# LeiXu84/fireFoam-dev

Measured on AMD Instinct MI355X. Metric: PIMPLE outer-iterations/sec on 64M-cell hex mesh; pEqn SpMV GB/s vs HBM peak, higher is better.
Workload: dtype f64; 1 GPU; synthetic 400^3 hex box (64000000 cells), buoyant plume + 5-species EDC-shaped source, PIMPLE 1/2/0: rhoEqn + UEqn + YEEqn(4 Yi + h) + 2 pEqn per step; cells=64000000, faces=191520000, parallelism=1 GPU, transport_solvers=PBiCGStab+DILU

## Files before the change

### firefoam-dev_amd/csrc/ffm_fused.hip

```cpp
#include "ffm_mesh.hpp"

constexpr int FUSE_MAX = 4;
#define CHECK_M(m) if (!(m)) { ffm_set_error("null mesh"); return FFM_ERR_ARG; }

struct GradMulti {
    const double *vf[FUSE_MAX], *vb[FUSE_MAX];
    double *gx[FUSE_MAX], *gy[FUSE_MAX], *gz[FUSE_MAX];
};

template <int W, int NF>
__global__ __launch_bounds__(256) void k_grad_multi(MeshView q, GradMulti a)
{
    CELL_SCHED(ci, q) {
        const int c = (int)ci;
        RowEnt<W> L, U; load_lower<W>(q.v, c, L); load_upper<W>(q.v, c, U);
        double wl[W], wu[W], sx[2 * W], sy[2 * W], sz[2 * W];
#pragma unroll
        for (int s = 0; s < W; s++) {
            wl[s] = q.w[L.f[s]]; wu[s] = q.w[U.f[s]];
            sx[s] = q.Sfx[L.f[s]]; sy[s] = q.Sfy[L.f[s]]; sz[s] = q.Sfz[L.f[s]];
            sx[W + s] = q.Sfx[U.f[s]]; sy[W + s] = q.Sfy[U.f[s]]; sz[W + s] = q.Sfz[U.f[s]];
        }
        const double V = q.V[c];
        const int j = q.cellB[c];
#pragma unroll 1
        for (int i = 0; i < NF; i++) {
            const double *__restrict__ vf = a.vf[i];
            const double P = vf[c];
            double vl[W], vu[W];
#pragma unroll
            for (int s = 0; s < W; s++) { vl[s] = vf[L.nb[s]]; vu[s] = vf[U.nb[s]]; }
            double ax = 0, ay = 0, az = 0;
#pragma unroll
            for (int s = 0; s < W; s++) if (L.on[s]) {
                const double ff = wl[s] * vl[s] + (1.0 - wl[s]) * P;
                ax -= sx[s] * ff; ay -= sy[s] * ff; az -= sz[s] * ff;
            }
#pragma unroll
            for (int s = 0; s < W; s++) if (U.on[s]) {
                const double ff = wu[s] * P + (1.0 - wu[s]) * vu[s];
                ax += sx[W + s] * ff; ay += sy[W + s] * ff; az += sz[W + s] * ff;
            }
            if (j >= 0) for (int t = q.bcStart[j]; t < q.bcStart[j + 1]; t++) {
                const int k = q.bcItem[t]; const double b = a.vb[i][k];
                ax += q.bSfx[k] * b; ay += q.bSfy[k] * b; az += q.bSfz[k] * b;
            }
            a.gx[i][c] = ax / V; a.gy[i][c] = ay / V; a.gz[i][c] = az / V;
        }
    }
}

__device__ __forceinline__ double limited_weight(int scheme, double twoByk, double lo, double hi, double flux, double wlin,
                                                 double P, double Nn, double dx, double dy, double dz, double gxu, double gyu, double gzu)
{
    const double p0 = flux >= 0 ? 1.0 : 0.0;
    const double gradf = Nn - P;
    const double gradcf = dx * gxu + dy * gyu + dz * gzu;
    double r;
    if (fabs(gradcf) >= 1000.0 * fabs(gradf)) {
        const double sa = gradcf >= 0 ? 1.0 : -1.0, sb = gradf >= 0 ? 1.0 : -1.0;
        r = 2.0 * 1000.0 * sa * sb - 1.0;
    } else r = 2.0 * (gradcf / gradf) - 1.0;
    double lim = fmax(fmin(twoByk * r, 1.0), 0.0);
    if (scheme == 3) {
        if ((flux > 0 && (P < lo || Nn > hi)) || (flux < 0 && (Nn < lo || P > hi))) lim = 0.0;
    }
    return lim * wlin + (1.0 - lim) * p0;
}

struct ScalarEqns {
    const double *vf[FUSE_MAX], *gx[FUSE_MAX], *gy[FUSE_MAX], *gz[FUSE_MAX], *vf0[FUSE_MAX];
    const double *f[FUSE_MAX], *ref[FUSE_MAX], *refGrad[FUSE_MAX];
    const double *su[FUSE_MAX];
    const double *su2[FUSE_MAX], *sp[FUSE_MAX];
    const double *expl[FUSE_MAX][3];
    double *diag[FUSE_MAX], *upper[FUSE_MAX], *lower[FUSE_MAX], *src[FUSE_MAX];
    const double *rho, *rho0, *phi, *phib, *gamma, *gammab;
    const double *Cx, *Cy, *Cz, *bMagSf, *bDelta;
    double rdt, twoByk, lo, hi;
    int scheme;
    const double *wGiven;
    int nOffDiag;
};

template <int W, int NF, bool GIVENW = false>
__global__ __launch_bounds__(256, ((NF > 1 && !GIVENW) ? 4 : 1)) void k_scalar_eqns(MeshView q, ScalarEqns a)
{
    CELL_SCHED(ci, q) {
        const int c = (int)ci;
        RowEnt<W> L, U; load_lower<W>(q.v, c, L); load_upper<W>(q.v, c, U);
        double fl[W], fu[W], wl[W], wu[W], gl[W], gu[W], dlx[W], dly[W], dlz[W], dux[W], duy[W], duz[W];
        const double cx = GIVENW ? 0.0 : a.Cx[c], cy = GIVENW ? 0.0 : a.Cy[c], cz = GIVENW ? 0.0 : a.Cz[c];
#pragma unroll
        for (int s = 0; s < W; s++) {
            const int el = L.f[s], eu = U.f[s];
            fl[s] = a.phi[el]; fu[s] = a.phi[eu];
            wl[s] = GIVENW ? a.wGiven[el] : q.w[el]; wu[s] = GIVENW ? a.wGiven[eu] : q.w[eu];
            gl[s] = a.gamma[el] * q.magSf[el] * q.delta[el]; gu[s] = a.gamma[eu] * q.magSf[eu] * q.delta[eu];
            if (!GIVENW) {
                dlx[s] = cx - a.Cx[L.nb[s]]; dly[s] = cy - a.Cy[L.nb[s]]; dlz[s] = cz - a.Cz[L.nb[s]];
                dux[s] = a.Cx[U.nb[s]] - cx; duy[s] = a.Cy[U.nb[s]] - cy; duz[s] = a.Cz[U.nb[s]] - cz;
            } else { dlx[s] = dly[s] = dlz[s] = dux[s] = duy[s] = duz[s] = 0.0; }
        }
        const double V = q.V[c], rhoc = a.rho[c], rho0c = a.rho0[c];
        const int j = q.cellB[c];
#ifndef FFM_SE2_UNROLL
#define FFM_SE2_UNROLL 1
#endif
#pragma unroll FFM_SE2_UNROLL
        for (int i = 0; i < NF; i++) {
            const double *__restrict__ vf = a.vf[i], *__restrict__ gx = a.gx[i], *__restrict__ gy = a.gy[i], *__restrict__ gz = a.gz[i];
            const double P = GIVENW ? 0.0 : vf[c], gxc = GIVENW ? 0.0 : gx[c], gyc = GIVENW ? 0.0 : gy[c], gzc = GIVENW ? 0.0 : gz[c];
            double dDiv = 0.0, dLap = 0.0;
#pragma unroll
            for (int s = 0; s < W; s++) if (L.on[s]) {
                const int o = L.nb[s];
                const double flux = fl[s];
                const bool upO = flux > 0;
                const double w = GIVENW ? wl[s] : limited_weight(a.scheme, a.twoByk, a.lo, a.hi, flux, wl[s], vf[o], P, dlx[s], dly[s], dlz[s],
                                                                  upO ? gx[o] : gxc, upO ? gy[o] : gyc, upO ? gz[o] : gzc);
                (void)o; (void)upO;
                const double lo = -w * flux;
                dDiv -= (lo + flux);
                dLap -= gl[s];
            }
#pragma unroll
            for (int s = 0; s < W; s++) if (U.on[s]) {
                const int n = U.nb[s];
                const double flux = fu[s];
                const bool upO = flux > 0;
                const double w = GIVENW ? wu[s] : limited_weight(a.scheme, a.twoByk, a.lo, a.hi, flux, wu[s], P, vf[n], dux[s], duy[s], duz[s],
                                                                  upO ? gxc : gx[n], upO ? gyc : gy[n], upO ? gzc : gz[n]);
                (void)n; (void)upO;
                double lo = -w * flux, up = lo + flux;
                dDiv -= lo;
                dLap -= gu[s];
                lo = lo - gu[s]; up = up - gu[s];
                if (!GIVENW || i < a.nOffDiag) { a.upper[i][U.f[s]] = up; a.lower[i][U.f[s]] = lo; }
            }
            double d = a.rdt * rhoc * V;
            d = d + dDiv;
            d = d - dLap;
            double sc = a.rdt * rho0c * a.vf0[i][c] * V;
            if (a.expl[i][0]) sc = ((sc - V * a.expl[i][0][c]) - V * a.expl[i][1][c]) - V * a.expl[i][2][c];
            if (a.su[i]) sc = sc + V * a.su[i][c];
            if (a.sp[i]) d = d + V * a.sp[i][c];
            if (a.su2[i]) sc = sc + V * a.su2[i][c];
            if (j >= 0) for (int t = q.bcStart[j]; t < q.bcStart[j + 1]; t++) {
                const int k = q.bcItem[t];
                const double fk = a.f[i][k], rk = a.ref[i][k], gk = a.refGrad[i][k], dk = a.bDelta[k], pb = a.phib[k];
                double ic = pb * (1.0 - fk), bc = -pb * (fk * rk + (1.0 - fk) * gk / dk);
                const double pG = a.gammab[k] * a.bMagSf[k];
                const double li = pG * (-fk * dk), lb = -pG * (fk * dk * rk + (1.0 - fk) * gk);
                ic = ic - li; bc = bc - lb;
                d += ic; sc += bc;
            }
            a.diag[i][c] = d; a.src[i][c] = sc;
        }
    }
}

constexpr int MV_MAX = 8;
struct MvWeights {
    const double *vf[MV_MAX], *gx[MV_MAX], *gy[MV_MAX], *gz[MV_MAX];
    int scheme[MV_MAX], nf;
    const double *phi, *Cx, *Cy, *Cz;
    double twoByk, lo, hi;
    double *out;
};
__device__ __forceinline__ double mv_limiter(int scheme, double twoByk, double lo, double hi, double flux, double P, double Nn, double gradcf)
{
    const double gradf = Nn - P;
    double r;
    if (fabs(gradcf) >= 1000.0 * fabs(gradf)) {
        const double sa = gradcf >= 0 ? 1.0 : -1.0, sb = gradf >= 0 ? 1.0 : -1.0;
        r = 2.0 * 1000.0 * sa * sb - 1.0;
    } else r = 2.0 * (gradcf / gradf) - 1.0;
    double l = fmax(fmin(twoByk * r, 1.0), 0.0);
    if (scheme == 3) {
        if ((flux > 0 && (P < lo || Nn > hi)) || (flux < 0 && (Nn < lo || P > hi))) l = 0.0;
    }
    return l;
}
template <int W>
__global__ __launch_bounds__(256) void k_mv_weights(MeshView q, MvWeights a)
{
    CELL_SCHED(ci, q) {
        const int c = (int)ci;
        RowEnt<W> L, U; load_lower<W>(q.v, c, L); load_upper<W>(q.v, c, U);
        const double cx = a.Cx[c], cy = a.Cy[c], cz = a.Cz[c];
        double fl[2 * W], lim[2 * W], dx[2 * W], dy[2 * W], dz[2 * W];
        bool mine[2 * W], ghostUp[W];
#pragma unroll
        for (int s = 0; s < W; s++) {
            fl[s] = L.on[s] ? a.phi[L.f[s]] : 0.0; mine[s] = L.on[s] && !(fl[s] > 0);
            dx[s] = cx - a.Cx[L.nb[s]]; dy[s] = cy - a.Cy[L.nb[s]]; dz[s] = cz - a.Cz[L.nb[s]];
            fl[W + s] = U.on[s] ? a.phi[U.f[s]] : 0.0; mine[W + s] = U.on[s] && fl[W + s] > 0;
            ghostUp[s] = U.on[s] && !(fl[W + s] > 0) && U.nb[s] >= q.v.N;
            dx[W + s] = a.Cx[U.nb[s]] - cx; dy[W + s] = a.Cy[U.nb[s]] - cy; dz[W + s] = a.Cz[U.nb[s]] - cz;
            lim[s] = lim[W + s] = 1.0;
        }
#pragma unroll 1
        for (int i = 0; i < a.nf; i++) {
            const double *__restrict__ vf = a.vf[i];
            const double vc = vf[c], gxc = a.gx[i][c], gyc = a.gy[i][c], gzc = a.gz[i][c];
            const int sch = a.scheme[i];
#pragma unroll
            for (int s = 0; s < W; s++) {
                if (mine[s]) {
                    const double l = mv_limiter(sch, a.twoByk, a.lo, a.hi, fl[s], vf[L.nb[s]], vc, dx[s] * gxc + dy[s] * gyc + dz[s] * gzc);
                    lim[s] = i == 0 ? l : fmin(lim[s], l);
                }
                if (mine[W + s]) {
                    const double l = mv_limiter(sch, a.twoByk, a.lo, a.hi, fl[W + s], vc, vf[U.nb[s]], dx[W + s] * gxc + dy[W + s] * gyc + dz[W + s] * gzc);
                    lim[W + s] = i == 0 ? l : fmin(lim[W + s], l);
                } else if (ghostUp[s]) {
                    const int n = U.nb[s];
                    const double l = mv_limiter(sch, a.twoByk, a.lo, a.hi, fl[W + s], vc, vf[n], dx[W + s] * a.gx[i][n] + dy[W + s] * a.gy[i][n] + dz[W + s] * a.gz[i][n]);
                    lim[W + s] = i == 0 ? l : fmin(lim[W + s], l);
                }
            }
        }
#pragma unroll
        for (int s = 0; s < W; s++) {
            if (mine[s]) { const int e = L.f[s]; const double p0 = fl[s] >= 0 ? 1.0 : 0.0; a.out[e] = lim[s] * q.w[e] + (1.0 - lim[s]) * p0; }
            if (mine[W + s] || ghostUp[s]) { const int e = U.f[s]; const double p0 = fl[W + s] >= 0 ? 1.0 : 0.0; a.out[e] = lim[W + s] * q.w[e] + (1.0 - lim[W + s]) * p0; }
        }
    }
// ... 111 lines not shown
                }
#pragma unroll
                for (int s = 0; s < 2 * W; s++) gcur[s] = gnext[s];
            }
#pragma unroll
            for (int s = 0; s < W; s++) {
                if (mine[s]) { const int e = L.f[s]; const double p0 = fl[s] >= 0 ? 1.0 : 0.0; a.out[e] = lim[s] * q.w[e] + (1.0 - lim[s]) * p0; }
                if (mine[W + s]) { const int e = U.f[s]; const double p0 = fl[W + s] >= 0 ? 1.0 : 0.0; a.out[e] = lim[W + s] * q.w[e] + (1.0 - lim[W + s]) * p0; }
            }
        }
        __syncthreads();
    }
}

extern "C" int ffm_fv_multivariate_weights_tiled(ffm_mesh *m, int nf, const int *schemes, double k, double lo, double hi, const double *phi_f,
                                                 const double *const *vf, const double *const *vb, double *out_w)
{
    CHECK_M(m);
    if (nf < 1 || !schemes || !phi_f || !vf || !vb || !out_w) return FFM_ERR_ARG;
    FfmFvSegs sg;
    if (nf > MVT_FLD || m->A->maxW > 3 || !ffm_tile_fv_segments(m->A, MVT_RUN, &sg)) return FFM_ERR_UNSUPPORTED;
    MvTile a;
    for (int i = 0; i < MVT_FLD; i++) {
        const int qq = i < nf ? i : 0;
        if (i < nf && ((schemes[qq] != 2 && schemes[qq] != 3) || !vf[qq] || (m->B && !vb[qq]))) return FFM_ERR_ARG;
        a.vf[i] = vf[qq]; a.vb[i] = vb[qq]; a.scheme[i] = schemes[qq];
    }
    a.nf = nf; a.phi = phi_f; a.Cx = m->C[0]; a.Cy = m->C[1]; a.Cz = m->C[2]; a.twoByk = 2.0 / std::max(k, 1e-15); a.lo = lo; a.hi = hi; a.out = out_w;
    a.seg = sg.seg; a.rec = sg.rec;
    hipLaunchKernelGGL(k_mv_tile<3>, dim3(sg.nSeg), dim3(256), 0, m->ctx->stream, mview(m), a);
    FFM_HIP(hipGetLastError());
    return FFM_OK;
}

struct LustSource {
    const double *gx[3], *gy[3], *gz[3], *U0[3];
    double *src[3];
    const double *phi, *rho0, *Cx, *Cy, *Cz, *Cfx, *Cfy, *Cfz;
    double rdt;
};

template <int W>
__global__ __launch_bounds__(256) void k_lust_source(MeshView q, LustSource a)
{
    CELL_SCHED(ci, q) {
        const int c = (int)ci;
        RowEnt<W> L, U; load_lower<W>(q.v, c, L); load_upper<W>(q.v, c, U);
        const double cx = a.Cx[c], cy = a.Cy[c], cz = a.Cz[c];
        double fl[W], fu[W], dlx[W], dly[W], dlz[W], dux[W], duy[W], duz[W];
        int upl[W], upu[W];
#pragma unroll
        for (int s = 0; s < W; s++) {
            const int el = L.f[s], eu = U.f[s];
            fl[s] = a.phi[el]; fu[s] = a.phi[eu];
            upl[s] = fl[s] > 0 ? L.nb[s] : c;
            upu[s] = fu[s] > 0 ? c : U.nb[s];
            dlx[s] = a.Cfx[el] - a.Cx[upl[s]]; dly[s] = a.Cfy[el] - a.Cy[upl[s]]; dlz[s] = a.Cfz[el] - a.Cz[upl[s]];
            dux[s] = a.Cfx[eu] - a.Cx[upu[s]]; duy[s] = a.Cfy[eu] - a.Cy[upu[s]]; duz[s] = a.Cfz[eu] - a.Cz[upu[s]];
        }
        (void)cx; (void)cy; (void)cz;
        const double V = q.V[c], r0 = a.rho0[c];
#pragma unroll
        for (int i = 0; i < 3; i++) {
            const double *__restrict__ gx = a.gx[i], *__restrict__ gy = a.gy[i], *__restrict__ gz = a.gz[i];
            double acc = 0.0;
#pragma unroll
            for (int s = 0; s < W; s++) if (L.on[s]) {
                const int u = upl[s];
                const double corr = 0.25 * ((dlx[s] * gx[u] + dly[s] * gy[u]) + dlz[s] * gz[u]);
                acc -= fl[s] * corr;
            }
#pragma unroll
            for (int s = 0; s < W; s++) if (U.on[s]) {
                const int u = upu[s];
                const double corr = 0.25 * ((dux[s] * gx[u] + duy[s] * gy[u]) + duz[s] * gz[u]);
                acc += fu[s] * corr;
            }
            const double divc = acc / V;
            a.src[i][c] = a.rdt * r0 * a.U0[i][c] * V - V * divc;
        }
    }
}


extern "C" int ffm_fvc_grad_multi(ffm_mesh *m, int nf, const double *const *vf, const double *const *vb, double *const *gx,
                                  double *const *gy, double *const *gz)
{
    CHECK_M(m);
    if (nf < 1 || nf > FUSE_MAX || !vf || !vb || !gx || !gy || !gz) return FFM_ERR_ARG;
    GradMulti a;
    for (int i = 0; i < FUSE_MAX; i++) { const int k = i < nf ? i : 0; a.vf[i] = vf[k]; a.vb[i] = vb[k]; a.gx[i] = gx[k]; a.gy[i] = gy[k]; a.gz[i] = gz[k]; }
    for (int i = 0; i < nf; i++) if (!vf[i] || (m->B && !vb[i]) || !gx[i] || !gy[i] || !gz[i]) return FFM_ERR_ARG;
#define GM(NF) FFM_DISPATCH_W(m->A->maxW, LAUNCH_CELLS((k_grad_multi<W, NF>), mview(m), a))
    switch (nf) { case 1: GM(1); break; case 2: GM(2); break; case 3: GM(3); break; default: GM(4); break; }
#undef GM
    FFM_HIP(hipGetLastError());
    return FFM_OK;
}

extern "C" int ffm_fvm_scalar_transport_multi(ffm_mesh *m, int nf, int scheme, double k, double lo, double hi, double rDeltaT,
                                              const double *rho, const double *rho0, const double *phi_f, const double *phi_b,
                                              const double *gamma_f, const double *gamma_b,
                                              const double *const *vf, const double *const *gx, const double *const *gy,
                                              const double *const *gz, const double *const *vf0, const double *const *f,
                                              const double *const *ref, const double *const *refGrad, const double *const *su,
                                              const double *const *su2, const double *const *sp,
                                              const double *const *expl3, double *const *diag, double *const *upper,
                                              double *const *lower, double *const *source)
{
    CHECK_M(m);
    if (nf < 1 || nf > FUSE_MAX || (scheme != 2 && scheme != 3) || !rho || !rho0 || !phi_f || !gamma_f || (m->B && (!phi_b || !gamma_b)))
        return FFM_ERR_ARG;
    if (!vf || !gx || !gy || !gz || !vf0 || !f || !ref || !refGrad || !diag || !upper || !lower || !source) return FFM_ERR_ARG;
    ScalarEqns a;
    for (int i = 0; i < FUSE_MAX; i++) {
        const int q = i < nf ? i : 0;
        if (i < nf && (!vf[q] || !gx[q] || !gy[q] || !gz[q] || !vf0[q] || !diag[q] || !upper[q] || !lower[q] || !source[q] ||
                       (m->B && (!f[q] || !ref[q] || !refGrad[q])))) return FFM_ERR_ARG;
        a.vf[i] = vf[q]; a.gx[i] = gx[q]; a.gy[i] = gy[q]; a.gz[i] = gz[q]; a.vf0[i] = vf0[q];
        a.f[i] = f[q]; a.ref[i] = ref[q]; a.refGrad[i] = refGrad[q];
        a.su[i] = su ? su[q] : nullptr;
        a.su2[i] = su2 ? su2[q] : nullptr; a.sp[i] = sp ? sp[q] : nullptr;
        for (int e = 0; e < 3; e++) a.expl[i][e] = expl3 ? expl3[3 * q + e] : nullptr;
        if (a.expl[i][0] && (!a.expl[i][1] || !a.expl[i][2])) return FFM_ERR_ARG;
        a.diag[i] = diag[q]; a.upper[i] = upper[q]; a.lower[i] = lower[q]; a.src[i] = source[q];
    }
    a.rho = rho; a.rho0 = rho0; a.phi = phi_f; a.phib = phi_b; a.gamma = gamma_f; a.gammab = gamma_b;
    a.Cx = m->C[0]; a.Cy = m->C[1]; a.Cz = m->C[2]; a.bMagSf = m->bMagSf; a.bDelta = m->bDelta;
    a.rdt = rDeltaT; a.twoByk = 2.0 / std::max(k, 1e-15); a.lo = lo; a.hi = hi; a.scheme = scheme; a.wGiven = nullptr; a.nOffDiag = nf;
#define SE(NF) FFM_DISPATCH_W(m->A->maxW, LAUNCH_CELLS((k_scalar_eqns<W, NF>), mview(m), a))
    switch (nf) { case 1: SE(1); break; case 2: SE(2); break; case 3: SE(3); break; default: SE(4); break; }
#undef SE
    FFM_HIP(hipGetLastError());
    return FFM_OK;
}

extern "C" int ffm_fv_multivariate_weights(ffm_mesh *m, int nf, const int *schemes, double k, double lo, double hi, const double *phi_f,
                                           const double *const *vf, const double *const *gx, const double *const *gy, const double *const *gz,
                                           double *out_w)
{
    CHECK_M(m);
    if (nf < 1 || nf > MV_MAX || !schemes || !phi_f || !vf || !gx || !gy || !gz || !out_w) return FFM_ERR_ARG;
    MvWeights a;
    for (int i = 0; i < MV_MAX; i++) {
        const int q = i < nf ? i : 0;
        if (i < nf && ((schemes[q] != 2 && schemes[q] != 3) || !vf[q] || !gx[q] || !gy[q] || !gz[q])) return FFM_ERR_ARG;
        a.vf[i] = vf[q]; a.gx[i] = gx[q]; a.gy[i] = gy[q]; a.gz[i] = gz[q]; a.scheme[i] = schemes[q];
    }
    a.nf = nf; a.phi = phi_f; a.Cx = m->C[0]; a.Cy = m->C[1]; a.Cz = m->C[2]; a.twoByk = 2.0 / std::max(k, 1e-15); a.lo = lo; a.hi = hi; a.out = out_w;
    FFM_DISPATCH_W(m->A->maxW, LAUNCH_CELLS(k_mv_weights<W>, mview(m), a));
    FFM_HIP(hipGetLastError());
    return FFM_OK;
}

extern "C" int ffm_fvm_scalar_transport_multi_w(ffm_mesh *m, int nf, const double *w_f, double rDeltaT, const double *rho, const double *rho0,
                                                const double *phi_f, const double *phi_b, const double *gamma_f, const double *gamma_b,
                                                const double *const *vf0, const double *const *f, const double *const *ref,
                                                const double *const *refGrad, const double *const *su, const double *const *su2,
                                                const double *const *sp, const double *const *expl3, double *const *diag,
                                                double *const *upper, double *const *lower, double *const *source)
{
    CHECK_M(m);
    if (nf < 1 || nf > FUSE_MAX || !w_f || !rho || !rho0 || !phi_f || !gamma_f || (m->B && (!phi_b || !gamma_b))) return FFM_ERR_ARG;
    if (!vf0 || !f || !ref || !refGrad || !diag || !upper || !lower || !source) return FFM_ERR_ARG;
    ScalarEqns a;
    for (int i = 0; i < FUSE_MAX; i++) {
        const int q = i < nf ? i : 0;
        if (i < nf && (!vf0[q] || !diag[q] || !source[q] || (m->B && (!f[q] || !ref[q] || !refGrad[q])))) return FFM_ERR_ARG;
        a.vf[i] = a.gx[i] = a.gy[i] = a.gz[i] = nullptr; a.vf0[i] = vf0[q];
        a.f[i] = f[q]; a.ref[i] = ref[q]; a.refGrad[i] = refGrad[q];
        a.su[i] = su ? su[q] : nullptr;
        a.su2[i] = su2 ? su2[q] : nullptr; a.sp[i] = sp ? sp[q] : nullptr;
        for (int e = 0; e < 3; e++) a.expl[i][e] = expl3 ? expl3[3 * q + e] : nullptr;
        if (a.expl[i][0] && (!a.expl[i][1] || !a.expl[i][2])) return FFM_ERR_ARG;
        a.diag[i] = diag[q]; a.upper[i] = upper[q]; a.lower[i] = lower[q]; a.src[i] = source[q];
    }
    a.rho = rho; a.rho0 = rho0; a.phi = phi_f; a.phib = phi_b; a.gamma = gamma_f; a.gammab = gamma_b;
    a.Cx = m->C[0]; a.Cy = m->C[1]; a.Cz = m->C[2]; a.bMagSf = m->bMagSf; a.bDelta = m->bDelta;
    a.rdt = rDeltaT; a.twoByk = 2.0; a.lo = 0.0; a.hi = 1.0; a.scheme = 0; a.wGiven = w_f;
    a.nOffDiag = 0;
    for (int i = 0; i < nf; i++) { if (upper[i] && lower[i]) { if (a.nOffDiag != i) return FFM_ERR_ARG; a.nOffDiag = i + 1; } else if ((upper[i] == nullptr) != (lower[i] == nullptr)) return FFM_ERR_ARG; }
#define SEW(NF) FFM_DISPATCH_W(m->A->maxW, LAUNCH_CELLS((k_scalar_eqns<W, NF, true>), mview(m), a))
    switch (nf) { case 1: SEW(1); break; case 2: SEW(2); break; case 3: SEW(3); break; default: SEW(4); break; }
#undef SEW
    FFM_HIP(hipGetLastError());
    return FFM_OK;
}

extern "C" int ffm_fvm_lust_source3(ffm_mesh *m, double rDeltaT, const double *phi_f, const double *rho0, const double *const *U0,
                                    const double *const *gx, const double *const *gy, const double *const *gz, double *const *source)
{
    CHECK_M(m);
    if (!phi_f || !rho0 || !U0 || !gx || !gy || !gz || !source) return FFM_ERR_ARG;
    if (!m->Cf[0]) { ffm_set_error("ffm_fvm_lust_source3: face centres not set (ffm_mesh_set_face_centres)"); return FFM_ERR_ARG; }
    LustSource a;
    for (int i = 0; i < 3; i++) {
        if (!U0[i] || !gx[i] || !gy[i] || !gz[i] || !source[i]) return FFM_ERR_ARG;
        a.gx[i] = gx[i]; a.gy[i] = gy[i]; a.gz[i] = gz[i]; a.U0[i] = U0[i]; a.src[i] = source[i];
    }
    a.phi = phi_f; a.rho0 = rho0; a.Cx = m->C[0]; a.Cy = m->C[1]; a.Cz = m->C[2]; a.Cfx = m->Cf[0]; a.Cfy = m->Cf[1]; a.Cfz = m->Cf[2];
    a.rdt = rDeltaT;
    FFM_DISPATCH_W(m->A->maxW, LAUNCH_CELLS(k_lust_source<W>, mview(m), a));
    FFM_HIP(hipGetLastError());
    return FFM_OK;
}

struct HbyA3 {
    const double *upper, *lower, *src[3], *ic[3], *bc[3], *psi[3], *rAU;
    double *out[3];
};
template <int W>
__global__ __launch_bounds__(256) void k_matrix_HbyA3(MeshView q, HbyA3 a)
{
    CELL_SCHED(ci, q) {
        const int c = (int)ci;
        RowEnt<W> L, U; load_lower<W>(q.v, c, L); load_upper<W>(q.v, c, U);
        double al[W], au[W];
#pragma unroll
        for (int s = 0; s < W; s++) { al[s] = a.lower[L.f[s]]; au[s] = a.upper[U.f[s]]; }
        double bd[3] = {0.0, 0.0, 0.0}, bda = 0.0, bs[3] = {0.0, 0.0, 0.0};
        const int j = q.cellB[c];
        if (j >= 0) for (int t = q.bcStart[j]; t < q.bcStart[j + 1]; t++) {
            const int k = q.bcItem[t];
            const double i0 = a.ic[0][k], i1 = a.ic[1][k], i2 = a.ic[2][k];
            bd[0] += i0; bd[1] += i1; bd[2] += i2; bda += (i0 + i1 + i2) / 3.0;
            bs[0] += a.bc[0][k]; bs[1] += a.bc[1][k]; bs[2] += a.bc[2][k];
        }
        const double V = q.V[c], r = a.rAU ? a.rAU[c] : 1.0;
#pragma unroll
        for (int d = 0; d < 3; d++) {
            const double *psi = a.psi[d];
            double hl = 0.0;
#pragma unroll
            for (int s = 0; s < W; s++) if (L.on[s]) hl -= al[s] * psi[L.nb[s]];
#pragma unroll
            for (int s = 0; s < W; s++) if (U.on[s]) hl -= au[s] * psi[U.nb[s]];
            double h = (bda - bd[d]) * psi[c];
            h += hl + a.src[d][c];
            h += bs[d];
            h = h / V;
            a.out[d][c] = a.rAU ? r * h : h;
        }
    }
}

extern "C" int ffm_fvm_HbyA3(ffm_mesh *m, const double *upper, const double *lower, const double *const *source, const double *const *ic,
                             const double *const *bc, const double *const *psi, const double *rAU, double *const *out)
{
    CHECK_M(m);
    if (!upper || !lower || !source || !ic || !bc || !psi || !out) return FFM_ERR_ARG;
    HbyA3 a; a.upper = upper; a.lower = lower; a.rAU = rAU;
    for (int d = 0; d < 3; d++) {
        if (!source[d] || !psi[d] || !out[d] || (m->B && (!ic[d] || !bc[d]))) return FFM_ERR_ARG;
        a.src[d] = source[d]; a.ic[d] = ic[d]; a.bc[d] = bc[d]; a.psi[d] = psi[d]; a.out[d] = out[d];
    }
    FFM_DISPATCH_W(m->A->maxW, LAUNCH_CELLS(k_matrix_HbyA3<W>, mview(m), a));
    FFM_HIP(hipGetLastError());
    return FFM_OK;
}

__global__ __launch_bounds__(256) void k_flux_rho(MeshView q, const double *__restrict__ rho, const double *__restrict__ vx,
                                                  const double *__restrict__ vy, const double *__restrict__ vz, double *__restrict__ out)
{
    CELL_SCHED(ci, q) {
        const int c = (int)ci; const double rP = rho[c]; const double Px = rP * vx[c], Py = rP * vy[c], Pz = rP * vz[c];
        FOR_OWN_FACES(q, c, e, nb) {
            const double w = q.w[e], rN = rho[nb];
            out[e] = (w * Px + (1.0 - w) * (rN * vx[nb])) * q.Sfx[e] + (w * Py + (1.0 - w) * (rN * vy[nb])) * q.Sfy[e] + (w * Pz + (1.0 - w) * (rN * vz[nb])) * q.Sfz[e];
        }
    }
}
extern "C" int ffm_fvc_flux_rho(ffm_mesh *m, const double *rho, const double *vx, const double *vy, const double *vz, double *out_f)
{
    CHECK_M(m);
    if (!rho || !vx || !vy || !vz || !out_f) return FFM_ERR_ARG;
    LAUNCH_CELLS(k_flux_rho, mview(m), rho, vx, vy, vz, out_f);
    FFM_HIP(hipGetLastError());
    return FFM_OK;
}

#define PC_ALL_SLOTS(q, c, e, nb)                                                      \
    const int sl_ = (c) >> 6, lane_ = (c)&63;                                          \
    const int ub_ = up_base((q).v, sl_), uw_ = up_width((q).v, sl_);                   \
    for (int s_ = 0, e = ub_ + lane_, nb = 0; s_ < uw_ && ((nb = (q).v.upNbr[e]), true); s_++, e += 64)
__global__ __launch_bounds__(256) void k_pc_phig(MeshView q, const double *__restrict__ rhorAUf, const double *__restrict__ ghf,
                                                 const double *__restrict__ rho, double *__restrict__ out)
{
    CELL_SCHED(ci, q) {
        const int c = (int)ci; const double P = rho[c];
        PC_ALL_SLOTS(q, c, e, nb) {
            if (nb < 0) { out[e] = 0.0; continue; }
            const double sg = q.delta[e] * (rho[nb] - P); out[e] = -rhorAUf[e] * ghf[e] * sg * q.magSf[e];
        }
    }
}
__global__ __launch_bounds__(256) void k_pc_phiHbyA(MeshView q, const double *__restrict__ rho, const double *__restrict__ vx,
                                                    const double *__restrict__ vy, const double *__restrict__ vz, const double *__restrict__ rhorAUf,
                                                    const double *__restrict__ dc, const double *__restrict__ phig, double *__restrict__ out)
{
    CELL_SCHED(ci, q) {
        const int c = (int)ci; const double rP = rho[c]; const double Px = rP * vx[c], Py = rP * vy[c], Pz = rP * vz[c];
        PC_ALL_SLOTS(q, c, e, nb) {
            if (nb < 0) { out[e] = 0.0; continue; }
            const double w = q.w[e], rN = rho[nb];
            const double fl = (w * Px + (1.0 - w) * (rN * vx[nb])) * q.Sfx[e] + (w * Py + (1.0 - w) * (rN * vy[nb])) * q.Sfy[e] + (w * Pz + (1.0 - w) * (rN * vz[nb])) * q.Sfz[e];
            out[e] = (fl + rhorAUf[e] * dc[e]) + phig[e];
        }
    }
}
__global__ __launch_bounds__(256) void k_pc_flux(MeshView q, const double *__restrict__ upper, const double *__restrict__ lower,
                                                 const double *__restrict__ psi, const double *__restrict__ phiHbyA, const double *__restrict__ phig,
                                                 const double *__restrict__ rhorAUf, double *__restrict__ fl, double *__restrict__ phi,
                                                 double *__restrict__ t)
{
    CELL_SCHED(ci, q) {
        const int c = (int)ci; const double P = psi[c];
        PC_ALL_SLOTS(q, c, e, nb) {
            if (nb < 0) { fl[e] = 0.0; phi[e] = 0.0; t[e] = 0.0; continue; }
            const double f = upper[e] * psi[nb] - lower[e] * P;
            fl[e] = f; phi[e] = phiHbyA[e] + f;
            t[e] = rhorAUf[e] != 0.0 ? (f + phig[e]) / rhorAUf[e] : 0.0;
        }
    }
}
__global__ __launch_bounds__(256) void k_ue_buoyancy_flux(MeshView q, const double *__restrict__ ghf, const double *__restrict__ rho,
                                                         const double *__restrict__ prgh, double *__restrict__ out)
{
    CELL_SCHED(ci, q) {
        const int c = (int)ci; const double rP = rho[c], pP = prgh[c];
        PC_ALL_SLOTS(q, c, e, nb) {
            if (nb < 0) { out[e] = 0.0; continue; }
            const double sgr = q.delta[e] * (rho[nb] - rP), sgp = q.delta[e] * (prgh[nb] - pP);
            out[e] = (-ghf[e] * sgr - sgp) * q.magSf[e];
        }
    }
}
extern "C" int ffm_ue_buoyancy_flux(ffm_mesh *m, const double *ghf, const double *rho, const double *p_rgh, double *t_f)
{
    CHECK_M(m);
    if (!ghf || !rho || !p_rgh || !t_f) return FFM_ERR_ARG;
    LAUNCH_CELLS(k_ue_buoyancy_flux, mview(m), ghf, rho, p_rgh, t_f);
    FFM_HIP(hipGetLastError());
    return FFM_OK;
}
extern "C" int ffm_pc_phig(ffm_mesh *m, const double *rhorAUf, const double *ghf, const double *rho, double *phig)
{
    CHECK_M(m);
    if (!rhorAUf || !ghf || !rho || !phig) return FFM_ERR_ARG;
    LAUNCH_CELLS(k_pc_phig, mview(m), rhorAUf, ghf, rho, phig);
    FFM_HIP(hipGetLastError());
    return FFM_OK;
}
extern "C" int ffm_pc_phiHbyA(ffm_mesh *m, const double *rho, const double *vx, const double *vy, const double *vz, const double *rhorAUf,
// ... 193 lines not shown
```

### firefoam-dev_amd/csrc/ffm_fv.hip

```cpp
#include "ffm_internal.hpp"
#include "ffm_device.hpp"
#include <algorithm>
#include <cmath>

#include "ffm_mesh.hpp"

template <class T, class Al> static int up(ffm_ctx *c, T **d, const std::vector<T, Al> &v)
{
    return ffm_upload_vec(c, d, v);
}

extern "C" int ffm_mesh_create(ffm_ldu *A, const double *V, const double *C, const double *Sf, const double *magSf,
                               const double *weights, const double *deltaCoeffs, int nPatches, const int *patchSizes,
                               const int *const *faceCells, const double *const *pSf, const double *const *pDelta,
                               ffm_mesh **out)
{
    if (!A || !V || !C || !out || nPatches < 0) return FFM_ERR_ARG;
    if (!A->identity) { ffm_set_error("ffm_mesh_create needs a mesh numbered with ffm_renumber_levels (native order)"); return FFM_ERR_UNSUPPORTED; }
    ffm_mesh *m = new ffm_mesh();
    m->A = A; m->ctx = A->ctx; m->N = A->nCells; m->F = A->nFaces; m->nNat = A->upTotal; m->nPatches = nPatches;
    const int N = m->N, F = m->F, nNat = m->nNat;
    m->patchOff.assign(nPatches + 1, 0);
    for (int p = 0; p < nPatches; p++) m->patchOff[p + 1] = m->patchOff[p] + patchSizes[p];
    m->B = m->patchOff[nPatches];
// ... 227 lines not shown
                const double d2 = (dx * a.gx[2][cc] + dy * a.gy[2][cc]) + dz * a.gz[2][cc];
                tc[s] = 2.0 * ((g0 * d0 + g1 * d1) + g2 * d2);
            }
            const double den = fmax(fabs(tc[0]), fabs(tc[1])) + 1.0e-15;
            double lim = (df > 0) ? l1 - kk * fmin(fmax(df - tc[0], 0.0), fmax(df - tc[1], 0.0)) / den
                                  : l1 - kk * fmin(fmax(tc[0] - df, 0.0), fmax(tc[1] - df, 0.0)) / den;
            lim = fmax(fmin(lim, 1.0), 0.0);
            const double p0 = phi[e] >= 0 ? 1.0 : 0.0;
            out[e] = lim * q.w[e] + (1.0 - lim) * p0;
        }
    }
}

__global__ void k_lust_correction(MeshView q, const double *__restrict__ phi, const double *__restrict__ gx, const double *__restrict__ gy,
                                  const double *__restrict__ gz, const double *__restrict__ Cx, const double *__restrict__ Cy,
                                  const double *__restrict__ Cz, const double *__restrict__ Cfx, const double *__restrict__ Cfy,
                                  const double *__restrict__ Cfz, double factor, double *__restrict__ out)
{
    CELL_SCHED(ci, q) {
        const int c = (int)ci;
        FOR_OWN_FACES(q, c, e, nb) {
            const int up = phi[e] > 0 ? c : nb;
            const double dx = Cfx[e] - Cx[up], dy = Cfy[e] - Cy[up], dz = Cfz[e] - Cz[up];
            out[e] = factor * ((dx * gx[up] + dy * gy[up]) + dz * gz[up]);
        }
    }
}

template <int W>
__global__ void k_relax(MeshView q, double alpha, int nc, const double *__restrict__ upper, const double *__restrict__ lower,
                        const double *__restrict__ ic0, const double *__restrict__ ic1, const double *__restrict__ ic2,
                        double *__restrict__ diag, const double *__restrict__ p0, const double *__restrict__ p1,
                        const double *__restrict__ p2, double *__restrict__ s0, double *__restrict__ s1, double *__restrict__ s2)
{
    CELL_SCHED(ci, q) {
        const int c = (int)ci;
        RowEnt<W> L, U; load_lower<W>(q.v, c, L); load_upper<W>(q.v, c, U);
        double sumOff = 0.0;
#pragma unroll
        for (int s = 0; s < W; s++) if (L.on[s]) sumOff += fabs(lower[L.f[s]]);
#pragma unroll
        for (int s = 0; s < W; s++) if (U.on[s]) sumOff += fabs(upper[U.f[s]]);
        const double D0 = diag[c];
        double D = D0;
        const int j = q.cellB[c];
        if (j >= 0) for (int t = q.bcStart[j]; t < q.bcStart[j + 1]; t++) {
            const int k = q.bcItem[t];
            D += (nc == 3) ? fmax(fmax(fabs(ic0[k]), fabs(ic1[k])), fabs(ic2[k])) : fabs(ic0[k]);
        }
        D = fmax(fabs(D), sumOff);
        D = D / alpha;
        if (j >= 0) for (int t = q.bcStart[j]; t < q.bcStart[j + 1]; t++) {
            const int k = q.bcItem[t];
            D -= (nc == 3) ? fmin(fmin(ic0[k], ic1[k]), ic2[k]) : ic0[k];
        }
        diag[c] = D;
        const double dd = D - D0;
        s0[c] += dd * p0[c];
        if (nc == 3) { s1[c] += dd * p1[c]; s2[c] += dd * p2[c]; }
    }
}

template <int MODE, int W>
__global__ void k_face_sum(MeshView q, const double *__restrict__ ssf, const double *__restrict__ ssb, double *__restrict__ out)
{
    CELL_SCHED(ci, q) {
        const int c = (int)ci;
        RowEnt<W> L, U; load_lower<W>(q.v, c, L); load_upper<W>(q.v, c, U);
        double a[W], b[W];
#pragma unroll
        for (int s = 0; s < W; s++) { a[s] = ssf[L.f[s]]; b[s] = ssf[U.f[s]]; }
        double acc = 0.0;
#pragma unroll
        for (int s = 0; s < W; s++) if (L.on[s]) acc = (MODE == 0) ? acc - a[s] : acc + a[s];
#pragma unroll
        for (int s = 0; s < W; s++) if (U.on[s]) acc += b[s];
        const int j = q.cellB[c];
        if (j >= 0 && ssb) for (int t = q.bcStart[j]; t < q.bcStart[j + 1]; t++) acc += ssb[q.bcItem[t]];
        out[c] = (MODE == 0) ? acc / q.V[c] : acc;
    }
}

template <int W>
__global__ void k_grad(MeshView q, const double *__restrict__ vf, const double *__restrict__ vb, double *__restrict__ gx,
                       double *__restrict__ gy, double *__restrict__ gz)
{
    CELL_SCHED(ci, q) {
        const int c = (int)ci;
        RowEnt<W> L, U; load_lower<W>(q.v, c, L); load_upper<W>(q.v, c, U);
        const double P = vf[c];
        double vl[W], vu[W], wl[W], wu[W], sx[2 * W], sy[2 * W], sz[2 * W];
#pragma unroll
        for (int s = 0; s < W; s++) {
            vl[s] = vf[L.nb[s]]; vu[s] = vf[U.nb[s]]; wl[s] = q.w[L.f[s]]; wu[s] = q.w[U.f[s]];
            sx[s] = q.Sfx[L.f[s]]; sy[s] = q.Sfy[L.f[s]]; sz[s] = q.Sfz[L.f[s]];
            sx[W + s] = q.Sfx[U.f[s]]; sy[W + s] = q.Sfy[U.f[s]]; sz[W + s] = q.Sfz[U.f[s]];
        }
        double ax = 0, ay = 0, az = 0;
#pragma unroll
        for (int s = 0; s < W; s++) if (L.on[s]) {
            const double ff = wl[s] * vl[s] + (1.0 - wl[s]) * P;
            ax -= sx[s] * ff; ay -= sy[s] * ff; az -= sz[s] * ff;
        }
#pragma unroll
        for (int s = 0; s < W; s++) if (U.on[s]) {
            const double ff = wu[s] * P + (1.0 - wu[s]) * vu[s];
            ax += sx[W + s] * ff; ay += sy[W + s] * ff; az += sz[W + s] * ff;
        }
        const int j = q.cellB[c];
        if (j >= 0) for (int t = q.bcStart[j]; t < q.bcStart[j + 1]; t++) {
            const int k = q.bcItem[t]; const double b = vb[k];
            ax += q.bSfx[k] * b; ay += q.bSfy[k] * b; az += q.bSfz[k] * b;
        }
        const double V = q.V[c];
        gx[c] = ax / V; gy[c] = ay / V; gz[c] = az / V;
    }
}

template <int W>
__global__ void k_reconstruct(MeshView q, long invStride, const double *__restrict__ invT, const double *__restrict__ bMagSf,
                              const double *__restrict__ ssf, const double *__restrict__ ssb, double *__restrict__ ox,
                              double *__restrict__ oy, double *__restrict__ oz)
{
    CELL_SCHED(ci, q) {
        const int c = (int)ci; const long N = invStride;
        RowEnt<W> L, U; load_lower<W>(q.v, c, L); load_upper<W>(q.v, c, U);
        double vx = 0, vy = 0, vz = 0;
#pragma unroll
        for (int s = 0; s < W; s++) if (L.on[s]) {
            const int e = L.f[s]; const double t = ssf[e], mg = q.magSf[e];
            vx += q.Sfx[e] / mg * t; vy += q.Sfy[e] / mg * t; vz += q.Sfz[e] / mg * t;
        }
#pragma unroll
        for (int s = 0; s < W; s++) if (U.on[s]) {
            const int e = U.f[s]; const double t = ssf[e], mg = q.magSf[e];
            vx += q.Sfx[e] / mg * t; vy += q.Sfy[e] / mg * t; vz += q.Sfz[e] / mg * t;
        }
        const int j = q.cellB[c];
        if (j >= 0 && ssb) for (int t = q.bcStart[j]; t < q.bcStart[j + 1]; t++) {
            const int k = q.bcItem[t]; const double b = ssb[k], mg = bMagSf[k];
            vx += q.bSfx[k] / mg * b; vy += q.bSfy[k] / mg * b; vz += q.bSfz[k] / mg * b;
        }
        const double xx = invT[c], xy = invT[N + c], xz = invT[2 * N + c], yy = invT[3 * N + c], yz = invT[4 * N + c], zz = invT[5 * N + c];
        ox[c] = xx * vx + xy * vy + xz * vz; oy[c] = xy * vx + yy * vy + yz * vz; oz[c] = xz * vx + yz * vy + zz * vz;
    }
}

template <int W>
__global__ void k_fvm_transport(MeshView q, double rDeltaT, const double *__restrict__ rho, const double *__restrict__ phi,
                                const double *__restrict__ wf, const double *__restrict__ gamma, double lapSign,
                                double *__restrict__ diag, double *__restrict__ upper, double *__restrict__ lower)
{
    CELL_SCHED(ci, q) {
        const int c = (int)ci;
        RowEnt<W> L, U; load_lower<W>(q.v, c, L); load_upper<W>(q.v, c, U);
        double dDiv = 0.0, dLap = 0.0;
#pragma unroll
        for (int s = 0; s < W; s++) if (L.on[s]) {
            const int e = L.f[s];
            if (phi) { const double f = phi[e]; const double lo = -wf[e] * f; dDiv -= (lo + f); }
            if (gamma) dLap -= gamma[e] * q.magSf[e] * q.delta[e];
        }
#pragma unroll
        for (int s = 0; s < W; s++) if (U.on[s]) {
            const int e = U.f[s];
            double lo = 0.0, up = 0.0;
            if (phi) { const double f = phi[e]; lo = -wf[e] * f; up = lo + f; dDiv -= lo; }
            if (gamma) {
                const double g = gamma[e] * q.magSf[e] * q.delta[e];
                dLap -= g;
                if (phi) { lo = lapSign < 0 ? lo - g : lo + g; up = lapSign < 0 ? up - g : up + g; }
                else { lo = lapSign < 0 ? -g : g; up = lo; }
            }
            if (upper) upper[e] = up;
            if (lower) lower[e] = lo;
        }
        double d = rho ? rDeltaT * rho[c] * q.V[c] : 0.0;
        if (phi) d = rho ? d + dDiv : dDiv;
        if (gamma) d = (rho || phi) ? (lapSign < 0 ? d - dLap : d + dLap) : (lapSign < 0 ? -dLap : dLap);
        diag[c] = d;
    }
}

__global__ void k_boundary_coeffs(int B, const double *__restrict__ phib, const double *__restrict__ gammab, double lapSign,
                                  const double *__restrict__ magSf, const double *__restrict__ delta, const double *__restrict__ f,
                                  const double *__restrict__ ref, const double *__restrict__ refGrad, double *__restrict__ ic,
                                  double *__restrict__ bc)
{
    GRID_STRIDE(k, B) {
        const double fk = f[k], rk = ref[k], gk = refGrad[k], dk = delta[k];
        double i = 0.0, b = 0.0;
        if (phib) { i = phib[k] * (1.0 - fk); b = -phib[k] * (fk * rk + (1.0 - fk) * gk / dk); }
        if (gammab) {
            const double pG = gammab[k] * magSf[k];
            const double li = pG * (-fk * dk), lb = -pG * (fk * dk * rk + (1.0 - fk) * gk);
            if (phib) { i = lapSign < 0 ? i - li : i + li; b = lapSign < 0 ? b - lb : b + lb; }
            else { i = lapSign < 0 ? -li : li; b = lapSign < 0 ? -lb : lb; }
        }
        ic[k] = i; bc[k] = b;
    }
}

__global__ void k_bc_values(int B, const int *__restrict__ fc, const double *__restrict__ delta, const double *__restrict__ f,
                            const double *__restrict__ ref, const double *__restrict__ refGrad, const double *__restrict__ vf,
                            double *__restrict__ out)
{ GRID_STRIDE(k, B) out[k] = f[k] * ref[k] + (1.0 - f[k]) * (vf[fc[k]] + refGrad[k] / delta[k]); }

__global__ void k_add_boundary(MeshView q, const double *__restrict__ ic, const double *__restrict__ bc,
                               const double *__restrict__ diag, const double *__restrict__ src, const double *__restrict__ su,
                               double *__restrict__ diagOut, double *__restrict__ srcOut)
{
    CELL_SCHED(ci, q) {
        const int c = (int)ci;
        double d = diag ? diag[c] : 0.0, s = src ? src[c] : 0.0;
        const int j = q.cellB[c];
        if (j >= 0) for (int t = q.bcStart[j]; t < q.bcStart[j + 1]; t++) { const int k = q.bcItem[t]; if (ic) d += ic[k]; if (bc) s += bc[k]; }
        if (su) s += q.V[c] * su[c];
        if (diagOut) diagOut[c] = d;
        if (srcOut) srcOut[c] = s;
    }
}

__global__ void k_matrix_A(MeshView q, int nc, const double *__restrict__ diag, const double *__restrict__ ic0,
                           const double *__restrict__ ic1, const double *__restrict__ ic2, double *__restrict__ out)
{
    CELL_SCHED(ci, q) {
        const int c = (int)ci;
        double d = diag[c];
        const int j = q.cellB[c];
        if (j >= 0) for (int t = q.bcStart[j]; t < q.bcStart[j + 1]; t++) {
            const int k = q.bcItem[t];
            d += (nc == 3) ? (ic0[k] + ic1[k] + ic2[k]) / 3.0 : ic0[k];
        }
        out[c] = d / q.V[c];
    }
}

template <int W>
__global__ void k_matrix_H(MeshView q, int nc, const double *__restrict__ upper, const double *__restrict__ lower,
                           const double *__restrict__ src, const double *__restrict__ icC, const double *__restrict__ ic0,
                           const double *__restrict__ ic1, const double *__restrict__ ic2, const double *__restrict__ bcC,
                           const double *__restrict__ psi, double *__restrict__ out)
{
    CELL_SCHED(ci, q) {
        const int c = (int)ci;
        RowEnt<W> L, U; load_lower<W>(q.v, c, L); load_upper<W>(q.v, c, U);
        double al[W], au[W], xl[W], xu[W];
#pragma unroll
        for (int s = 0; s < W; s++) { al[s] = lower[L.f[s]]; au[s] = upper[U.f[s]]; xl[s] = psi[L.nb[s]]; xu[s] = psi[U.nb[s]]; }
        double bd = 0.0, bda = 0.0, bs = 0.0;
        const int j = q.cellB[c];
        if (j >= 0) for (int t = q.bcStart[j]; t < q.bcStart[j + 1]; t++) {
            const int k = q.bcItem[t];
            bd += icC[k]; bda += (nc == 3) ? (ic0[k] + ic1[k] + ic2[k]) / 3.0 : ic0[k]; bs += bcC[k];
        }
        double hl = 0.0;
#pragma unroll
        for (int s = 0; s < W; s++) if (L.on[s]) hl -= al[s] * xl[s];
#pragma unroll
        for (int s = 0; s < W; s++) if (U.on[s]) hl -= au[s] * xu[s];
        double h = (bda - bd) * psi[c];
        h += hl + src[c];
        h += bs;
        out[c] = h / q.V[c];
    }
}

__global__ void k_matrix_flux(MeshView q, const double *__restrict__ upper, const double *__restrict__ lower,
                              const double *__restrict__ psi, double *__restrict__ out)
{
    CELL_SCHED(ci, q) {
        const int c = (int)ci; const double P = psi[c];
        FOR_OWN_FACES(q, c, e, nb) out[e] = upper[e] * psi[nb] - lower[e] * P;
    }
}
__global__ void k_matrix_flux_b(int B, const int *__restrict__ fc, const double *__restrict__ ic, const double *__restrict__ bc,
                                const double *__restrict__ psi, double *__restrict__ out)
{ GRID_STRIDE(k, B) out[k] = ic[k] * psi[fc[k]] - bc[k]; }

#define CHECK_M(m) if (!(m)) { ffm_set_error("null mesh"); return FFM_ERR_ARG; }
#define DONE() FFM_HIP(hipGetLastError()); return FFM_OK

extern "C" int ffm_fvc_interpolate(ffm_mesh *m, const double *w_f, const double *vf, double *out_f)
{ CHECK_M(m); LAUNCH_CELLS(k_interpolate, mview(m), w_f, vf, out_f); DONE(); }
extern "C" int ffm_fvc_snGrad(ffm_mesh *m, const double *vf, double *out_f)
{ CHECK_M(m); LAUNCH_CELLS(k_snGrad, mview(m), vf, out_f); DONE(); }
extern "C" int ffm_fvc_snGrad_b(ffm_mesh *m, const double *vf, const double *vb, double *out_b)
{ CHECK_M(m); if (m->B) LAUNCH(k_snGrad_b, m->B, m->B, m->bCells, m->bDelta, vf, vb, out_b); DONE(); }
extern "C" int ffm_fvc_flux(ffm_mesh *m, const double *vx, const double *vy, const double *vz, double *out_f)
{ CHECK_M(m); LAUNCH_CELLS(k_flux, mview(m), vx, vy, vz, out_f); DONE(); }
extern "C" int ffm_fvc_surface_integrate(ffm_mesh *m, const double *ssf, const double *ssb, double *out)
{ CHECK_M(m); FFM_DISPATCH_W(m->A->maxW, LAUNCH_CELLS((k_face_sum<0, W>), mview(m), ssf, ssb, out)); DONE(); }
extern "C" int ffm_fvc_surface_sum(ffm_mesh *m, const double *ssf, const double *ssb, double *out)
{ CHECK_M(m); FFM_DISPATCH_W(m->A->maxW, LAUNCH_CELLS((k_face_sum<1, W>), mview(m), ssf, ssb, out)); DONE(); }
extern "C" int ffm_fvc_grad(ffm_mesh *m, const double *vf, const double *vb, double *gx, double *gy, double *gz)
{ CHECK_M(m); FFM_DISPATCH_W(m->A->maxW, LAUNCH_CELLS(k_grad<W>, mview(m), vf, vb, gx, gy, gz)); DONE(); }
extern "C" int ffm_fvc_reconstruct(ffm_mesh *m, const double *ssf, const double *ssb, double *ox, double *oy, double *oz)
{ CHECK_M(m); FFM_DISPATCH_W(m->A->maxW, LAUNCH_CELLS(k_reconstruct<W>, mview(m), (long)m->N, m->invT, m->bMagSf, ssf, ssb, ox, oy, oz)); DONE(); }
extern "C" int ffm_fv_limited_weights(ffm_mesh *m, int scheme, double k, double lo, double hi, const double *phi_f,
                                      const double *vf, const double *gx, const double *gy, const double *gz, double *out_w)
{
    CHECK_M(m);
    if (scheme < 0 || scheme > 5 || !phi_f || !out_w || ((scheme == 2 || scheme == 3) && (!vf || !gx || !gy || !gz))) return FFM_ERR_ARG;
    LAUNCH_CELLS(k_limited_weights<0>, mview(m), scheme, 2.0 / std::max(k, 1e-15), lo, hi, phi_f, vf, gx, gy, gz, m->C[0], m->C[1], m->C[2], out_w);
    DONE();
}
extern "C" int ffm_fv_limited_limiter(ffm_mesh *m, int scheme, double k, double lo, double hi, const double *phi_f, const double *vf,
                                      const double *gx, const double *gy, const double *gz, double *lim_f, int accumulateMin)
{
    CHECK_M(m);
    if ((scheme != 2 && scheme != 3) || !phi_f || !lim_f || !vf || !gx || !gy || !gz) return FFM_ERR_ARG;
    if (accumulateMin) LAUNCH_CELLS(k_limited_weights<2>, mview(m), scheme, 2.0 / std::max(k, 1e-15), lo, hi, phi_f, vf, gx, gy, gz, m->C[0], m->C[1], m->C[2], lim_f);
    else LAUNCH_CELLS(k_limited_weights<1>, mview(m), scheme, 2.0 / std::max(k, 1e-15), lo, hi, phi_f, vf, gx, gy, gz, m->C[0], m->C[1], m->C[2], lim_f);
    DONE();
}
__global__ void k_weights_from_limiter(MeshView q, const double *__restrict__ phi, const double *__restrict__ lim, double *__restrict__ out)
{
    CELL_SCHED(ci, q) {
        const int c = (int)ci;
        FOR_OWN_FACES(q, c, e, nb) { (void)nb; const double l = lim[e], p0 = phi[e] >= 0 ? 1.0 : 0.0; out[e] = l * q.w[e] + (1.0 - l) * p0; }
    }
}
extern "C" int ffm_fv_weights_from_limiter(ffm_mesh *m, const double *phi_f, const double *lim_f, double *out_w)
{
    CHECK_M(m);
    if (!phi_f || !lim_f || !out_w) return FFM_ERR_ARG;
    LAUNCH_CELLS(k_weights_from_limiter, mview(m), phi_f, lim_f, out_w);
    DONE();
}
extern "C" int ffm_fv_filtered_linear2V_weights(ffm_mesh *m, double k, double l, const double *phi_f, const double *const *U,
                                                const double *const *gx, const double *const *gy, const double *const *gz, double *out_w)
{
    CHECK_M(m);
    if (!phi_f || !U || !gx || !gy || !gz || !out_w || k < 0 || k > 1 || l < 0 || l > 1) return FFM_ERR_ARG;
    FL2V a;
    for (int d = 0; d < 3; d++) {
        if (!U[d] || !gx[d] || !gy[d] || !gz[d]) return FFM_ERR_ARG;
        a.U[d] = U[d]; a.gx[d] = gx[d]; a.gy[d] = gy[d]; a.gz[d] = gz[d];
    }
    LAUNCH_CELLS(k_filtered_linear2V_weights, mview(m), k, l + 1.0, phi_f, a, m->C[0], m->C[1], m->C[2], out_w);
    DONE();
}
extern "C" int ffm_mesh_set_face_centres(ffm_mesh *m, const double *Cf)
{
    CHECK_M(m);
    if (!Cf) return FFM_ERR_ARG;
    std::vector<double> v(std::max(m->nNat, 1));
    for (int d = 0; d < 3; d++) {
        const int *c2n = m->A->h_callerToNative.data(); double *vp = v.data(); const double *src = Cf + (size_t)d * m->F;
        ffm_parallel_for(m->nNat, [=](long lo, long hi) { for (long q = lo; q < hi; q++) vp[q] = 0.0; });
        ffm_parallel_for(m->F, [=](long lo, long hi) { for (long f = lo; f < hi; f++) vp[c2n[f]] = src[f]; });
        hipFree(m->Cf[d]); m->Cf[d] = nullptr;
        FFM_TRY(up(m->ctx, &m->Cf[d], v));
    }
    return FFM_OK;
}
extern "C" int ffm_mesh_set_nonorth_correction(ffm_mesh *m, const double *corrVec)
{
    CHECK_M(m);
    if (!corrVec) return FFM_ERR_ARG;
    std::vector<double> v(std::max(m->nNat, 1));
    for (int d = 0; d < 3; d++) {
        const int *c2n = m->A->h_callerToNative.data(); double *vp = v.data(); const double *src = corrVec + (size_t)d * m->F;
        ffm_parallel_for(m->nNat, [=](long lo, long hi) { for (long q = lo; q < hi; q++) vp[q] = 0.0; });
        ffm_parallel_for(m->F, [=](long lo, long hi) { for (long f = lo; f < hi; f++) vp[c2n[f]] = src[f]; });
        hipFree(m->corr[d]); m->corr[d] = nullptr;
        FFM_TRY(up(m->ctx, &m->corr[d], v));
    }
    return FFM_OK;
}
extern "C" int ffm_fvc_snGrad_correction(ffm_mesh *m, const double *gx, const double *gy, const double *gz, double *out_f)
{
    CHECK_M(m);
    if (!gx || !gy || !gz || !out_f) return FFM_ERR_ARG;
    if (!m->corr[0]) { ffm_set_error("ffm_fvc_snGrad_correction: correction vectors not set (ffm_mesh_set_nonorth_correction)"); return FFM_ERR_ARG; }
    LAUNCH_CELLS(k_snGrad_correction, mview(m), m->corr[0], m->corr[1], m->corr[2], gx, gy, gz, out_f);
    DONE();
}
extern "C" int ffm_fv_lust_correction(ffm_mesh *m, const double *phi_f, const double *gx, const double *gy, const double *gz, double *out_f)
{
    CHECK_M(m);
    if (!phi_f || !gx || !gy || !gz || !out_f) return FFM_ERR_ARG;
    if (!m->Cf[0]) { ffm_set_error("ffm_fv_lust_correction: face centres not set (ffm_mesh_set_face_centres)"); return FFM_ERR_ARG; }
    LAUNCH_CELLS(k_lust_correction, mview(m), phi_f, gx, gy, gz, m->C[0], m->C[1], m->C[2], m->Cf[0], m->Cf[1], m->Cf[2], 0.25, out_f);
    DONE();
}
extern "C" int ffm_fv_linear_upwind_correction(ffm_mesh *m, const double *phi_f, const double *gx, const double *gy, const double *gz, double *out_f)
{
    CHECK_M(m);
    if (!phi_f || !gx || !gy || !gz || !out_f) return FFM_ERR_ARG;
    if (!m->Cf[0]) { ffm_set_error("ffm_fv_linear_upwind_correction: face centres not set (ffm_mesh_set_face_centres)"); return FFM_ERR_ARG; }
    LAUNCH_CELLS(k_lust_correction, mview(m), phi_f, gx, gy, gz, m->C[0], m->C[1], m->C[2], m->Cf[0], m->Cf[1], m->Cf[2], 1.0, out_f);
    DONE();
}
extern "C" int ffm_fvm_relax(ffm_mesh *m, double alpha, int nc, const double *upper, const double *lower, const double *ic0,
                             const double *ic1, const double *ic2, double *diag, const double *psi0, const double *psi1,
                             const double *psi2, double *src0, double *src1, double *src2)
{
    CHECK_M(m);
    if ((nc != 1 && nc != 3) || !upper || !lower || !diag || !psi0 || !src0 || (m->B && !ic0)) return FFM_ERR_ARG;
    if (nc == 3 && (!psi1 || !psi2 || !src1 || !src2 || (m->B && (!ic1 || !ic2)))) return FFM_ERR_ARG;
    if (alpha <= 0) return FFM_OK;
    FFM_DISPATCH_W(m->A->maxW, LAUNCH_CELLS(k_relax<W>, mview(m), alpha, nc, upper, lower, ic0, ic1, ic2, diag, psi0, psi1, psi2, src0, src1, src2));
    DONE();
}
extern "C" int ffm_fvm_transport(ffm_mesh *m, double rDeltaT, const double *rho, const double *phi_f, const double *w_f,
                                 const double *gamma_f, int laplacianSign, double *diag, double *upper, double *lower)
{
    CHECK_M(m);
    if (!diag || ((phi_f || gamma_f) && !upper) || (phi_f && (!w_f || !lower))) return FFM_ERR_ARG;
    FFM_DISPATCH_W(m->A->maxW, LAUNCH_CELLS(k_fvm_transport<W>, mview(m), rDeltaT, rho, phi_f, w_f, gamma_f, (double)laplacianSign, diag, upper, lower));
    DONE();
}
extern "C" int ffm_fvm_boundary_coeffs(ffm_mesh *m, const double *phib, const double *gammab, int laplacianSign, const double *f,
                                       const double *ref, const double *refGrad, double *ic, double *bc)
{ CHECK_M(m); if (m->B) LAUNCH(k_boundary_coeffs, m->B, m->B, phib, gammab, (double)laplacianSign, m->bMagSf, m->bDelta, f, ref, refGrad, ic, bc); DONE(); }
extern "C" int ffm_bc_values(ffm_mesh *m, const double *f, const double *ref, const double *refGrad, const double *vf, double *out_b)
{ CHECK_M(m); if (m->B) LAUNCH(k_bc_values, m->B, m->B, m->bCells, m->bDelta, f, ref, refGrad, vf, out_b); DONE(); }
extern "C" int ffm_fvm_add_boundary(ffm_mesh *m, const double *ic, const double *bc, const double *diag, const double *src,
                                    const double *su, double *diagOut, double *srcOut)
{ CHECK_M(m); LAUNCH_CELLS(k_add_boundary, mview(m), ic, bc, diag, src, su, diagOut, srcOut); DONE(); }
extern "C" int ffm_fvm_A(ffm_mesh *m, int nc, const double *diag, const double *ic0, const double *ic1, const double *ic2, double *out)
{ CHECK_M(m); if (nc != 1 && nc != 3) return FFM_ERR_ARG; LAUNCH_CELLS(k_matrix_A, mview(m), nc, diag, ic0, ic1, ic2, out); DONE(); }
extern "C" int ffm_fvm_H(ffm_mesh *m, int nc, int cmpt, const double *upper, const double *lower, const double *src,
                         const double *ic0, const double *ic1, const double *ic2, const double *bcC, const double *psi, double *out)
{
    CHECK_M(m); if ((nc != 1 && nc != 3) || cmpt < 0 || cmpt >= nc) return FFM_ERR_ARG;
    const double *icC = cmpt == 0 ? ic0 : cmpt == 1 ? ic1 : ic2;
    FFM_DISPATCH_W(m->A->maxW, LAUNCH_CELLS(k_matrix_H<W>, mview(m), nc, upper, lower, src, icC, ic0, ic1, ic2, bcC, psi, out));
    DONE();
}
extern "C" int ffm_fvm_flux(ffm_mesh *m, const double *upper, const double *lower, const double *ic, const double *bc,
                            const double *psi, double *out_f, double *out_b)
{
    CHECK_M(m);
    if (out_f) LAUNCH_CELLS(k_matrix_flux, mview(m), upper, lower, psi, out_f);
    if (m->B && out_b) LAUNCH(k_matrix_flux_b, m->B, m->B, m->bCells, ic, bc, psi, out_b);
    DONE();
}

extern "C" const double *ffm_mesh_geometry_d(const ffm_mesh *m, int which)
{
    if (!m) return nullptr;
    switch (which) {
    case 0: return m->V; case 1: return m->magSf; case 2: return m->delta; case 3: return m->w; case 4: return m->bMagSf; case 5: return m->bDelta;
    case 6: return m->bSf[0]; case 7: return m->bSf[1]; case 8: return m->bSf[2];
    case 9: return m->Sf[0]; case 10: return m->Sf[1]; case 11: return m->Sf[2]; case 12: return m->C[0]; case 13: return m->C[1]; case 14: return m->C[2];
    }
    return nullptr;
}

const int *ffm_mesh_bcells(const ffm_mesh *m) { return m->bCells; }
const double *ffm_mesh_geom(const ffm_mesh *m, int which)
{
    switch (which) {
    case 0: return m->V; case 1: return m->magSf; case 2: return m->delta; case 3: return m->w;
    case 4: return m->bMagSf; case 5: return m->bDelta; case 6: return m->bSf[0]; case 7: return m->bSf[1]; case 8: return m->bSf[2];
    case 9: return m->Sf[0]; case 10: return m->Sf[1]; case 11: return m->Sf[2]; case 12: return m->C[0]; case 13: return m->C[1]; case 14: return m->C[2];
    }
    return nullptr;
}
```

### firefoam-dev_amd/csrc/ffm_plume.hip

```cpp
#include "ffm_internal.hpp"
#include "ffm_device.hpp"
#include <algorithm>
#include <cmath>
#include <string>

struct ffm_mesh;
extern "C" {
int ffm_ldu_bind_coeffs_native_d(ffm_ldu *, const double *, const double *, const double *, int);
int ffm_mesh_create(ffm_ldu *, const double *, const double *, const double *, const double *, const double *, const double *, int,
                    const int *, const int *const *, const double *const *, const double *const *, ffm_mesh **);
int ffm_mesh_destroy(ffm_mesh *);
int ffm_mesh_set_face_centres(ffm_mesh *, const double *);
int ffm_fv_lust_correction(ffm_mesh *, const double *, const double *, const double *, const double *, double *);
int ffm_fvc_interpolate(ffm_mesh *, const double *, const double *, double *);
int ffm_fvc_snGrad(ffm_mesh *, const double *, double *);
int ffm_fvc_snGrad_b(ffm_mesh *, const double *, const double *, double *);
int ffm_fvc_flux(ffm_mesh *, const double *, const double *, const double *, double *);
int ffm_fvc_surface_integrate(ffm_mesh *, const double *, const double *, double *);
int ffm_fvc_grad(ffm_mesh *, const double *, const double *, double *, double *, double *);
int ffm_fvc_reconstruct(ffm_mesh *, const double *, const double *, double *, double *, double *);
int ffm_fv_limited_weights(ffm_mesh *, int, double, double, double, const double *, const double *, const double *, const double *,
                           const double *, double *);
int ffm_fvm_transport(ffm_mesh *, double, const double *, const double *, const double *, const double *, int, double *, double *, double *);
int ffm_fvm_boundary_coeffs(ffm_mesh *, const double *, const double *, int, const double *, const double *, const double *, double *, double *);
int ffm_bc_values(ffm_mesh *, const double *, const double *, const double *, const double *, double *);
int ffm_fvm_add_boundary(ffm_mesh *, const double *, const double *, const double *, const double *, const double *, double *, double *);
int ffm_fvm_A(ffm_mesh *, int, const double *, const double *, const double *, const double *, double *);
int ffm_fvm_H(ffm_mesh *, int, int, const double *, const double *, const double *, const double *, const double *, const double *,
              const double *, const double *, double *);
int ffm_fvm_flux(ffm_mesh *, const double *, const double *, const double *, const double *, const double *, double *, double *);
int ffm_fvc_grad_multi(ffm_mesh *, int, const double *const *, const double *const *, double *const *, double *const *, double *const *);
int ffm_fvm_scalar_transport_multi(ffm_mesh *, int, int, double, double, double, double, const double *, const double *, const double *,
                                   const double *, const double *, const double *, const double *const *, const double *const *,
                                   const double *const *, const double *const *, const double *const *, const double *const *,
                                   const double *const *, const double *const *, const double *const *, const double *const *,
                                   const double *const *, const double *const *,
                                   double *const *, double *const *, double *const *, double *const *);
int ffm_pc_phig(ffm_mesh *, const double *, const double *, const double *, double *);
int ffm_ue_buoyancy_flux(ffm_mesh *, const double *, const double *, const double *, double *);
int ffm_pc_phiHbyA(ffm_mesh *, const double *, const double *, const double *, const double *, const double *, const double *, const double *, double *);
int ffm_pc_flux(ffm_mesh *, const double *, const double *, const double *, const double *, const double *, const double *, double *, double *, double *);
int ffm_fv_limited_limiter(ffm_mesh *, int, double, double, double, const double *, const double *, const double *, const double *,
                           const double *, double *, int);
int ffm_fv_weights_from_limiter(ffm_mesh *, const double *, const double *, double *);
int ffm_fv_multivariate_weights(ffm_mesh *, int, const int *, double, double, double, const double *, const double *const *,
                                const double *const *, const double *const *, const double *const *, double *);
int ffm_fvm_scalar_transport_multi_w(ffm_mesh *, int, const double *, double, const double *, const double *, const double *, const double *,
                                     const double *, const double *, const double *const *, const double *const *, const double *const *,
                                     const double *const *, const double *const *, const double *const *, const double *const *,
                                     const double *const *, double *const *, double *const *, double *const *, double *const *);
int ffm_fvm_lust_source3(ffm_mesh *, double, const double *, const double *, const double *const *, const double *const *,
                         const double *const *, const double *const *, double *const *);
int ffm_fv_multivariate_weights_tiled(ffm_mesh *, int, const int *, double, double, double, const double *, const double *const *,
                                      const double *const *, double *);
}
const int *ffm_mesh_bcells(const ffm_mesh *m);
const double *ffm_mesh_geom(const ffm_mesh *m, int which);

namespace {
constexpr double RR = 8314.47, CP = 1005.0, TREF = 298.15, PREF = 101325.0, MU = 1.8e-5, PR = 0.7;
constexpr double S_O2 = 3.6282945, HC = 46357151.0, TAU = 0.05, T_IN = 600.0, U_IN = 0.5;
constexpr int NSP = 5, INERT = 4;
const double WMOL[NSP] = {31.9988, 18.0153, 44.0962, 44.01, 28.0134};
const double Y_AMB[NSP] = {0.23301, 0.0, 0.0, 0.0, 0.76699};
const double Y_IN[NSP] = {0.0, 0.0, 1.0, 0.0, 0.0};
const double NU[NSP] = {-S_O2, 4 * 18.0153 / 44.0962, -1.0, 3 * 44.01 / 44.0962, 0.0};
const char *SPN[NSP] = {"O2", "H2O", "C3H8", "CO2", "N2"};
enum { P_INLET = 0, P_FLOOR = 1, P_TOP = 2, P_SIDES = 3 };

template <class F> __global__ void k_for(long n, F f)
{
    for (long i = (long)blockIdx.x * blockDim.x + threadIdx.x; i < n; i += (long)gridDim.x * blockDim.x) f(i);
}
inline int sgrid(long n) { long g = (n + 255) / 256; return (int)std::max(1L, std::min(g, (long)RED_BLOCKS)); }
}

struct SolveLog { char name[16]; ffm_perf perf; };

struct ffm_plume {
    ffm_ctx *ctx = nullptr; ffm_ldu *A = nullptr; ffm_mesh *mesh = nullptr;
    int nx = 0, ny = 0, nz = 0, N = 0, nOwn = 0, F = 0, nNat = 0, B = 0;
    double h = 0.05, dt = 1e-3, rdt = 1e3, time = 0.0;
    std::vector<int> newToOld;
    std::vector<int> faceNewToOld;
    bool mvOverride = false;
    double hAmb = 0.0;
    std::vector<double *> pool;
    double *Y[NSP], *Y0[NSP], *T, *hs, *hs0, *U[3], *U0[3], *p, *p0, *p_rgh, *p_rgh0, *psi, *psi0, *rho, *rho0, *K, *K0, *dpdt;
    double *phi, *phi0, *phib, *phib0, *gh, *ghf, *ph_rgh, *ph_rgh_b;
    double *kind_d;
    double *fU[3], *refU[3], *fS, *refS, *fP, *refP, *gradP, *zeroB, *oneB;
    double *fStaticU[3], *fStaticS, *fStaticH, *fH, *refY[NSP], *refH;
    double *diag, *upper, *lower, *src[3], *ic[3], *bc[3], *dWork, *sWork;
    double *UdW[3] = {nullptr, nullptr, nullptr}, *UsW[3] = {nullptr, nullptr, nullptr};
    double *wN[12], *wF[6], *wB[8];
    double *ddtCorrF = nullptr; bool ddtCorrValid = false;
    double *gM[4][3], *spD[4], *spU[4], *spL[4], *spS[4], *spB[4], *suM[4];
    bool mvSelection = true;
    double *wMv = nullptr, *mvG[2][3] = {{nullptr, nullptr, nullptr}, {nullptr, nullptr, nullptr}};
    bool fused = true;
    double *Udiag, *Uupper, *Ulower, *Usrc[3], *Uic[3], *Ubc[3];
    std::vector<SolveLog> log;
    bool tight = false;
    int stepNo = 0, radFreq = 0;
    std::vector<double> rayD, rayOmega;
    std::vector<int> hL2, hU2, hOldToNew; std::vector<signed char> hFd2;
    int *radCm[3] = {nullptr, nullptr, nullptr}, *radFm[3] = {nullptr, nullptr, nullptr};
    double *radDB = nullptr, *radSB = nullptr, *radPsiB = nullptr, *radUB = nullptr, *radLB = nullptr;
    bool radOrdered = false;
    std::vector<double *> I; double *G = nullptr, *radJ = nullptr, *radW = nullptr, *radJb = nullptr, *radF = nullptr, *radRef = nullptr, *radSrc = nullptr;
    bool radCoupled = false; double radA = 0.1, Ehrr1 = 0.0, Ehrr2 = 0.0;
    double *radE = nullptr, *radShSu = nullptr, *radShSp = nullptr; bool radHaveG = false;
    bool stecklerSolvers = false;
};

#define PL_HIP(call) do { hipError_t e_ = (call); if (e_ != hipSuccess) { ffm_set_error("%s:%d %s", __FILE__, __LINE__, hipGetErrorString(e_)); return FFM_ERR_HIP; } } while (0)

static double *dalloc(ffm_plume *P, size_t n)
{
    double *p = nullptr;
    if (hipMalloc((void **)&p, sizeof(double) * std::max<size_t>(n, 1)) != hipSuccess) return nullptr;
    if (ffm_dzero(P->ctx, p, sizeof(double) * std::max<size_t>(n, 1)) != FFM_OK) { hipFree(p); return nullptr; }
    P->pool.push_back(p);
    return p;
}
static double *dupload(ffm_plume *P, const std::vector<double> &v)
{
    double *p = dalloc(P, v.size());
    if (p && !v.empty() && ffm_h2d(P->ctx, p, v.data(), sizeof(double) * v.size()) != FFM_OK) return nullptr;
    return p;
}
template <class Fn> static void forN(ffm_plume *P, long n, Fn f)
{
    if (n > 0) hipLaunchKernelGGL(k_for<Fn>, dim3(sgrid(n)), dim3(256), 0, P->ctx->stream, n, f);
}
static double *dfill(ffm_plume *P, size_t n, double value)
{
    double *p = dalloc(P, n);
    if (p && n) forN(P, (long)n, [=] __device__(long i) { p[i] = value; });
    return p;
}
static void dcopy(ffm_plume *P, double *d, const double *s, long n)
{ hipMemcpyAsync(d, s, sizeof(double) * n, hipMemcpyDeviceToDevice, P->ctx->stream); }

static int HX(ffm_plume *P, double *f) { return (P->N > P->nOwn) ? ffm_halo_refresh_d(P->A, f) : FFM_OK; }

static void standin_thermo(ffm_plume *P)
{
    double *T = P->T, *psi = P->psi; const double *h = P->hs;
    const double *y0 = P->Y[0], *y1 = P->Y[1], *y2 = P->Y[2], *y3 = P->Y[3], *y4 = P->Y[4];
    const double w0 = WMOL[0], w1 = WMOL[1], w2 = WMOL[2], w3 = WMOL[3], w4 = WMOL[4];
    forN(P, P->N, [=] __device__(long i) {
        const double t = TREF + h[i] / CP;
        T[i] = t;
        psi[i] = 1.0 / (RR * t * ((((y0[i] / w0 + y1[i] / w1) + y2[i] / w2) + y3[i] / w3) + y4[i] / w4));
    });
}
static void mul(ffm_plume *P, double *o, const double *a, const double *b, long n) { forN(P, n, [=] __device__(long i) { o[i] = a[i] * b[i]; }); }

static void zg(ffm_plume *P, double *ob, const double *vf)
{ const int *fc = ffm_mesh_bcells(P->mesh); forN(P, P->B, [=] __device__(long k) { ob[k] = vf[fc[k]]; }); }

static void bc_update_f(ffm_plume *P, double *f, const double *fStatic)
{ const double *pb = P->phib; forN(P, P->B, [=] __device__(long k) { f[k] = fStatic[k] < 0 ? 1.0 - (pb[k] >= 0 ? 1.0 : 0.0) : fStatic[k]; }); }

static int solve_named(ffm_plume *P, const char *name, int solver, int pre, double tol, double relTol, const double *d,
                       const double *up, const double *lo, double *psi, const double *src, bool sameOffDiag = false, bool keepSolver = false)
{
    FFM_TRY(ffm_ldu_bind_coeffs_native_d(P->A, d, up, lo, sameOffDiag ? 1 : 0));
    SolveLog L; memset(&L, 0, sizeof(L)); strncpy(L.name, name, sizeof(L.name) - 1);
    if (P->tight) { tol = 1e-13; relTol = 0.0; }
    int maxIter = 1000;
    if (P->stecklerSolvers && solver == FFM_PBICGSTAB && !keepSolver) { solver = FFM_SMOOTH; pre = FFM_SYMGS; maxIter = P->tight ? 1000 : 10; }
    FFM_TRY(ffm_solve_d(P->A, solver, pre, tol, relTol, 0, maxIter, 1, psi, src, &L.perf));
    P->log.push_back(L);
    return FFM_OK;
}

static int solve_named_multi(ffm_plume *P, int n, const char *const *names, double tol, const double *const *d, const double *up, const double *lo,
                             double *const *psi, const double *const *src)
{
    if (P->stecklerSolvers || n < 2) {
        for (int i = 0; i < n; i++) FFM_TRY(solve_named(P, names[i], FFM_PBICGSTAB, FFM_DILU, tol, 0.0, d[i], up, lo, psi[i], src[i], i > 0));
        return FFM_OK;
    }
    double relTol = 0.0;
    if (P->tight) { tol = 1e-13; relTol = 0.0; }
    std::vector<ffm_perf> pf(n);
    FFM_TRY(ffm_solve_multi_d(P->A, n, FFM_PBICGSTAB, FFM_DILU, tol, relTol, 0, 1000, d, up, lo, psi, src, pf.data()));
    for (int i = 0; i < n; i++) { SolveLog L; memset(&L, 0, sizeof(L)); strncpy(L.name, names[i], sizeof(L.name) - 1); L.perf = pf[i]; P->log.push_back(L); }
    return FFM_OK;
}

static int U_boundary(ffm_plume *P, double *Ub[3])
{
    for (int c = 0; c < 3; c++) FFM_TRY(ffm_bc_values(P->mesh, P->fU[c], P->refU[c], P->zeroB, P->U[c], Ub[c]));
    return FFM_OK;
}

static int update_bcs(ffm_plume *P)
{
    for (int c = 0; c < 3; c++) bc_update_f(P, P->fU[c], P->fStaticU[c]);
    bc_update_f(P, P->fS, P->fStaticS);
    bc_update_f(P, P->fH, P->fStaticH);
    return FFM_OK;
}

static int bc_p_rgh(ffm_plume *P, const double *grad , double *Ub[3], const double *rhob)
{
    const double *kind = P->kind_d, *pb = P->phib, *phb = P->ph_rgh_b;
    const double *u0 = Ub[0], *u1 = Ub[1], *u2 = Ub[2];
    double *f = P->fP, *ref = P->refP, *g = P->gradP;
    forN(P, P->B, [=] __device__(long k) {
        if (kind[k] < 1.5) { f[k] = 0.0; ref[k] = 0.0; g[k] = grad ? grad[k] : 0.0; }
        else {
            f[k] = 1.0; g[k] = 0.0;
            ref[k] = phb[k] - 0.5 * rhob[k] * (1.0 - (pb[k] >= 0 ? 1.0 : 0.0)) * ((u0[k] * u0[k] + u1[k] * u1[k]) + u2[k] * u2[k]);
        }
    });
    return FFM_OK;
}

static int rho_eqn(ffm_plume *P)
{
    double *div = P->wN[0];
    FFM_TRY(ffm_fvc_surface_integrate(P->mesh, P->phi, P->phib, div));
    const double *V = ffm_mesh_geom(P->mesh, 0), *rho0 = P->rho0; double *rho = P->rho; const double rdt = P->rdt;
    forN(P, P->nOwn, [=] __device__(long i) { rho[i] = (rdt * rho0[i] * V[i] - V[i] * div[i]) / (rdt * V[i]); });
    return HX(P, rho);
}

static int hydrostatic_init(ffm_plume *P)
{
    ffm_mesh *m = P->mesh; const int N = P->N, B = P->B;
    double *ph = P->ph_rgh, *rhof = P->wF[0], *sg = P->wF[1], *phig = P->wF[2], *rhob = P->wB[0];
    const double *gh = P->gh, *ghf = P->ghf, *magSf = ffm_mesh_geom(m, 1);
    double *p = P->p, *rho = P->rho; const double *psi = P->psi;
    double *fTop = P->wB[1]; const double *kind = P->kind_d;
    forN(P, B, [=] __device__(long k) { fTop[k] = (kind[k] > 1.5 && kind[k] < 2.5) ? 1.0 : 0.0; });
    forN(P, N, [=] __device__(long i) { p[i] = ph[i] + rho[i] * gh[i] + PREF; });
    standin_thermo(P); mul(P, rho, psi, p, N);
    const long nNat = P->nNat;
    for (int corr = 0; corr < 5; corr++) {
        FFM_TRY(ffm_fvc_interpolate(m, nullptr, rho, rhof));
        zg(P, rhob, rho);
        FFM_TRY(ffm_fvc_snGrad(m, rho, sg));
        forN(P, nNat, [=] __device__(long e) { phig[e] = -rhof[e] * ghf[e] * sg[e] * magSf[e]; });
        FFM_TRY(ffm_fvm_transport(m, 0.0, nullptr, nullptr, nullptr, rhof, +1, P->diag, P->upper, P->lower));
        FFM_TRY(ffm_fvm_boundary_coeffs(m, nullptr, rhob, +1, fTop, P->zeroB, P->zeroB, P->ic[0], P->bc[0]));
        FFM_TRY(ffm_fvc_surface_integrate(m, phig, P->zeroB, P->wN[0]));
        {
            double *s0 = P->src[0]; const double *dv = P->wN[0], *V = ffm_mesh_geom(m, 0);
            forN(P, N, [=] __device__(long i) { s0[i] = V[i] * dv[i]; });
        }
        FFM_TRY(ffm_fvm_add_boundary(m, P->ic[0], P->bc[0], P->diag, P->src[0], nullptr, P->dWork, P->sWork));
        FFM_TRY(solve_named(P, "ph_rgh", FFM_PCG, FFM_DIC, 1e-6, 0.01, P->dWork, P->upper, nullptr, ph, P->sWork));
        FFM_TRY(HX(P, ph));
        forN(P, N, [=] __device__(long i) { p[i] = ph[i] + rho[i] * gh[i] + PREF; });
        standin_thermo(P); mul(P, rho, psi, p, N);
    }
    FFM_TRY(ffm_bc_values(m, fTop, P->zeroB, P->zeroB, ph, P->ph_rgh_b));
    dcopy(P, P->p_rgh, ph, N);
    return FFM_OK;
}

static int scalar_transport(ffm_plume *P, const char *name, int scheme, double *vf, const double *vf0, const double *fBC, const double *ref,
                            const double *gamma_f, const double *gamma_b, const double *su, const double *const *expl, double tol,
                            const double *su2 = nullptr, const double *sp = nullptr, const double *wGiven = nullptr)
{
    ffm_mesh *m = P->mesh; const int N = P->N;
    double *vb = P->wB[2], *gx = P->wN[1], *gy = P->wN[2], *gz = P->wN[3];
    const double *w = wGiven;
    if (!wGiven) {
        FFM_TRY(ffm_bc_values(m, fBC, ref, P->zeroB, vf, vb));
        FFM_TRY(ffm_fvc_grad(m, vf, vb, gx, gy, gz));
        FFM_TRY(HX(P, gx)); FFM_TRY(HX(P, gy)); FFM_TRY(HX(P, gz));
        FFM_TRY(ffm_fv_limited_weights(m, scheme, 1.0, 0.0, 1.0, P->phi, vf, gx, gy, gz, P->wF[3]));
        w = P->wF[3];
    }
    FFM_TRY(ffm_fvm_transport(m, P->rdt, P->rho, P->phi, w, gamma_f, -1, P->diag, P->upper, P->lower));
    FFM_TRY(ffm_fvm_boundary_coeffs(m, P->phib, gamma_b, -1, fBC, ref, P->zeroB, P->ic[0], P->bc[0]));
    const double *V = ffm_mesh_geom(m, 0), *rho0 = P->rho0; double *s = P->src[0]; const double rdt = P->rdt;
    if (expl) { const double *e0 = expl[0], *e1 = expl[1], *e2 = expl[2];
                forN(P, N, [=] __device__(long i) { s[i] = ((rdt * rho0[i] * vf0[i] * V[i] - V[i] * e0[i]) - V[i] * e1[i]) - V[i] * e2[i]; }); }
    else forN(P, N, [=] __device__(long i) { s[i] = rdt * rho0[i] * vf0[i] * V[i]; });
    double *s2 = P->wN[4];
    if (su) { forN(P, N, [=] __device__(long i) { s2[i] = s[i] + V[i] * su[i]; }); }
    else s2 = s;
    if (sp) { double *dg = P->diag; forN(P, N, [=] __device__(long i) { dg[i] = dg[i] + V[i] * sp[i]; }); }
    if (su2) { double *s3 = P->src[1]; const double *sIn = s2; forN(P, N, [=] __device__(long i) { s3[i] = sIn[i] + V[i] * su2[i]; }); s2 = s3; }
    FFM_TRY(ffm_fvm_add_boundary(m, P->ic[0], P->bc[0], P->diag, s2, nullptr, P->dWork, P->sWork));
    FFM_TRY(solve_named(P, name, FFM_PBICGSTAB, FFM_DILU, tol, 0.0, P->dWork, P->upper, P->lower, vf, P->sWork));
    return HX(P, vf);
}

constexpr double SIGMA_SB = 5.670367e-8;
extern "C" int ffm_reduce_sum(ffm_ctx *, const double *, long, double *);
static int plume_rad_fraction(ffm_plume *P, double *out)
{
    const double *kind = P->kind_d, *pb = P->phib; double *t = P->wB[0];
    forN(P, P->B, [=] __device__(long k) { t[k] = kind[k] < 0.5 ? pb[k] : 0.0; });
    double sum = 0.0;
    FFM_TRY(ffm_reduce_sum(P->ctx, t, P->B, &sum));
    const double mlr = -sum, e1 = P->Ehrr1, e2 = P->Ehrr2;
    *out = std::max(std::min(e1, e2), (mlr * e1 + mlr * e2) / std::max(1e-15, mlr + mlr));
    return FFM_OK;
}
static int radiation_correct(ffm_plume *P)
{
    ffm_mesh *m = P->mesh; const int N = P->N, B = P->B; const long nNat = P->nNat;
    const double *V = ffm_mesh_geom(m, 0);
    const double *sx = ffm_mesh_geom(m, 9), *sy = ffm_mesh_geom(m, 10), *sz = ffm_mesh_geom(m, 11);
    const double *bx = ffm_mesh_geom(m, 6), *by = ffm_mesh_geom(m, 7), *bz = ffm_mesh_geom(m, 8);
    const double Ib = SIGMA_SB * ((TREF * TREF) * (TREF * TREF)) / M_PI;
    double *G = P->G, *J = P->radJ, *w = P->radW, *Jb = P->radJb, *f = P->radF, *ref = P->radRef, *su = P->radSrc;
    const double *T = P->T;
    forN(P, N, [=] __device__(long c) { G[c] = 0.0; });
    forN(P, B, [=] __device__(long k) { ref[k] = Ib; });
    const double KA = P->radA;
    const double *Ee = nullptr;
    if (P->radCoupled) {
        double frac = 0.0;
        FFM_TRY(plume_rad_fraction(P, &frac));
        double *E = P->radE; const double *Qd = P->wN[9];
        forN(P, N, [=] __device__(long c) { E[c] = frac * Qd[c]; });
        Ee = E;
    }
    const int nRay = (int)P->rayOmega.size();
    for (int i = 0; i < nRay; i++) {
        const double d0 = P->rayD[3 * i], d1 = P->rayD[3 * i + 1], d2 = P->rayD[3 * i + 2], omega = P->rayOmega[i];
        forN(P, nNat, [=] __device__(long e) { const double j = (d0 * sx[e] + d1 * sy[e]) + d2 * sz[e]; J[e] = j; w[e] = j >= 0 ? 1.0 : 0.0; });
        forN(P, B, [=] __device__(long k) { const double j = (d0 * bx[k] + d1 * by[k]) + d2 * bz[k]; Jb[k] = j; f[k] = 1.0 - (j >= 0 ? 1.0 : 0.0); });
        FFM_TRY(ffm_fvm_transport(m, 0.0, nullptr, J, w, nullptr, -1, P->diag, P->upper, P->lower));
        FFM_TRY(ffm_fvm_boundary_coeffs(m, Jb, nullptr, -1, f, ref, P->zeroB, P->ic[0], P->bc[0]));
        double *dg = P->diag; const double kO = KA * omega, cS = 1.0 / M_PI * omega, kS = KA * SIGMA_SB;
        forN(P, N, [=] __device__(long c) {
            dg[c] = dg[c] + V[c] * kO;
            const double t = T[c];
            su[c] = Ee ? V[c] * (cS * (kS * ((t * t) * (t * t)) + Ee[c] / 4.0)) : V[c] * (cS * (kS * ((t * t) * (t * t))));
        });
        FFM_TRY(ffm_fvm_add_boundary(m, P->ic[0], P->bc[0], P->diag, su, nullptr, P->dWork, P->sWork));
        char nm[16]; snprintf(nm, sizeof(nm), "I%d", i);
        int flip = -1;
        if (P->radOrdered) {
            const int neg = (d0 < 0) + (d1 < 0) + (d2 < 0);
            if (neg == 1) flip = d0 < 0 ? 0 : d1 < 0 ? 1 : 2;
            else if (neg == 2) flip = d0 >= 0 ? 0 : d1 >= 0 ? 1 : 2;
        }
        if (flip < 0) {
            FFM_TRY(solve_named(P, nm, FFM_PBICGSTAB, FFM_DILU, 1e-4, 0.0, P->dWork, P->upper, P->lower, P->I[i], P->sWork, false, true));
        } else {
            const int *cm = P->radCm[flip], *fm = P->radFm[flip];
            const double *dW = P->dWork, *sW = P->sWork, *up = P->upper, *lo = P->lower; double *Ii = P->I[i];
            double *dB = P->radDB, *sB = P->radSB, *pB = P->radPsiB, *uB = P->radUB, *lB = P->radLB;
            forN(P, N, [=] __device__(long c) { const int s = cm[c]; dB[c] = dW[s]; sB[c] = sW[s]; pB[c] = Ii[s]; });
            forN(P, nNat, [=] __device__(long e) {
                const int t = fm[e];
                if (t >= 0) { uB[e] = up[t]; lB[e] = lo[t]; } else { uB[e] = lo[~t]; lB[e] = up[~t]; }
            });
            FFM_TRY(solve_named(P, nm, FFM_PBICGSTAB, FFM_DILU, 1e-4, 0.0, dB, uB, lB, pB, sB, false, true));
            forN(P, N, [=] __device__(long c) { Ii[cm[c]] = pB[c]; });
        }
        FFM_TRY(HX(P, P->I[i]));
        const double *Ii = P->I[i];
        forN(P, N, [=] __device__(long c) { G[c] = G[c] + Ii[c] * omega; });
    }
    P->radHaveG = true;
    return FFM_OK;
}

static int p_corrector(ffm_plume *P, bool final)
{
    ffm_mesh *m = P->mesh; const int N = P->N, B = P->B; const long nNat = P->nNat; const double rdt = P->rdt;
    const double *V = ffm_mesh_geom(m, 0), *magSf = ffm_mesh_geom(m, 1), *bMag = ffm_mesh_geom(m, 4);
    const double *bSx = ffm_mesh_geom(m, 6), *bSy = ffm_mesh_geom(m, 7), *bSz = ffm_mesh_geom(m, 8);
    const double *Sx = ffm_mesh_geom(m, 9), *Sy = ffm_mesh_geom(m, 10), *Sz = ffm_mesh_geom(m, 11), *wlin = ffm_mesh_geom(m, 3);
    double *rho = P->rho; const double *psi = P->psi; double *p = P->p;
    double *rAU = P->wN[0], *rhorAU = P->wN[1], *HbyA[3] = {P->wN[2], P->wN[3], P->wN[4]};
    FFM_TRY(ffm_fvm_A(m, 3, P->Udiag, P->Uic[0], P->Uic[1], P->Uic[2], rAU));
    if (P->fused && P->N == P->nOwn) {
        forN(P, N, [=] __device__(long i) { const double r = psi[i] * p[i], a = 1.0 / rAU[i]; rho[i] = r; rAU[i] = a; rhorAU[i] = r * a; });
    } else {
    mul(P, rho, psi, p, N);
    forN(P, P->nOwn, [=] __device__(long i) { rAU[i] = 1.0 / rAU[i]; });
    FFM_TRY(HX(P, rAU));
    forN(P, N, [=] __device__(long i) { rhorAU[i] = rho[i] * rAU[i]; });
    }
    double *rhorAUf = P->wF[0], *rhorAUfb = P->wB[0];
    FFM_TRY(ffm_fvc_interpolate(m, nullptr, rhorAU, rhorAUf));
    zg(P, rhorAUfb, rhorAU);
    if (P->fused) {
        const double *srcs[3] = {P->Usrc[0], P->Usrc[1], P->Usrc[2]}, *ics[3] = {P->Uic[0], P->Uic[1], P->Uic[2]}, *bcs[3] = {P->Ubc[0], P->Ubc[1], P->Ubc[2]};
        const double *us[3] = {P->U[0], P->U[1], P->U[2]};
        FFM_TRY(ffm_fvm_HbyA3(m, P->Uupper, P->Ulower, srcs, ics, bcs, us, rAU, HbyA));
        for (int c = 0; c < 3; c++) FFM_TRY(HX(P, HbyA[c]));
    } else
    for (int c = 0; c < 3; c++) {
        FFM_TRY(ffm_fvm_H(m, 3, c, P->Uupper, P->Ulower, P->Usrc[c], P->Uic[0], P->Uic[1], P->Uic[2], P->Ubc[c], P->U[c], HbyA[c]));
        double *Hc = HbyA[c];
        forN(P, P->nOwn, [=] __device__(long i) { Hc[i] = rAU[i] * Hc[i]; });
        FFM_TRY(HX(P, Hc));
    }
    FFM_TRY(update_bcs(P));
    double *Ub[3] = {P->wB[1], P->wB[2], P->wB[3]};
    FFM_TRY(U_boundary(P, Ub));
    double *rhob = P->wB[4];
    zg(P, rhob, rho);
    double *sg = P->wF[1], *phig = P->wF[2];
    const double *ghf = P->ghf;
    if (P->fused) FFM_TRY(ffm_pc_phig(m, rhorAUf, ghf, rho, phig));
    else {
    FFM_TRY(ffm_fvc_snGrad(m, rho, sg));
    forN(P, nNat, [=] __device__(long e) { phig[e] = -rhorAUf[e] * ghf[e] * sg[e] * magSf[e]; });
    }
    double *phiHbyA = P->wF[3], *phiHbyAb = P->wB[5];
    if (P->fused) {  }
    else {
        double *rH[3] = {P->wN[5], P->wN[6], P->wN[7]};
        for (int c = 0; c < 3; c++) mul(P, rH[c], rho, HbyA[c], N);
        FFM_TRY(ffm_fvc_flux(m, rH[0], rH[1], rH[2], phiHbyA));
    }
    {
        const int *fc = ffm_mesh_bcells(m); const double *kind = P->kind_d;
        const double *h0 = HbyA[0], *h1 = HbyA[1], *h2 = HbyA[2], *u0 = Ub[0], *u1 = Ub[1], *u2 = Ub[2];
        forN(P, B, [=] __device__(long k) {
            const bool fixed = kind[k] < 1.5; const int c = fc[k];
            const double a0 = fixed ? u0[k] : h0[c], a1 = fixed ? u1[k] : h1[c], a2 = fixed ? u2[k] : h2[c];
            phiHbyAb[k] = (rhob[k] * a0 * bSx[k] + rhob[k] * a1 * bSy[k]) + rhob[k] * a2 * bSz[k];
        });
    }
    {
        double *dc = P->ddtCorrF;
        if (!P->ddtCorrValid) {
            double *fl0 = P->wF[4];
            if (P->fused) FFM_TRY(ffm_fvc_flux_rho(m, P->rho0, P->U0[0], P->U0[1], P->U0[2], fl0));
            else {
                double *rU0[3] = {P->wN[8], P->wN[9], P->wN[10]};
                for (int c = 0; c < 3; c++) mul(P, rU0[c], P->rho0, P->U0[c], N);
                FFM_TRY(ffm_fvc_flux(m, rU0[0], rU0[1], rU0[2], fl0));
            }
            const double *phi0 = P->phi0;
            forN(P, nNat, [=] __device__(long e) {
                const double phiCorr = phi0[e] - fl0[e];
                const double coeff = 1.0 - fmin(fabs(phiCorr) / (fabs(phi0[e]) + 1e-15), 1.0);
                dc[e] = coeff * rdt * phiCorr;
            });
            P->ddtCorrValid = true;
        }
        if (P->fused) FFM_TRY(ffm_pc_phiHbyA(m, rho, HbyA[0], HbyA[1], HbyA[2], rhorAUf, dc, phig, phiHbyA));
        else forN(P, nNat, [=] __device__(long e) { phiHbyA[e] = (phiHbyA[e] + rhorAUf[e] * dc[e]) + phig[e]; });
        (void)Sx; (void)Sy; (void)Sz; (void)wlin;
    }
    double *grads = P->wB[6];
    {
        const double *u0 = Ub[0], *u1 = Ub[1], *u2 = Ub[2];
        forN(P, B, [=] __device__(long k) {
            grads[k] = (phiHbyAb[k] - rhob[k] * ((bSx[k] * u0[k] + bSy[k] * u1[k]) + bSz[k] * u2[k])) / (bMag[k] * rhorAUfb[k]);
        });
    }
    FFM_TRY(bc_p_rgh(P, grads, Ub, rhob));
    if (P->fused) {
        FFM_TRY(ffm_fvm_boundary_coeffs(m, nullptr, rhorAUfb, -1, P->fP, P->refP, P->gradP, P->ic[0], P->bc[0]));
        FFM_TRY(ffm_fvm_pressure_eqn(m, rdt, psi, P->psi0, P->p_rgh0, rho, P->rho0, P->gh, PREF, rhorAUf, phiHbyA, phiHbyAb, P->ic[0], P->bc[0],
                                     P->upper, P->lower, P->dWork, P->sWork));
    } else {
    FFM_TRY(ffm_fvm_transport(m, rdt, psi, nullptr, nullptr, rhorAUf, -1, P->diag, P->upper, P->lower));
    FFM_TRY(ffm_fvm_boundary_coeffs(m, nullptr, rhorAUfb, -1, P->fP, P->refP, P->gradP, P->ic[0], P->bc[0]));
    double *div = P->wN[8];
    FFM_TRY(ffm_fvc_surface_integrate(m, phiHbyA, phiHbyAb, div));
    {
        double *s = P->src[0]; const double *psi0 = P->psi0, *prgh0 = P->p_rgh0, *rho0 = P->rho0, *gh = P->gh;
        forN(P, N, [=] __device__(long i) {
            s[i] = ((rdt * psi0[i] * prgh0[i] * V[i] - V[i] * (rdt * (psi[i] * rho[i] - psi0[i] * rho0[i]) * gh[i]))
                    - V[i] * (rdt * (psi[i] - psi0[i]) * PREF)) - V[i] * div[i];
        });
    }
    FFM_TRY(ffm_fvm_add_boundary(m, P->ic[0], P->bc[0], P->diag, P->src[0], nullptr, P->dWork, P->sWork));
    }
    FFM_TRY(solve_named(P, "p_rgh", FFM_PCG, FFM_DIC, 1e-6, final ? 0.0 : 0.01, P->dWork, P->upper, nullptr, P->p_rgh, P->sWork));
    FFM_TRY(HX(P, P->p_rgh));
    double *fl = P->wF[4], *flb = P->wB[7];
    if (P->fused) {
        FFM_TRY(ffm_fvm_flux(m, P->upper, P->lower, P->ic[0], P->bc[0], P->p_rgh, nullptr, flb));
        FFM_TRY(ffm_pc_flux(m, P->upper, P->lower, P->p_rgh, phiHbyA, phig, rhorAUf, fl, P->phi, P->wF[5]));
    } else
    FFM_TRY(ffm_fvm_flux(m, P->upper, P->lower, P->ic[0], P->bc[0], P->p_rgh, fl, flb));
    {
        double *phi = P->phi, *phib = P->phib, *t = P->wF[5], *tb = P->wB[6];
        if (!P->fused) forN(P, nNat, [=] __device__(long e) { phi[e] = phiHbyA[e] + fl[e]; t[e] = rhorAUf[e] != 0.0 ? (fl[e] + phig[e]) / rhorAUf[e] : 0.0; });
        forN(P, B, [=] __device__(long k) { phib[k] = phiHbyAb[k] + flb[k]; tb[k] = flb[k] / rhorAUfb[k]; });
        double *rx = P->wN[5], *ry = P->wN[6], *rz = P->wN[7];
        FFM_TRY(ffm_fvc_reconstruct(m, t, tb, rx, ry, rz));
        double *U0 = P->U[0], *U1 = P->U[1], *U2 = P->U[2]; const double *h0 = HbyA[0], *h1 = HbyA[1], *h2 = HbyA[2];
        double *K = P->K, *dpdt = P->dpdt; const double *p_rgh = P->p_rgh, *gh = P->gh, *p0 = P->p0;
        if (P->fused && P->N == P->nOwn) {
            forN(P, N, [=] __device__(long i) {
                const double a = h0[i] + rAU[i] * rx[i], b = h1[i] + rAU[i] * ry[i], c = h2[i] + rAU[i] * rz[i];
                U0[i] = a; U1[i] = b; U2[i] = c;
                K[i] = 0.5 * ((a * a + b * b) + c * c);
                const double pp = p_rgh[i] + rho[i] * gh[i] + PREF;
                p[i] = pp; dpdt[i] = rdt * (pp - p0[i]);
            });
            FFM_TRY(rho_eqn(P));
        } else {
        forN(P, P->nOwn, [=] __device__(long i) {
            const double a = h0[i] + rAU[i] * rx[i], b = h1[i] + rAU[i] * ry[i], c = h2[i] + rAU[i] * rz[i];
            U0[i] = a; U1[i] = b; U2[i] = c;
        });
        FFM_TRY(HX(P, U0)); FFM_TRY(HX(P, U1)); FFM_TRY(HX(P, U2));
        forN(P, N, [=] __device__(long i) { p[i] = p_rgh[i] + rho[i] * gh[i] + PREF; });
        FFM_TRY(rho_eqn(P));
        forN(P, N, [=] __device__(long i) {
            K[i] = 0.5 * ((U0[i] * U0[i] + U1[i] * U1[i]) + U2[i] * U2[i]);
            dpdt[i] = rdt * (p[i] - p0[i]);
        });
        }
    }
    return FFM_OK;
}

extern "C" int ffm_plume_step(ffm_plume *P)
{
    if (!P) return FFM_ERR_ARG;
    ffm_mesh *m = P->mesh; const int N = P->N, B = P->B; const long nNat = P->nNat; const double rdt = P->rdt;
    const double *V = ffm_mesh_geom(m, 0), *magSf = ffm_mesh_geom(m, 1);
    P->log.clear();
    P->ddtCorrValid = false;
    dcopy(P, P->rho0, P->rho, N); dcopy(P, P->hs0, P->hs, N); dcopy(P, P->K0, P->K, N); dcopy(P, P->p0, P->p, N);
    dcopy(P, P->psi0, P->psi, N); dcopy(P, P->p_rgh0, P->p_rgh, N); dcopy(P, P->phi0, P->phi, nNat); dcopy(P, P->phib0, P->phib, B);
    for (int c = 0; c < 3; c++) dcopy(P, P->U0[c], P->U[c], N);
    for (int i = 0; i < NSP; i++) dcopy(P, P->Y0[i], P->Y[i], N);
    FFM_TRY(rho_eqn(P));
    FFM_TRY(update_bcs(P));
    double *Ub[3] = {P->wB[1], P->wB[2], P->wB[3]};
    FFM_TRY(U_boundary(P, Ub));
    double *gx = P->wN[1], *gy = P->wN[2], *gz = P->wN[3], *wU = P->wF[3];
    FFM_TRY(ffm_fv_limited_weights(m, 4, 1.0, 0.0, 1.0, P->phi, nullptr, nullptr, nullptr, nullptr, wU));
    double *muf = P->wF[0], *mub = P->wB[4];
    forN(P, nNat, [=] __device__(long e) { muf[e] = MU; });
    forN(P, B, [=] __device__(long k) { mub[k] = MU; });
    FFM_TRY(ffm_fvm_transport(m, rdt, P->rho, P->phi, wU, muf, -1, P->Udiag, P->Uupper, P->Ulower));
    double *sgr = P->wF[1], *sgp = P->wF[2], *t = P->wF[4], *tb = P->wB[5], *rhob = P->wB[6], *pb = P->wB[7];
    if (!P->fused) FFM_TRY(ffm_fvc_snGrad(m, P->rho, sgr));
    zg(P, rhob, P->rho);
    FFM_TRY(bc_p_rgh(P, nullptr, Ub, rhob));
    FFM_TRY(ffm_bc_values(m, P->fP, P->refP, P->gradP, P->p_rgh, pb));
    if (!P->fused) FFM_TRY(ffm_fvc_snGrad(m, P->p_rgh, sgp));
    FFM_TRY(ffm_fvc_snGrad_b(m, P->p_rgh, pb, tb));
    {
        const double *ghf = P->ghf, *bMag = ffm_mesh_geom(m, 4);
        if (P->fused) FFM_TRY(ffm_ue_buoyancy_flux(m, ghf, P->rho, P->p_rgh, t));
        else forN(P, nNat, [=] __device__(long e) { t[e] = (-ghf[e] * sgr[e] - sgp[e]) * magSf[e]; });
        forN(P, B, [=] __device__(long k) { tb[k] = -tb[k] * bMag[k]; });
    }
    double *rx = P->wN[5], *ry = P->wN[6], *rz = P->wN[7];
    FFM_TRY(ffm_fvc_reconstruct(m, t, tb, rx, ry, rz));
    double *rec[3] = {rx, ry, rz};
    if (P->fused) {
        for (int c = 0; c < 3; c++) FFM_TRY(ffm_fvm_boundary_coeffs(m, P->phib, mub, -1, P->fU[c], P->refU[c], P->zeroB, P->Uic[c], P->Ubc[c]));
        const double *uf[3] = {P->U[0], P->U[1], P->U[2]}, *ub[3] = {Ub[0], Ub[1], Ub[2]}, *u0[3] = {P->U0[0], P->U0[1], P->U0[2]};
        double *ggx[3] = {P->gM[0][0], P->gM[1][0], P->gM[2][0]}, *ggy[3] = {P->gM[0][1], P->gM[1][1], P->gM[2][1]}, *ggz[3] = {P->gM[0][2], P->gM[1][2], P->gM[2][2]};
        FFM_TRY(ffm_fvc_grad_multi(m, 3, uf, ub, ggx, ggy, ggz));
        for (int c = 0; c < 3; c++) { FFM_TRY(HX(P, ggx[c])); FFM_TRY(HX(P, ggy[c])); FFM_TRY(HX(P, ggz[c])); }
        FFM_TRY(ffm_fvm_lust_source3(m, rdt, P->phi, P->rho0, u0, ggx, ggy, ggz, P->Usrc));
    } else
    for (int c = 0; c < 3; c++) {
        FFM_TRY(ffm_fvm_boundary_coeffs(m, P->phib, mub, -1, P->fU[c], P->refU[c], P->zeroB, P->Uic[c], P->Ubc[c]));
        double *corr = P->wF[4], *divc = P->wN[4];
        FFM_TRY(ffm_fvc_grad(m, P->U[c], Ub[c], gx, gy, gz));
        FFM_TRY(HX(P, gx)); FFM_TRY(HX(P, gy)); FFM_TRY(HX(P, gz));
        FFM_TRY(ffm_fv_lust_correction(m, P->phi, gx, gy, gz, corr));
        { const double *phi = P->phi; forN(P, nNat, [=] __device__(long e) { corr[e] = phi[e] * corr[e]; }); }
        FFM_TRY(ffm_fvc_surface_integrate(m, corr, P->zeroB, divc));
        double *s = P->Usrc[c]; const double *rho0 = P->rho0, *u0 = P->U0[c];
        forN(P, N, [=] __device__(long i) { s[i] = rdt * rho0[i] * u0[i] * V[i] - V[i] * divc[i]; });
    }
    {
        const char *nm[3] = {"Ux", "Uy", "Uz"};
        const double *dd[3], *ss[3]; double *pp[3];
        for (int c = 0; c < 3; c++) {
            if (!P->UdW[c]) { P->UdW[c] = dalloc(P, N); P->UsW[c] = dalloc(P, N); if (!P->UdW[c] || !P->UsW[c]) return FFM_ERR_HIP; }
            FFM_TRY(ffm_fvm_add_boundary(m, P->Uic[c], P->Ubc[c], P->Udiag, P->Usrc[c], rec[c], P->UdW[c], P->UsW[c]));
            dd[c] = P->UdW[c]; ss[c] = P->UsW[c]; pp[c] = P->U[c];
        }
        FFM_TRY(solve_named_multi(P, 3, nm, 1e-6, dd, P->Uupper, P->Ulower, pp, ss));
        for (int c = 0; c < 3; c++) FFM_TRY(HX(P, P->U[c]));
    }
    {
        double *K = P->K; const double *U0 = P->U[0], *U1 = P->U[1], *U2 = P->U[2];
        forN(P, N, [=] __device__(long i) { K[i] = 0.5 * ((U0[i] * U0[i] + U1[i] * U1[i]) + U2[i] * U2[i]); });
    }
    double *af = P->wF[0], *afb = P->wB[4];
    forN(P, nNat, [=] __device__(long e) { af[e] = 0.5 * (MU / PR) + (1.0 - 0.5) * (MU / PR); });
    forN(P, B, [=] __device__(long k) { afb[k] = MU / PR; });
    double *wFuel = P->wN[8], *Qdot = P->wN[9], *Yt = P->wN[10], *su = P->wN[11];
    {
        const double *rho = P->rho, *fuel = P->Y[2], *o2 = P->Y[0];
        forN(P, N, [=] __device__(long i) { const double w = rho[i] * fmin(fuel[i], o2[i] / S_O2) / TAU; wFuel[i] = w; Qdot[i] = w * HC; Yt[i] = 0.0; });
    }
    if (P->mvSelection && P->mvOverride) P->mvOverride = false;
    else if (P->mvSelection) {
        int sp4[NSP - 1], n4 = 0;
        for (int i = 0; i < NSP; i++) if (i != INERT) sp4[n4++] = i;
        double *Nb = P->wB[1], *hb = P->wB[3];
        for (int j = 0; j < n4; j++) FFM_TRY(ffm_bc_values(m, P->fS, P->refY[sp4[j]], P->zeroB, P->Y[sp4[j]], P->spB[j]));
        {
            const double *b0 = P->spB[0], *b1 = P->spB[1], *b2 = P->spB[2], *b3 = P->spB[3];
            forN(P, B, [=] __device__(long k) { const double t = ((fmax(b0[k], 0.0) + fmax(b1[k], 0.0)) + fmax(b2[k], 0.0)) + fmax(b3[k], 0.0); Nb[k] = fmax(1.0 - t, 0.0); });
        }
        FFM_TRY(ffm_bc_values(m, P->fH, P->refH, P->zeroB, P->hs, hb));
        int rcTiled = FFM_ERR_UNSUPPORTED;
        if (P->fused) {
            const double *af6[6] = {P->hs, P->Y[sp4[0]], P->Y[sp4[1]], P->Y[sp4[2]], P->Y[sp4[3]], P->Y[INERT]};
            const double *ab6[6] = {hb, P->spB[0], P->spB[1], P->spB[2], P->spB[3], Nb};
            const int sch6[6] = {2, 3, 3, 3, 3, 3};
            rcTiled = ffm_fv_multivariate_weights_tiled(m, 6, sch6, 1.0, 0.0, 1.0, P->phi, af6, ab6, P->wMv);
            if (rcTiled != FFM_OK && rcTiled != FFM_ERR_UNSUPPORTED) return rcTiled;
        }
        if (rcTiled == FFM_OK) {  }
        else if (P->fused) {
            const double *vf[6], *vb[4], *cgx[6], *cgy[6], *cgz[6]; double *ggx[4], *ggy[4], *ggz[4]; int sch[6];
            const double *vf2[2] = {P->hs, P->Y[INERT]}, *vb2[2] = {hb, Nb};
            double *g2x[2] = {P->mvG[0][0], P->mvG[1][0]}, *g2y[2] = {P->mvG[0][1], P->mvG[1][1]}, *g2z[2] = {P->mvG[0][2], P->mvG[1][2]};
            FFM_TRY(ffm_fvc_grad_multi(m, 2, vf2, vb2, g2x, g2y, g2z));
            for (int j = 0; j < n4; j++) { vf[j] = P->Y[sp4[j]]; vb[j] = P->spB[j]; ggx[j] = P->gM[j][0]; ggy[j] = P->gM[j][1]; ggz[j] = P->gM[j][2]; }
            FFM_TRY(ffm_fvc_grad_multi(m, n4, vf, vb, ggx, ggy, ggz));
            for (int j = 0; j < 2; j++) { FFM_TRY(HX(P, g2x[j])); FFM_TRY(HX(P, g2y[j])); FFM_TRY(HX(P, g2z[j])); }
            for (int j = 0; j < n4; j++) { FFM_TRY(HX(P, ggx[j])); FFM_TRY(HX(P, ggy[j])); FFM_TRY(HX(P, ggz[j])); }
            const double *af6[6] = {P->hs, P->Y[sp4[0]], P->Y[sp4[1]], P->Y[sp4[2]], P->Y[sp4[3]], P->Y[INERT]};
            for (int j = 0; j < 6; j++) { vf[j] = af6[j]; sch[j] = j == 0 ? 2 : 3; }
            cgx[0] = g2x[0]; cgy[0] = g2y[0]; cgz[0] = g2z[0]; cgx[5] = g2x[1]; cgy[5] = g2y[1]; cgz[5] = g2z[1];
            for (int j = 0; j < n4; j++) { cgx[1 + j] = ggx[j]; cgy[1 + j] = ggy[j]; cgz[1 + j] = ggz[j]; }
            FFM_TRY(ffm_fv_multivariate_weights(m, 6, sch, 1.0, 0.0, 1.0, P->phi, vf, cgx, cgy, cgz, P->wMv));
        } else {
            double *gx = P->wN[1], *gy = P->wN[2], *gz = P->wN[3], *lim = P->wF[1];
            const double *fld[6] = {P->hs, P->Y[sp4[0]], P->Y[sp4[1]], P->Y[sp4[2]], P->Y[sp4[3]], P->Y[INERT]};
            const double *fb[6] = {hb, P->spB[0], P->spB[1], P->spB[2], P->spB[3], Nb};
            for (int j = 0; j < 6; j++) {
                FFM_TRY(ffm_fvc_grad(m, fld[j], fb[j], gx, gy, gz));
                FFM_TRY(HX(P, gx)); FFM_TRY(HX(P, gy)); FFM_TRY(HX(P, gz));
                FFM_TRY(ffm_fv_limited_limiter(m, j == 0 ? 2 : 3, 1.0, 0.0, 1.0, P->phi, fld[j], gx, gy, gz, lim, j == 0 ? 0 : 1));
            }
            FFM_TRY(ffm_fv_weights_from_limiter(m, P->phi, lim, P->wMv));
        }
    }
    if (P->fused) {
        int sp[NSP - 1], ns = 0;
        for (int i = 0; i < NSP; i++) if (i != INERT) sp[ns++] = i;
        const double *vf[4], *vb[4], *vf0[4], *fq[4], *rq[4], *gq[4], *suq[4], *cgx[4], *cgy[4], *cgz[4];
        double *ggx[4], *ggy[4], *ggz[4];
        for (int j = 0; j < ns; j++) {
            const int i = sp[j]; const double nu = NU[i]; double *sj = P->suM[j];
            forN(P, N, [=] __device__(long c) { sj[c] = nu * wFuel[c]; });
            if (!P->mvSelection) FFM_TRY(ffm_bc_values(m, P->fS, P->refY[i], P->zeroB, P->Y[i], P->spB[j]));
            vf[j] = P->Y[i]; vb[j] = P->spB[j]; vf0[j] = P->Y0[i]; fq[j] = P->fS; rq[j] = P->refY[i]; gq[j] = P->zeroB; suq[j] = sj;
            ggx[j] = P->gM[j][0]; ggy[j] = P->gM[j][1]; ggz[j] = P->gM[j][2]; cgx[j] = ggx[j]; cgy[j] = ggy[j]; cgz[j] = ggz[j];
        }
        double *uShared[4] = {P->spU[0], nullptr, nullptr, nullptr}, *lShared[4] = {P->spL[0], nullptr, nullptr, nullptr};
        if (P->mvSelection)
            FFM_TRY(ffm_fvm_scalar_transport_multi_w(m, ns, P->wMv, rdt, P->rho, P->rho0, P->phi, P->phib, af, afb, vf0, fq, rq, gq, suq, nullptr, nullptr,
                                                     nullptr, P->spD, uShared, lShared, P->spS));
        else {
        FFM_TRY(ffm_fvc_grad_multi(m, ns, vf, vb, ggx, ggy, ggz));
        for (int j = 0; j < ns; j++) { FFM_TRY(HX(P, ggx[j])); FFM_TRY(HX(P, ggy[j])); FFM_TRY(HX(P, ggz[j])); }
        FFM_TRY(ffm_fvm_scalar_transport_multi(m, ns, 3, 1.0, 0.0, 1.0, rdt, P->rho, P->rho0, P->phi, P->phib, af, afb, vf, cgx, cgy, cgz, vf0,
                                               fq, rq, gq, suq, nullptr, nullptr, nullptr, P->spD, P->spU, P->spL, P->spS));
        }
        if (P->mvSelection) {
            const char *nmq[4]; const double *dq[4], *sq[4]; double *pq[4];
            for (int j = 0; j < ns; j++) { nmq[j] = SPN[sp[j]]; dq[j] = P->spD[j]; sq[j] = P->spS[j]; pq[j] = P->Y[sp[j]]; }
            FFM_TRY(solve_named_multi(P, ns, nmq, 1e-8, dq, P->spU[0], P->spL[0], pq, sq));
        }
        for (int j = 0; j < ns; j++) {
            const int i = sp[j];
            if (!P->mvSelection) FFM_TRY(solve_named(P, SPN[i], FFM_PBICGSTAB, FFM_DILU, 1e-8, 0.0, P->spD[j], P->spU[j], P->spL[j], P->Y[i], P->spS[j]));
            FFM_TRY(HX(P, P->Y[i]));
            double *Yi = P->Y[i];
            forN(P, N, [=] __device__(long c) { const double v = fmax(Yi[c], 0.0); Yi[c] = v; Yt[c] += v; });
        }
    } else
    for (int i = 0; i < NSP; i++) {
        if (i == INERT) continue;
        const double nu = NU[i];
        forN(P, N, [=] __device__(long c) { su[c] = nu * wFuel[c]; });
        FFM_TRY(scalar_transport(P, SPN[i], 3, P->Y[i], P->Y0[i], P->fS, P->refY[i], af, afb, su, nullptr, 1e-8, nullptr, nullptr, P->mvSelection ? P->wMv : nullptr));
        double *Yi = P->Y[i];
        forN(P, N, [=] __device__(long c) { const double v = fmax(Yi[c], 0.0); Yi[c] = v; Yt[c] += v; });
    }
    {
        double *Yn = P->Y[INERT];
        forN(P, N, [=] __device__(long c) { Yn[c] = fmax(1.0 - Yt[c], 0.0); });
    }
    bool speciesOffDiagBound = P->fused && P->mvSelection;
    if (P->radFreq > 0 && P->stepNo % P->radFreq == 0) { FFM_TRY(radiation_correct(P)); speciesOffDiagBound = false; }
    {
        FFM_TRY(U_boundary(P, Ub));
        double *Kb = P->wB[0], *kgx = P->wN[1], *kgy = P->wN[2], *kgz = P->wN[3], *wK = P->wF[3], *Kf = P->wF[4], *KfB = P->wB[5];
        const double *b0 = Ub[0], *b1 = Ub[1], *b2 = Ub[2];
        forN(P, B, [=] __device__(long k) { Kb[k] = 0.5 * ((b0[k] * b0[k] + b1[k] * b1[k]) + b2[k] * b2[k]); });
        FFM_TRY(ffm_fvc_grad(m, P->K, Kb, kgx, kgy, kgz));
        FFM_TRY(HX(P, kgx)); FFM_TRY(HX(P, kgy)); FFM_TRY(HX(P, kgz));
        FFM_TRY(ffm_fv_limited_weights(m, 2, 1.0, 0.0, 1.0, P->phi, P->K, kgx, kgy, kgz, wK));
        FFM_TRY(ffm_fvc_interpolate(m, wK, P->K, Kf));
        const double *phi = P->phi, *phib = P->phib;
        forN(P, nNat, [=] __device__(long e) { Kf[e] = phi[e] * Kf[e]; });
        forN(P, B, [=] __device__(long k) { KfB[k] = phib[k] * Kb[k]; });
        double *divK = P->wN[4];
        FFM_TRY(ffm_fvc_surface_integrate(m, Kf, KfB, divK));
        double *ddtK = P->wN[0], *ndpdt = P->wN[5]; const double *rho = P->rho, *rho0 = P->rho0, *K = P->K, *K0 = P->K0, *dpdt = P->dpdt;
        forN(P, N, [=] __device__(long c) { ddtK[c] = rdt * (rho[c] * K[c] - rho0[c] * K0[c]); ndpdt[c] = -dpdt[c]; });
        const double *expl[3] = {ddtK, divK, ndpdt};
        const double *shSu = nullptr, *shSp = nullptr;
        if (P->radCoupled && P->radHaveG) {
            double frac = 0.0;
            FFM_TRY(plume_rad_fraction(P, &frac));
            const double Rp = 4.0 * P->radA * SIGMA_SB, KA = P->radA;
            double *su2 = P->radShSu, *sp2 = P->radShSp; const double *G = P->G, *T = P->T, *hh = P->hs, *Qd = Qdot;
            forN(P, N, [=] __device__(long c) {
                const double t = T[c], T3 = t * t * t;
                const double Ru = KA * G[c] - frac * Qd[c];
                sp2[c] = 4.0 * Rp * T3 / CP;
                su2[c] = Ru - Rp * T3 * (t - 4.0 * hh[c] / CP);
            });
            shSu = su2; shSp = sp2;
        }
        if (P->fused) {
            const double *vf[1] = {P->hs}, *vb[1] = {P->spB[0]}, *vf0[1] = {P->hs0}, *fq[1] = {P->fH}, *rq[1] = {P->refH}, *gq[1] = {P->zeroB}, *suq[1] = {Qdot};
            double *ggx[1] = {P->gM[0][0]}, *ggy[1] = {P->gM[0][1]}, *ggz[1] = {P->gM[0][2]};
            const double *cgx[1] = {ggx[0]}, *cgy[1] = {ggy[0]}, *cgz[1] = {ggz[0]}, *su2q[1] = {shSu}, *spq[1] = {shSp};
            double *dd[1] = {P->dWork}, *uu[1] = {P->upper}, *ll[1] = {P->lower}, *ss[1] = {P->sWork};
            const bool shareH = speciesOffDiagBound;
            if (shareH) { uu[0] = nullptr; ll[0] = nullptr; }
            if (P->mvSelection)
                FFM_TRY(ffm_fvm_scalar_transport_multi_w(m, 1, P->wMv, rdt, P->rho, P->rho0, P->phi, P->phib, af, afb, vf0, fq, rq, gq, suq, su2q, spq, expl,
                                                         dd, uu, ll, ss));
            else {
            FFM_TRY(ffm_bc_values(m, P->fH, P->refH, P->zeroB, P->hs, P->spB[0]));
            FFM_TRY(ffm_fvc_grad_multi(m, 1, vf, vb, ggx, ggy, ggz));
            FFM_TRY(HX(P, ggx[0])); FFM_TRY(HX(P, ggy[0])); FFM_TRY(HX(P, ggz[0]));
            FFM_TRY(ffm_fvm_scalar_transport_multi(m, 1, 2, 1.0, 0.0, 1.0, rdt, P->rho, P->rho0, P->phi, P->phib, af, afb, vf, cgx, cgy, cgz, vf0,
                                                   fq, rq, gq, suq, su2q, spq, expl, dd, uu, ll, ss));
            }
            if (shareH) FFM_TRY(solve_named(P, "h", FFM_PBICGSTAB, FFM_DILU, 1e-8, 0.0, P->dWork, P->spU[0], P->spL[0], P->hs, P->sWork, true));
            else FFM_TRY(solve_named(P, "h", FFM_PBICGSTAB, FFM_DILU, 1e-8, 0.0, P->dWork, P->upper, P->lower, P->hs, P->sWork));
            FFM_TRY(HX(P, P->hs));
        } else
        FFM_TRY(scalar_transport(P, "h", 2, P->hs, P->hs0, P->fH, P->refH, af, afb, Qdot, expl, 1e-8, shSu, shSp, P->mvSelection ? P->wMv : nullptr));
    }
    standin_thermo(P);
    FFM_TRY(p_corrector(P, false));
    FFM_TRY(p_corrector(P, true));
    mul(P, P->rho, P->psi, P->p, N);
    P->time += P->dt; P->stepNo++;
    PL_HIP(hipStreamSynchronize(P->ctx->stream));
    return FFM_OK;
}

extern "C" int ffm_plume_create(ffm_ctx *ctx, int nx, int ny, int nz, double h, double dt, ffm_plume **out)
{
    const int lo[3] = {0, 0, 0}, hi[3] = {nx, ny, nz}, nbr[6] = {-1, -1, -1, -1, -1, -1};
    return ffm_plume_create_block(ctx, nx, ny, nz, lo, hi, nbr, h, dt, out);
}

extern "C" int ffm_plume_create_block(ffm_ctx *ctx, int gx, int gy, int gz, const int *lo, const int *hi, const int *nbrRank,
                                      double h, double dt, ffm_plume **out)
{
    if (!ctx || !out || !lo || !hi || !nbrRank) return FFM_ERR_ARG;
    const int nx = hi[0] - lo[0], ny = hi[1] - lo[1], nz = hi[2] - lo[2];
    if (nx < 2 || ny < 2 || nz < 2) { ffm_set_error("plume block must be at least 2 cells wide in every direction"); return FFM_ERR_ARG; }
    for (int d = 0; d < 3; d++) {
        const int G = d == 0 ? gx : d == 1 ? gy : gz;
        if ((lo[d] == 0) != (nbrRank[2 * d] < 0) || (hi[d] == G) != (nbrRank[2 * d + 1] < 0)) { ffm_set_error("plume block: neighbour ranks inconsistent with the block position"); return FFM_ERR_ARG; }
    }
    PL_HIP(hipSetDevice(ctx->device));
    FfmStageTimer tmAll_("plume_create: total");
    ffm_plume *P = new ffm_plume();
    P->ctx = ctx; P->nx = nx; P->ny = ny; P->nz = nz; P->h = h; P->dt = dt; P->rdt = 1.0 / dt;
    P->tight = getenv("FFM_PLUME_TIGHT") != nullptr;
    if (const char *e = getenv("FFM_PLUME_SOLVERS")) P->stecklerSolvers = e[0] == 's';
    const long nOwn = (long)nx * ny * nz;
    const int cnt[6] = {ny * nz, ny * nz, nx * nz, nx * nz, nx * ny, nx * ny};
    int gOff[7]; gOff[0] = 0;
    for (int s6 = 0; s6 < 6; s6++) gOff[s6 + 1] = gOff[s6] + (nbrRank[s6] >= 0 ? cnt[s6] : 0);
    const long nGhost = gOff[6], N = nOwn + nGhost;
    P->N = (int)N; P->nOwn = (int)nOwn;
    auto cellOf = [&](int i, int j, int k) { return i + nx * (j + ny * k); };
    auto ghostOf = [&](int side, int i, int j, int k) -> int {
        switch (side >> 1) {
        case 0: return (int)nOwn + gOff[side] + j + ny * k;
        case 1: return (int)nOwn + gOff[side] + i + nx * k;
        default: return (int)nOwn + gOff[side] + i + nx * j;
        }
    };
// ... 25 lines not shown
      int *l2p = l2.data(), *u2p = u2.data(); signed char *fd2p = fd2.data(), *sg2p = sg2.data();
      ffm_parallel_for(F, [=](long a, long b) { for (long f = a; f < b; f++) { l2p[f] = o2n[lp[f2p[f]]]; u2p[f] = o2n[up_[f2p[f]]]; fd2p[f] = fdp[f2p[f]]; sg2p[f] = sgp[f2p[f]]; } }); }
    delete tmS_; tmS_ = nullptr;
    {
        std::vector<int> hintNew(nOwn);
        for (long c = 0; c < nOwn; c++) hintNew[c] = hint[c2[c]];
        FfmStageTimer tm_("plume_create: ldu_create");
        FFM_TRY(ffm_ldu_create_hint(ctx, (int)nOwn, (int)nGhost, F, l2.data(), u2.data(), hintNew.data(), &P->A));
    }
    if (!P->A->identity) { ffm_set_error("plume: renumbered mesh is not native"); return FFM_ERR_ADDR; }
    if (nGhost == 0) { P->hL2 = l2; P->hU2 = u2; P->hOldToNew = oldToNew; P->hFd2 = fd2; }
    FFM_TRY(ffm_ldu_set_global_cells(P->A, (long)gx * gy * gz));
    P->nNat = P->A->upTotal;
    tmS_ = new FfmStageTimer("plume_create: geometry + patches");
    ffm_hvec<double> V = ffm_hvec_fill<double>(N, h * h * h), C(3 * N), Sf = ffm_hvec_fill<double>(3 * (size_t)F, 0.0), magSf = ffm_hvec_fill<double>(F, h * h),
                     wgt = ffm_hvec_fill<double>(F, 0.5), del = ffm_hvec_fill<double>(F, 1.0 / h), Cfy(F);
    {
        double *Cp = C.data(), *Sfp = Sf.data(), *Cfyp = Cfy.data(); const int *c2p = c2.data(), *l2p = l2.data(); const signed char *fd2p = fd2.data(), *sg2p = sg2.data();
        const int lo0 = lo[0], lo1 = lo[1], lo2 = lo[2]; int gO[7]; for (int q = 0; q < 7; q++) gO[q] = gOff[q];
        ffm_parallel_for(N, [=](long a, long b) { for (long cn = a; cn < b; cn++) {
            const int co = c2p[cn];
            int i, j, k;
            if (co < nOwn) { i = co % nx; j = (co / nx) % ny; k = co / (nx * ny); }
            else {
                int side = 0; while (co - nOwn >= gO[side + 1]) side++;
                const int r = co - (int)nOwn - gO[side];
                switch (side >> 1) {
                case 0: j = r % ny; k = r / ny; i = (side & 1) ? nx : -1; break;
                case 1: i = r % nx; k = r / nx; j = (side & 1) ? ny : -1; break;
                default: i = r % nx; j = r / nx; k = (side & 1) ? nz : -1; break;
                }
            }
            Cp[cn] = (lo0 + i + 0.5) * h; Cp[N + cn] = (lo1 + j + 0.5) * h; Cp[2 * N + cn] = (lo2 + k + 0.5) * h;
        } });
        ffm_parallel_for(F, [=](long a, long b) { for (long f = a; f < b; f++) { Sfp[(size_t)fd2p[f] * F + f] = sg2p[f] * h * h; Cfyp[f] = Cp[N + l2p[f]] + (fd2p[f] == 1 ? sg2p[f] * 0.5 * h : 0.0); } });
    }
    {
        std::vector<int> ranks, sc, rc, cells;
        for (int s6 = 0; s6 < 6; s6++) if (nbrRank[s6] >= 0) {
            ranks.push_back(nbrRank[s6]); sc.push_back(cnt[s6]); rc.push_back(cnt[s6]);
            const int d = s6 >> 1, pos = (s6 & 1) ? (d == 0 ? nx : d == 1 ? ny : nz) - 1 : 0;
            if (d == 0) for (int k = 0; k < nz; k++) for (int j = 0; j < ny; j++) cells.push_back(oldToNew[cellOf(pos, j, k)]);
            else if (d == 1) for (int k = 0; k < nz; k++) for (int i = 0; i < nx; i++) cells.push_back(oldToNew[cellOf(i, pos, k)]);
            else for (int j = 0; j < ny; j++) for (int i = 0; i < nx; i++) cells.push_back(oldToNew[cellOf(i, j, pos)]);
        }
        if (!ranks.empty()) FFM_TRY(ffm_ldu_set_ghost_exchange(P->A, (int)ranks.size(), ranks.data(), sc.data(), cells.data(), rc.data()));
    }
    const double Lx = gx * h, Lz = gz * h, hwx = std::min(0.5, Lx / 4), hwz = std::min(0.5, Lz / 4);
    std::vector<int> pc[4]; std::vector<double> pS[4][3];
    auto addFace = [&](int patch, int cOld, double sx, double sy, double sz) {
        pc[patch].push_back(oldToNew[cOld]); pS[patch][0].push_back(sx); pS[patch][1].push_back(sy); pS[patch][2].push_back(sz);
    };
    if (nbrRank[2] < 0) for (int k = 0; k < nz; k++) for (int i = 0; i < nx; i++) {
        const bool in = std::fabs((lo[0] + i + 0.5) * h - Lx / 2) < hwx && std::fabs((lo[2] + k + 0.5) * h - Lz / 2) < hwz;
        addFace(in ? P_INLET : P_FLOOR, cellOf(i, 0, k), 0, -h * h, 0);
    }
    if (nbrRank[3] < 0) for (int k = 0; k < nz; k++) for (int i = 0; i < nx; i++) addFace(P_TOP, cellOf(i, ny - 1, k), 0, h * h, 0);
    if (nbrRank[0] < 0) for (int k = 0; k < nz; k++) for (int j = 0; j < ny; j++) addFace(P_SIDES, cellOf(0, j, k), -h * h, 0, 0);
    if (nbrRank[1] < 0) for (int k = 0; k < nz; k++) for (int j = 0; j < ny; j++) addFace(P_SIDES, cellOf(nx - 1, j, k), h * h, 0, 0);
    if (nbrRank[4] < 0) for (int j = 0; j < ny; j++) for (int i = 0; i < nx; i++) addFace(P_SIDES, cellOf(i, j, 0), 0, 0, -h * h);
    if (nbrRank[5] < 0) for (int j = 0; j < ny; j++) for (int i = 0; i < nx; i++) addFace(P_SIDES, cellOf(i, j, nz - 1), 0, 0, h * h);
    int sizes[4]; const int *fcs[4]; const double *pSf[4]; const double *pDel[4];
    std::vector<double> pSflat[4], pD[4];
    int Btot = 0;
    for (int p = 0; p < 4; p++) {
        sizes[p] = (int)pc[p].size(); fcs[p] = pc[p].data(); Btot += sizes[p];
        for (int d = 0; d < 3; d++) pSflat[p].insert(pSflat[p].end(), pS[p][d].begin(), pS[p][d].end());
        pD[p].assign(sizes[p], 2.0 / h); pSf[p] = pSflat[p].data(); pDel[p] = pD[p].data();
    }
    P->B = Btot;
    delete tmS_; tmS_ = nullptr;
    { FfmStageTimer tm_("plume_create: mesh_create"); FFM_TRY(ffm_mesh_create(P->A, V.data(), C.data(), Sf.data(), magSf.data(), wgt.data(), del.data(), 4, sizes, fcs, pSf, pDel, &P->mesh)); }
    tmS_ = new FfmStageTimer("plume_create: face centres");
    {
        ffm_hvec<double> Cf(3 * (size_t)F);
        { double *Cfp = Cf.data(); const double *Cp = C.data(); const int *l2p = l2.data(); const signed char *fd2p = fd2.data(), *sg2p = sg2.data();
          ffm_parallel_for(F, [=](long a, long b) { for (long f = a; f < b; f++) for (int d = 0; d < 3; d++) Cfp[(size_t)d * F + f] = Cp[(size_t)d * N + l2p[f]] + (fd2p[f] == d ? sg2p[f] * 0.5 * h : 0.0); }); }
        FFM_TRY(ffm_mesh_set_face_centres(P->mesh, Cf.data()));
    }
    delete tmS_; tmS_ = new FfmStageTimer("plume_create: fields + tables");
    const int ny_glob = gy;
    const int B = Btot; const long nNat = P->nNat;
    auto NN = [&]() { return dalloc(P, N); };
    for (int i = 0; i < NSP; i++) { P->Y[i] = dfill(P, N, Y_AMB[i]); P->Y0[i] = NN(); }
    P->T = dfill(P, N, TREF); P->hs = NN(); P->hs0 = NN();
    for (int c = 0; c < 3; c++) { P->U[c] = NN(); P->U0[c] = NN(); }
    P->p = dfill(P, N, PREF); P->p0 = NN(); P->p_rgh = NN(); P->p_rgh0 = NN(); P->psi = NN(); P->psi0 = NN();
    P->rho = NN(); P->rho0 = NN(); P->K = NN(); P->K0 = NN(); P->dpdt = NN(); P->ph_rgh = NN();
    P->phi = dalloc(P, nNat); P->phi0 = dalloc(P, nNat); P->phib = dalloc(P, B); P->phib0 = dalloc(P, B); P->ph_rgh_b = dalloc(P, B);
    {
        const double ghRef = -9.81 * (ny_glob * h);
        std::vector<double> gh(N), ghf(std::max<long>(nNat, 1), 0.0);
        for (long c = 0; c < N; c++) gh[c] = -9.81 * C[N + c] - ghRef;
        for (int f = 0; f < F; f++) ghf[P->A->h_callerToNative[f]] = -9.81 * Cfy[f] - ghRef;
        P->gh = dupload(P, gh); P->ghf = dupload(P, ghf);
    }
    std::vector<double> kind(B), fsU[3], rU[3], fsS(B), fsH(B), rY[NSP], rH(B);
    for (int c = 0; c < 3; c++) { fsU[c].assign(B, 0.0); rU[c].assign(B, 0.0); }
    for (int i = 0; i < NSP; i++) rY[i].assign(B, 0.0);
    int k0 = 0;
    for (int p = 0; p < 4; p++) for (int q = 0; q < sizes[p]; q++, k0++) {
        kind[k0] = p;
        for (int c = 0; c < 3; c++) {
            if (p == P_INLET) { fsU[c][k0] = 1.0; rU[c][k0] = (c == 1) ? U_IN : 0.0; }
            else if (p == P_FLOOR) fsU[c][k0] = 1.0;
            else fsU[c][k0] = (pS[p][c][q] != 0.0) ? 0.0 : -1.0;
        }
        fsH[k0] = (p == P_INLET || p == P_FLOOR) ? 1.0 : -1.0;
        if (p == P_INLET) { fsS[k0] = 1.0; rH[k0] = CP * (T_IN - TREF); for (int i = 0; i < NSP; i++) rY[i][k0] = Y_IN[i]; }
        else if (p == P_FLOOR) { fsS[k0] = 0.0; }
        else { fsS[k0] = -1.0; rH[k0] = 0.0; for (int i = 0; i < NSP; i++) rY[i][k0] = Y_AMB[i]; }
    }
    P->kind_d = dupload(P, kind);
    for (int c = 0; c < 3; c++) { P->fStaticU[c] = dupload(P, fsU[c]); P->refU[c] = dupload(P, rU[c]); P->fU[c] = dalloc(P, B); }
    P->fStaticS = dupload(P, fsS); P->fS = dalloc(P, B); P->refH = dupload(P, rH);
    P->fStaticH = dupload(P, fsH); P->fH = dalloc(P, B);
    for (int i = 0; i < NSP; i++) P->refY[i] = dupload(P, rY[i]);
    P->fP = dalloc(P, B); P->refP = dalloc(P, B); P->gradP = dalloc(P, B); P->zeroB = dalloc(P, B);
    P->oneB = dupload(P, std::vector<double>(std::max(B, 1), 1.0));
    P->diag = NN(); P->upper = dalloc(P, nNat); P->lower = dalloc(P, nNat); P->dWork = NN(); P->sWork = NN();
    P->Udiag = NN(); P->Uupper = dalloc(P, nNat); P->Ulower = dalloc(P, nNat);
    for (int c = 0; c < 3; c++) { P->src[c] = NN(); P->ic[c] = dalloc(P, B); P->bc[c] = dalloc(P, B); P->Usrc[c] = NN(); P->Uic[c] = dalloc(P, B); P->Ubc[c] = dalloc(P, B); }
    for (auto &w : P->wN) w = NN();
    for (auto &w : P->wF) w = dalloc(P, nNat);
    P->ddtCorrF = dalloc(P, nNat);
    for (auto &w : P->wB) w = dalloc(P, B);
    P->fused = getenv("FFM_PLUME_UNFUSED") == nullptr;
    P->mvSelection = getenv("FFM_PLUME_INDEPENDENT_LIMITERS") == nullptr;
    if (P->mvSelection) { P->wMv = dalloc(P, nNat); if (P->fused) for (int j = 0; j < 2; j++) for (int d = 0; d < 3; d++) P->mvG[j][d] = NN(); }
    for (int j = 0; j < 4; j++) {
        for (int d = 0; d < 3; d++) P->gM[j][d] = P->fused ? NN() : nullptr;
        P->spD[j] = P->fused ? NN() : nullptr; P->spS[j] = P->fused ? NN() : nullptr; P->suM[j] = P->fused ? NN() : nullptr;
        const bool ownOffDiag = P->fused && (j == 0 || !P->mvSelection);
        P->spU[j] = ownOffDiag ? dalloc(P, nNat) : nullptr; P->spL[j] = ownOffDiag ? dalloc(P, nNat) : nullptr; P->spB[j] = (P->fused || P->mvSelection) ? dalloc(P, B) : nullptr;
    }
    for (double *p : P->pool) if (!p) { ffm_set_error("plume: out of device memory"); return FFM_ERR_HIP; }
    PL_HIP(hipDeviceSynchronize());
    delete tmS_; tmS_ = new FfmStageTimer("plume_create: hydrostatic init");
    standin_thermo(P);
    mul(P, P->rho, P->psi, P->p, N);
    FFM_TRY(hydrostatic_init(P));
    PL_HIP(hipStreamSynchronize(ctx->stream));
    delete tmS_; tmS_ = nullptr;
    if (const char *e = getenv("FFM_PLUME_RADIATION")) { if (atoi(e) > 0) FFM_TRY(ffm_plume_set_radiation(P, atoi(e), 2, 4, nullptr, nullptr)); }
    *out = P;
    return FFM_OK;
}

extern "C" int ffm_plume_destroy(ffm_plume *P)
{
    if (!P) return FFM_OK;
    hipStreamSynchronize(P->ctx->stream);
    for (double *p : P->pool) hipFree(p);
    for (int a = 0; a < 3; a++) { hipFree(P->radCm[a]); hipFree(P->radFm[a]); }
    ffm_mesh_destroy(P->mesh); ffm_ldu_destroy(P->A);
    delete P;
    return FFM_OK;
}

extern "C" int ffm_plume_set_tight(ffm_plume *P, int on) { if (!P) return FFM_ERR_ARG; P->tight = on != 0; return FFM_OK; }
extern "C" int ffm_plume_set_radiation(ffm_plume *P, int solverFreq, int nPhi, int nTheta, const double *dAve, const double *omega)
{
    if (!P || solverFreq < 0 || nPhi < 1 || nTheta < 1 || ((dAve == nullptr) != (omega == nullptr))) return FFM_ERR_ARG;
    PL_HIP(hipSetDevice(P->ctx->device));
    const int nRay = 4 * nPhi * nTheta;
    P->rayD.assign(3 * (size_t)nRay, 0.0); P->rayOmega.assign(nRay, 0.0);
    if (dAve) { std::copy(dAve, dAve + 3 * nRay, P->rayD.begin()); std::copy(omega, omega + nRay, P->rayOmega.begin()); }
    else {
        const double dPhi = M_PI / (2.0 * nPhi), dTheta = M_PI / nTheta; int i = 0;
        for (int n = 1; n <= nTheta; n++) for (int mm = 1; mm <= 4 * nPhi; mm++, i++) {
            const double theta = (2.0 * n - 1.0) * dTheta / 2.0, phi = (2.0 * mm - 1.0) * dPhi / 2.0;
            const double a = sin(0.5 * dPhi) * (dTheta - cos(2.0 * theta) * sin(dTheta));
            P->rayOmega[i] = 2.0 * sin(theta) * sin(dTheta / 2.0) * dPhi;
            P->rayD[3 * i] = sin(phi) * a; P->rayD[3 * i + 1] = cos(phi) * a; P->rayD[3 * i + 2] = 0.5 * dPhi * sin(2.0 * theta) * sin(dTheta);
        }
    }
    if ((int)P->I.size() < nRay) {
        for (int i = (int)P->I.size(); i < nRay; i++) { double *p = dalloc(P, P->N); if (!p) return FFM_ERR_HIP; P->I.push_back(p); }
    }
    if (!P->G) {
        P->G = dalloc(P, P->N); P->radSrc = dalloc(P, P->N); P->radJ = dalloc(P, P->nNat); P->radW = dalloc(P, P->nNat);
        P->radJb = dalloc(P, P->B); P->radF = dalloc(P, P->B); P->radRef = dalloc(P, P->B);
        if (!P->G || !P->radSrc || !P->radJ || !P->radW || !P->radJb || !P->radF || !P->radRef) return FFM_ERR_HIP;
    }
    if (!P->hL2.empty() && !P->radOrdered) {
        const int N = P->N, F = P->F, nx = P->nx, ny = P->ny, nz = P->nz; const long nNat = P->nNat;
        std::vector<int> ownerStart(N + 1, 0);
        for (int f = 0; f < F; f++) ownerStart[P->hL2[f] + 1]++;
        for (int c = 0; c < N; c++) ownerStart[c + 1] += ownerStart[c];
        const std::vector<int> &c2n = P->A->h_callerToNative;
        for (int a = 0; a < 3; a++) {
            std::vector<int> cm(N), fm(std::max<long>(nNat, 1));
            for (long e = 0; e < nNat; e++) fm[e] = (int)e;
            for (int c = 0; c < N; c++) {
                const int o = P->newToOld[c]; int i = o % nx, j = (o / nx) % ny, k = o / (nx * ny);
                if (a == 0) i = nx - 1 - i; else if (a == 1) j = ny - 1 - j; else k = nz - 1 - k;
                cm[c] = P->hOldToNew[i + nx * (j + ny * k)];
            }
            for (int f = 0; f < F; f++) {
                int o = cm[P->hL2[f]], n = cm[P->hU2[f]]; bool swap = false;
                if (o > n) { std::swap(o, n); swap = true; }
                int fp = -1;
                for (int g = ownerStart[o]; g < ownerStart[o + 1]; g++) if (P->hU2[g] == n) { fp = g; break; }
                if (fp < 0) { ffm_set_error("plume radiation: the flipped image of a face is not a face"); return FFM_ERR_ADDR; }
                fm[c2n[f]] = swap ? ~c2n[fp] : c2n[fp];
            }
            PL_HIP(hipMalloc((void **)&P->radCm[a], sizeof(int) * N)); PL_HIP(hipMalloc((void **)&P->radFm[a], sizeof(int) * std::max<long>(nNat, 1)));
            FFM_TRY(ffm_h2d(P->ctx, P->radCm[a], cm.data(), sizeof(int) * N));
            FFM_TRY(ffm_h2d(P->ctx, P->radFm[a], fm.data(), sizeof(int) * std::max<long>(nNat, 1)));
        }
        P->radDB = dalloc(P, N); P->radSB = dalloc(P, N); P->radPsiB = dalloc(P, N); P->radUB = dalloc(P, nNat); P->radLB = dalloc(P, nNat);
        if (!P->radDB || !P->radSB || !P->radPsiB || !P->radUB || !P->radLB) return FFM_ERR_HIP;
        P->radOrdered = true;
    }
    P->radFreq = solverFreq;
    return FFM_OK;
}

extern "C" int ffm_plume_set_radiation_model(ffm_plume *P, double absorption, double Ehrr1, double Ehrr2)
{
    if (!P || absorption < 0 || Ehrr1 < 0 || Ehrr2 < 0) return FFM_ERR_ARG;
    PL_HIP(hipSetDevice(P->ctx->device));
    if (!P->radE) { P->radE = dalloc(P, P->N); P->radShSu = dalloc(P, P->N); P->radShSp = dalloc(P, P->N); }
    if (!P->radE || !P->radShSu || !P->radShSp) return FFM_ERR_HIP;
    P->radA = absorption; P->Ehrr1 = Ehrr1; P->Ehrr2 = Ehrr2; P->radCoupled = true;
    return FFM_OK;
}
extern "C" int ffm_plume_set_initial_state(ffm_plume *P, const double *const *Y, const double *h, const double *Yamb, const double *Yin, double hAmb)
{
    if (!P || !Y || !h || !Yamb || !Yin) return FFM_ERR_ARG;
    if (P->stepNo != 0 || P->N != P->nOwn) { ffm_set_error("plume: the start state can be set on a single block before the first step only"); return FFM_ERR_ARG; }
    PL_HIP(hipSetDevice(P->ctx->device));
    const int N = P->N, B = P->B;
    std::vector<double> v(N);
    auto up = [&](double *dst, const double *nat) -> int {
        for (int c = 0; c < N; c++) v[c] = nat[P->newToOld[c]];
        return ffm_memcpy_h2d(P->ctx, dst, v.data(), sizeof(double) * N);
    };
    for (int i = 0; i < NSP; i++) FFM_TRY(up(P->Y[i], Y[i]));
    FFM_TRY(up(P->hs, h));
    P->hAmb = hAmb;
    const double *kind = P->kind_d; double *rH = P->refH;
    for (int i = 0; i < NSP; i++) {
        double *r = P->refY[i]; const double a = Yamb[i], b = Yin[i];
        forN(P, B, [=] __device__(long k) { r[k] = kind[k] < 0.5 ? b : kind[k] > 1.5 ? a : 0.0; });
    }
    forN(P, B, [=] __device__(long k) { rH[k] = kind[k] < 0.5 ? CP * (T_IN - TREF) : kind[k] > 1.5 ? hAmb : 0.0; });
    double *p = P->p, *ph = P->ph_rgh;
    forN(P, N, [=] __device__(long c) { p[c] = PREF; ph[c] = 0.0; });
    P->log.clear();
    standin_thermo(P);
    mul(P, P->rho, P->psi, P->p, N);
    FFM_TRY(hydrostatic_init(P));
    PL_HIP(hipStreamSynchronize(P->ctx->stream));
    return FFM_OK;
}

extern "C" int ffm_plume_override_mv_weights(ffm_plume *P, const double *w)
{
    if (!P || !w) return FFM_ERR_ARG;
    if (!P->mvSelection || P->N != P->nOwn) { ffm_set_error("plume: weights can be handed in on a single block with the common limiter only"); return FFM_ERR_ARG; }
    PL_HIP(hipSetDevice(P->ctx->device));
    std::vector<double> v(std::max<long>(P->nNat, 1), 0.0);
    const std::vector<int> &c2n = P->A->h_callerToNative;
    for (int f = 0; f < P->F; f++) v[c2n[f]] = w[P->faceNewToOld[f]];
    FFM_TRY(ffm_memcpy_h2d(P->ctx, P->wMv, v.data(), sizeof(double) * P->nNat));
    P->mvOverride = true;
    return FFM_OK;
}
extern "C" int ffm_plume_set_solvers(ffm_plume *P, int stecklerSelection) { if (!P) return FFM_ERR_ARG; P->stecklerSolvers = stecklerSelection != 0; return FFM_OK; }
extern "C" int ffm_plume_ncells(const ffm_plume *P) { return P ? P->nOwn : FFM_ERR_ARG; }
extern "C" int ffm_plume_nfaces(const ffm_plume *P) { return P ? P->F : FFM_ERR_ARG; }

extern "C" int ffm_plume_get_field(ffm_plume *P, const char *name, double *out)
{
    if (!P || !name || !out) return FFM_ERR_ARG;
    const std::string n(name);
    const double *src = nullptr;
    if (n == "rho") src = P->rho; else if (n == "p") src = P->p; else if (n == "p_rgh") src = P->p_rgh; else if (n == "T") src = P->T;
    else if (n == "h") src = P->hs; else if (n == "K") src = P->K; else if (n == "Ux") src = P->U[0]; else if (n == "Uy") src = P->U[1];
    else if (n == "Uz") src = P->U[2]; else if (n == "psi") src = P->psi; else if (n == "ph_rgh") src = P->ph_rgh;
    else if (n == "G") src = P->G; else if (n == "ShSu") src = P->radShSu; else if (n == "ShSp") src = P->radShSp; else if (n == "radE") src = P->radE;
    else if (n.size() > 1 && n[0] == 'I' && isdigit((unsigned char)n[1])) { const int i = atoi(n.c_str() + 1); if (i < (int)P->I.size()) src = P->I[i]; }
    else for (int i = 0; i < NSP; i++) if (n == SPN[i]) src = P->Y[i];
    if (!src) { ffm_set_error("unknown field %s", name); return FFM_ERR_ARG; }
    std::vector<double> v(P->N);
    PL_HIP(hipStreamSynchronize(P->ctx->stream));
    FFM_TRY(ffm_d2h(P->ctx, v.data(), src, sizeof(double) * P->N));
    for (int c = 0; c < P->nOwn; c++) out[P->newToOld[c]] = v[c];
    return FFM_OK;
}

extern "C" long ffm_plume_get_raw(ffm_plume *P, const char *name, double *out, long cap)
{
    if (!P || !name || !out) return FFM_ERR_ARG;
    if (P->N != P->nOwn) { ffm_set_error("ffm_plume_get_raw: single block only"); return FFM_ERR_ARG; }
    const std::string n(name);
    const long N = P->N, F = P->F, B = P->B;
    auto cellF = [&](const double *src) -> long { if (cap < N) return FFM_ERR_ARG; return ffm_d2h(P->ctx, out, src, sizeof(double) * N) == FFM_OK ? N : FFM_ERR_HIP; };
    auto bndF = [&](const double *src) -> long { if (cap < B) return FFM_ERR_ARG; return ffm_d2h(P->ctx, out, src, sizeof(double) * B) == FFM_OK ? B : FFM_ERR_HIP; };
    auto faceF = [&](const double *src) -> long {
        if (cap < F) return FFM_ERR_ARG;
        std::vector<double> v(std::max<long>(P->nNat, 1));
        if (ffm_d2h(P->ctx, v.data(), src, sizeof(double) * P->nNat) != FFM_OK) return FFM_ERR_HIP;
        const std::vector<int> &c2n = P->A->h_callerToNative;
        for (long f = 0; f < F; f++) out[f] = v[c2n[f]];
        return F;
    };
    if (n == "rho") return cellF(P->rho); if (n == "p") return cellF(P->p); if (n == "p_rgh") return cellF(P->p_rgh); if (n == "h") return cellF(P->hs);
    if (n == "K") return cellF(P->K); if (n == "dpdt") return cellF(P->dpdt); if (n == "gh") return cellF(P->gh); if (n == "T") return cellF(P->T);
    if (n == "Ux") return cellF(P->U[0]); if (n == "Uy") return cellF(P->U[1]); if (n == "Uz") return cellF(P->U[2]);
    for (int i = 0; i < NSP; i++) if (n == SPN[i]) return cellF(P->Y[i]);
    if (n == "phi") return faceF(P->phi); if (n == "ghf") return faceF(P->ghf);
    if (n == "phib") return bndF(P->phib); if (n == "ph_rgh_b") return bndF(P->ph_rgh_b); if (n == "kind") return bndF(P->kind_d);
    if (n == "fStaticS") return bndF(P->fStaticS); if (n == "fStaticH") return bndF(P->fStaticH); if (n == "refH") return bndF(P->refH);
    for (int c = 0; c < 3; c++) { if (n == std::string("fStaticU") + char('0' + c)) return bndF(P->fStaticU[c]); if (n == std::string("refU") + char('0' + c)) return bndF(P->refU[c]); }
    for (int i = 0; i < NSP; i++) if (n == std::string("refY") + char('0' + i)) return bndF(P->refY[i]);
    if (n == "ghfB") {
        if (cap < B) return FFM_ERR_ARG;
        std::vector<double> gh(N), sy(B), mg(B); std::vector<int> bc(B);
        if (ffm_d2h(P->ctx, gh.data(), P->gh, sizeof(double) * N) != FFM_OK || ffm_d2h(P->ctx, sy.data(), ffm_mesh_geom(P->mesh, 7), sizeof(double) * B) != FFM_OK ||
            ffm_d2h(P->ctx, mg.data(), ffm_mesh_geom(P->mesh, 4), sizeof(double) * B) != FFM_OK || ffm_d2h(P->ctx, bc.data(), ffm_mesh_bcells(P->mesh), sizeof(int) * B) != FFM_OK) return FFM_ERR_HIP;
        for (long k = 0; k < B; k++) out[k] = gh[bc[k]] + (-9.81) * (0.5 * P->h * (sy[k] / mg[k]));
        return B;
    }
    ffm_set_error("ffm_plume_get_raw: unknown array %s", name);
    return FFM_ERR_ARG;
}

extern "C" int ffm_plume_nsolves(const ffm_plume *P) { return P ? (int)P->log.size() : FFM_ERR_ARG; }
extern "C" int ffm_plume_get_solve(const ffm_plume *P, int i, char *name16, ffm_perf *perf)
{
    if (!P || i < 0 || i >= (int)P->log.size()) return FFM_ERR_ARG;
    if (name16) memcpy(name16, P->log[i].name, 16);
    if (perf) *perf = P->log[i].perf;
    return FFM_OK;
}
extern "C" ffm_ldu *ffm_plume_ldu(ffm_plume *P) { return P ? P->A : nullptr; }
extern "C" ffm_mesh *ffm_plume_mesh(ffm_plume *P) { return P ? P->mesh : nullptr; }
```

### include/ffm.h

```cpp
#ifndef FFM_H
#define FFM_H

#include <stddef.h>
#include <stdint.h>

#ifdef __cplusplus
extern "C" {
#endif

typedef struct ffm_ctx ffm_ctx;
typedef struct ffm_ldu ffm_ldu;

typedef enum ffm_status {
    FFM_OK = 0,
    FFM_ERR_ARG = -1,
    FFM_ERR_ADDR = -2,
    FFM_ERR_HIP = -3,
    FFM_ERR_NODEVICE = -4,
    FFM_ERR_UNSUPPORTED = -5,
    FFM_ERR_COMM = -6
} ffm_status;

typedef enum ffm_solver {
    FFM_PCG = 0, FFM_PBICGSTAB = 1, FFM_PBICG = 2, FFM_DIAGONAL = 3, FFM_SMOOTH = 4,
// ... 110 lines not shown

int ffm_bench_spmv(ffm_ldu *ldu, const double *x_d, double *y_d, int reps,
                   double *avg_ms);
int ffm_bench_precond(ffm_ldu *ldu, int precond, const double *r_d, double *w_d, int reps, double *avg_ms);

typedef struct ffm_mesh ffm_mesh;
int ffm_mesh_create(ffm_ldu *ldu, const double *V, const double *C,
                    const double *Sf, const double *magSf, const double *weights,
                    const double *deltaCoeffs, int nPatches, const int *patchSizes,
                    const int *const *faceCells, const double *const *patchSf,
                    const double *const *patchDeltaCoeffs, ffm_mesh **out);
int ffm_mesh_set_face_centres(ffm_mesh *mesh, const double *Cf);
int ffm_mesh_set_nonorth_correction(ffm_mesh *mesh, const double *corrVec);
int ffm_mesh_destroy(ffm_mesh *mesh);
int ffm_mesh_nboundary(const ffm_mesh *mesh);
const double *ffm_mesh_geometry_d(const ffm_mesh *mesh, int which);
int ffm_mesh_nnative(const ffm_mesh *mesh);
int ffm_faces_to_native(const ffm_mesh *mesh, const double *lduOrder, double *native_d);
int ffm_faces_from_native(const ffm_mesh *mesh, const double *native_d, double *lduOrder);

int ffm_fvc_interpolate(ffm_mesh *m, const double *w_f, const double *vf, double *out_f);
int ffm_fvc_snGrad(ffm_mesh *m, const double *vf, double *out_f);
int ffm_fvc_snGrad_b(ffm_mesh *m, const double *vf, const double *vb, double *out_b);
int ffm_fvc_flux(ffm_mesh *m, const double *vx, const double *vy, const double *vz, double *out_f);
int ffm_fvc_surface_integrate(ffm_mesh *m, const double *ssf_f, const double *ssf_b, double *out);
int ffm_fvc_surface_sum(ffm_mesh *m, const double *ssf_f, const double *ssf_b, double *out);
int ffm_fvc_grad(ffm_mesh *m, const double *vf, const double *vb, double *gx, double *gy, double *gz);
int ffm_fvc_reconstruct(ffm_mesh *m, const double *ssf_f, const double *ssf_b, double *ox, double *oy, double *oz);
int ffm_fvc_snGrad_correction(ffm_mesh *m, const double *gx, const double *gy, const double *gz, double *out_f);
int ffm_fv_limited_weights(ffm_mesh *m, int scheme, double k, double lo, double hi,
                           const double *phi_f, const double *vf, const double *gx,
                           const double *gy, const double *gz, double *out_w_f);
int ffm_fv_limited_limiter(ffm_mesh *m, int scheme, double k, double lo, double hi, const double *phi_f, const double *vf,
                           const double *gx, const double *gy, const double *gz, double *lim_f, int accumulateMin);
int ffm_fv_weights_from_limiter(ffm_mesh *m, const double *phi_f, const double *lim_f, double *out_w);
int ffm_fv_multivariate_weights(ffm_mesh *m, int nf, const int *schemes, double k, double lo, double hi, const double *phi_f,
                                const double *const *vf, const double *const *gx, const double *const *gy, const double *const *gz,
                                double *out_w);
int ffm_fv_multivariate_weights_tiled(ffm_mesh *m, int nf, const int *schemes, double k, double lo, double hi, const double *phi_f,
                                      const double *const *vf, const double *const *vb, double *out_w);

int ffm_fv_filtered_linear2V_weights(ffm_mesh *m, double k, double l, const double *phi_f, const double *const *U,
                                     const double *const *gx, const double *const *gy, const double *const *gz, double *out_w_f);

int ffm_fv_lust_correction(ffm_mesh *m, const double *phi_f, const double *gx, const double *gy,
                           const double *gz, double *out_f);
int ffm_fv_linear_upwind_correction(ffm_mesh *m, const double *phi_f, const double *gx, const double *gy,
                                    const double *gz, double *out_f);

int ffm_fvm_transport(ffm_mesh *m, double rDeltaT, const double *rho,
                      const double *phi_f, const double *w_f, const double *gamma_f,
                      int laplacianSign, double *diag, double *upper, double *lower);
int ffm_fvm_boundary_coeffs(ffm_mesh *m, const double *phi_b, const double *gamma_b,
                            int laplacianSign, const double *f, const double *ref,
                            const double *refGrad, double *internalCoeffs, double *boundaryCoeffs);
int ffm_bc_values(ffm_mesh *m, const double *f, const double *ref, const double *refGrad,
                  const double *vf, double *out_b);
int ffm_fvm_add_boundary(ffm_mesh *m, const double *internalCoeffs, const double *boundaryCoeffs,
                         const double *diag, const double *source, const double *su,
                         double *diagOut, double *sourceOut);
int ffm_fvm_relax(ffm_mesh *m, double alpha, int nCmpt, const double *upper, const double *lower,
                  const double *ic0, const double *ic1, const double *ic2, double *diag,
                  const double *psiPrev0, const double *psiPrev1, const double *psiPrev2,
                  double *source0, double *source1, double *source2);
int ffm_fvm_A(ffm_mesh *m, int nCmpt, const double *diag, const double *ic0, const double *ic1,
              const double *ic2, double *out);
int ffm_fvm_H(ffm_mesh *m, int nCmpt, int cmpt, const double *upper, const double *lower,
              const double *source, const double *ic0, const double *ic1, const double *ic2,
              const double *bcCmpt, const double *psi, double *out);
int ffm_fvm_HbyA3(ffm_mesh *m, const double *upper, const double *lower, const double *const *source,
                  const double *const *internalCoeffs, const double *const *boundaryCoeffs, const double *const *psi,
                  const double *rAU, double *const *out);
int ffm_fvm_pressure_eqn(ffm_mesh *m, double rDeltaT, const double *psi, const double *psi0, const double *p0,
                         const double *rho, const double *rho0, const double *gh, double pRef, const double *gamma_f,
                         const double *phiHbyA_f, const double *phiHbyA_b, const double *internalCoeffs,
                         const double *boundaryCoeffs, double *upper, double *lower, double *diagOut, double *sourceOut);
int ffm_pc_phig(ffm_mesh *m, const double *rhorAUf, const double *ghf, const double *rho, double *phig);
int ffm_pc_phiHbyA(ffm_mesh *m, const double *rho, const double *vx, const double *vy, const double *vz, const double *rhorAUf,
                   const double *ddtCorr, const double *phig, double *phiHbyA);
int ffm_pc_flux(ffm_mesh *m, const double *upper, const double *lower, const double *psi, const double *phiHbyA, const double *phig,
                const double *rhorAUf, double *flux_f, double *phi_f, double *t_f);
int ffm_ue_buoyancy_flux(ffm_mesh *m, const double *ghf, const double *rho, const double *p_rgh, double *t_f);
int ffm_fvc_flux_rho(ffm_mesh *m, const double *rho, const double *vx, const double *vy, const double *vz, double *out_f);
int ffm_fvm_flux(ffm_mesh *m, const double *upper, const double *lower, const double *internalCoeffs,
                 const double *boundaryCoeffs, const double *psi, double *out_f, double *out_b);

int ffm_fvc_grad_multi(ffm_mesh *m, int nf, const double *const *vf, const double *const *vb, double *const *gx,
                       double *const *gy, double *const *gz);
int ffm_fvm_scalar_transport_multi(ffm_mesh *m, int nf, int scheme, double k, double lo, double hi, double rDeltaT,
                                   const double *rho, const double *rho0, const double *phi_f, const double *phi_b,
                                   const double *gamma_f, const double *gamma_b,
                                   const double *const *vf, const double *const *gx, const double *const *gy,
                                   const double *const *gz, const double *const *vf0, const double *const *f,
                                   const double *const *ref, const double *const *refGrad, const double *const *su,
                                   const double *const *su2, const double *const *sp,
                                   const double *const *expl3, double *const *diag, double *const *upper,
                                   double *const *lower, double *const *source);
int ffm_fvm_scalar_transport_multi_w(ffm_mesh *m, int nf, const double *w_f, double rDeltaT, const double *rho, const double *rho0,
                                     const double *phi_f, const double *phi_b, const double *gamma_f, const double *gamma_b,
                                     const double *const *vf0, const double *const *f, const double *const *ref,
                                     const double *const *refGrad, const double *const *su, const double *const *su2,
                                     const double *const *sp, const double *const *expl3, double *const *diag,
                                     double *const *upper, double *const *lower, double *const *source);
int ffm_fvm_lust_source3(ffm_mesh *m, double rDeltaT, const double *phi_f, const double *rho0, const double *const *U0,
                         const double *const *gx, const double *const *gy, const double *const *gz, double *const *source);

int ffm_fvdom_wall_coeffs_d(ffm_mesh *mesh, int nRay, int ray, const double *d3, const double *dAve3, double sigma, const double *Iw_b,
                            const double *emissivity_b, const double *T_b, double *qin_all, double *qem_all, double *qr_all,
                            double *valueFraction_b, double *refValue_b);
int ffm_fvdom_sum_rays_d(ffm_mesh *mesh, int nRay, const double *all, double *out_b);

typedef struct ffm_plume ffm_plume;
int ffm_plume_create(ffm_ctx *ctx, int nx, int ny, int nz, double h, double deltaT, ffm_plume **out);
int ffm_plume_create_block(ffm_ctx *ctx, int gx, int gy, int gz, const int *lo, const int *hi,
                           const int *nbrRank, double h, double deltaT, ffm_plume **out);
int ffm_plume_destroy(ffm_plume *p);
int ffm_plume_step(ffm_plume *p);
int ffm_plume_set_tight(ffm_plume *p, int on);
int ffm_plume_set_solvers(ffm_plume *plume, int stecklerSelection);
int ffm_plume_set_radiation(ffm_plume *plume, int solverFreq, int nPhi, int nTheta, const double *dAve, const double *omega);
int ffm_plume_set_radiation_model(ffm_plume *plume, double absorption, double Ehrr1, double Ehrr2);
int ffm_plume_set_initial_state(ffm_plume *plume, const double *const *Y, const double *h, const double *Yamb, const double *Yin, double hAmb);
int ffm_plume_override_mv_weights(ffm_plume *plume, const double *w);
int ffm_plume_ncells(const ffm_plume *p);
int ffm_plume_nfaces(const ffm_plume *p);
int ffm_plume_get_field(ffm_plume *p, const char *name, double *out);
int ffm_plume_nsolves(const ffm_plume *p);
int ffm_plume_get_solve(const ffm_plume *p, int i, char *name16, ffm_perf *perf);
long ffm_plume_get_raw(ffm_plume *p, const char *name, double *out, long cap);
ffm_ldu *ffm_plume_ldu(ffm_plume *p);
ffm_mesh *ffm_plume_mesh(ffm_plume *p);

typedef struct ffm_pyro ffm_pyro;
int ffm_pyro_create(ffm_ctx *ctx, int nCol, int nLay, double thickness, double faceArea, double T0, double Yvirgin0, ffm_pyro **out);
int ffm_pyro_set_solids(ffm_pyro *p, const double *virgin , const double *charred);
int ffm_pyro_set_reaction(ffm_pyro *p, double A, double Ta, double Tcrit, double n);
int ffm_pyro_step(ffm_pyro *p, double deltaT, const double *qSurf_d, int backFixed, double Tback);
int ffm_pyro_get(ffm_pyro *p, const char *name, double *out);
const double *ffm_pyro_surface_T_d(const ffm_pyro *p);
const double *ffm_pyro_phiGas_d(const ffm_pyro *p);
int ffm_pyro_couple_d(ffm_pyro *p, const int *map_d, const double *TgasCell_d, const double *kappaDelta_d, const double *qin_d,
                      double emissivity, double absorptivity, const double *rho_b_d, const double *magSf_d,
                      const double *nfx_d, const double *nfy_d, const double *nfz_d, double hocSolid, double qFuel,
                      double *refT_d, double *Ux_d, double *Uy_d, double *Uz_d);
const double *ffm_pyro_qSurf_d(const ffm_pyro *p);
int ffm_pyro_set_model(ffm_pyro *p, int reactingOneDim21, int harmonicAlpha, int harmonicKappa);
int ffm_pyro_set_back(ffm_pyro *p, int mode, double h, double Tinf);
int ffm_pyro_set_surface_radiation(ffm_pyro *p, double absorptivityVirgin, double emissivityVirgin, double absorptivityChar, double emissivityChar);
int ffm_pyro_evolve_d(ffm_pyro *p, double deltaT, const int *map_d, const double *TgasCell_d, const double *kappaDelta_d, const double *qin_d,
                      double emissivity, double absorptivity);
int ffm_pyro_gas_side_d(ffm_pyro *p, const int *map_d, const double *rho_b_d, const double *magSf_d, const double *nfx_d, const double *nfy_d,
                        const double *nfz_d, double hocSolid, double qFuel, double *refT_d, double *Ux_d, double *Uy_d, double *Uz_d,
                        double *emissivity_d);
int ffm_pyro_diff_no(ffm_pyro *p, double deltaT, double *out);
int ffm_pyro_set_incident_radiation(ffm_pyro *p, double uniformQr, const double *Qr_d);
int ffm_pyro_set_qr_source(ffm_pyro *p, int on, const double *qr0_d);
int ffm_pyro_step_incident(ffm_pyro *p, double deltaT);
int ffm_pyro_run_incident(ffm_pyro *p, double deltaT, int nSteps, int sampleEvery, double *hist_d, long histCap);
int ffm_pyro_destroy(ffm_pyro *p);

typedef struct ffm_thermo ffm_thermo;
int ffm_thermo_create(ffm_ctx *ctx, int nSpecies, const double *W, const double *Tlow, const double *Thigh, const double *Tcommon,
                      const double *highCpCoeffs, const double *lowCpCoeffs, const double *As, const double *Ts, double RR,
                      ffm_thermo **out);
int ffm_thermo_correct_d(ffm_thermo *th, long n, const double *const *Y_d, const double *he_d, const double *p_d, double *T_d,
                         double *psi_d, double *mu_d, double *alpha_d);
int ffm_thermo_he_d(ffm_thermo *th, long n, const double *const *Y_d, const double *T_d, double *he_d);
int ffm_thermo_properties_d(ffm_thermo *th, long n, const double *const *Y_d, const double *T_d, double *psi_d, double *mu_d,
                            double *alpha_d);
int ffm_thermo_Cp_d(ffm_thermo *th, long n, const double *const *Y_d, const double *T_d, double *Cp_d);
int ffm_thermo_destroy(ffm_thermo *th);
int ffm_edc_correct_d(ffm_ctx *ctx, long n, const double *rho_d, const double *k_d, const double *delta_d, const double *alpha_d,
                      const double *Yfuel_d, const double *YO2_d, double s, double deltaT, double Ce, double C_EDC, double C_Diff,
                      double C_Stiff, double qFuel, double *wFuel_d, double *Qdot_d);
int ffm_les_keqn_nut_d(ffm_ctx *ctx, long n, double Ck, double Prt, const double *k_d, const double *delta_d, const double *rho_d,
                       double *nut_d, double *alphat_d);

int ffm_fvc_div_dev2T_gradU(ffm_mesh *m, const double *const *g, const double *gamma, const double *gamma_b,
                            const double *const *U, const double *const *U_b, double *const *out);
int ffm_les_keqn_G(ffm_mesh *m, const double *const *g, const double *nut, double *G);

int ffm_ctx_set_gamg_forward(ffm_ctx *ctx, int forward);
int ffm_ctx_gamg_forward(const ffm_ctx *ctx);
typedef struct ffm_gamg ffm_gamg;
int ffm_gamg_face_area_pair_weights(int nFaces, const double *Sf, double *weights);
int ffm_gamg_create(ffm_ctx *ctx, ffm_ldu *finest, int nCells, int nFaces, const int *lowerAddr, const int *upperAddr,
// ... 67 lines not shown
```

Measured before the change: 2.854 outer-iterations/s.

## Fuse rhoEqn, rAU, divPhiK and ddtCorr into single kernels; drop unused buffers

Adds fused kernels for the density equation, rAU/rhorAU computation, the div(phi*K)+ddt(rho K)+dpdt energy terms, and the ddt flux correction, each replacing a chain of separate launches and intermediate face arrays. Also adds a scaled-Su variant of the given-weight scalar transport kernel, clamps the inert species inside the fused path, and stops allocating phi0/phib0 and the inert Y0. The aim is to cut kernel launches and HBM round-trips of face and cell temporaries. The cost is extra code paths with fallbacks and a changed reset path in set_initial_state.

```diff
diff --git a/firefoam-dev_amd/csrc/ffm_fused.hip b/firefoam-dev_amd/csrc/ffm_fused.hip
--- a/firefoam-dev_amd/csrc/ffm_fused.hip
+++ b/firefoam-dev_amd/csrc/ffm_fused.hip
@@ -72,6 +72,7 @@
     const double *vf[FUSE_MAX], *gx[FUSE_MAX], *gy[FUSE_MAX], *gz[FUSE_MAX], *vf0[FUSE_MAX];
     const double *f[FUSE_MAX], *ref[FUSE_MAX], *refGrad[FUSE_MAX];
     const double *su[FUSE_MAX];
+    double suFactor[FUSE_MAX];
     const double *su2[FUSE_MAX], *sp[FUSE_MAX];
     const double *expl[FUSE_MAX][3];
     double *diag[FUSE_MAX], *upper[FUSE_MAX], *lower[FUSE_MAX], *src[FUSE_MAX];
@@ -83,7 +84,7 @@
     int nOffDiag;
 };
 
-template <int W, int NF, bool GIVENW = false>
+template <int W, int NF, bool GIVENW = false, bool SUSCALED = false>
 __global__ __launch_bounds__(256, ((NF > 1 && !GIVENW) ? 4 : 1)) void k_scalar_eqns(MeshView q, ScalarEqns a)
 {
     CELL_SCHED(ci, q) {
@@ -143,7 +144,7 @@
             d = d - dLap;
             double sc = a.rdt * rho0c * a.vf0[i][c] * V;
             if (a.expl[i][0]) sc = ((sc - V * a.expl[i][0][c]) - V * a.expl[i][1][c]) - V * a.expl[i][2][c];
-            if (a.su[i]) sc = sc + V * a.su[i][c];
+            if (a.su[i]) sc = sc + V * (SUSCALED ? a.suFactor[i] * a.su[i][c] : a.su[i][c]);
             if (a.sp[i]) d = d + V * a.sp[i][c];
             if (a.su2[i]) sc = sc + V * a.su2[i][c];
             if (j >= 0) for (int t = q.bcStart[j]; t < q.bcStart[j + 1]; t++) {
@@ -421,6 +422,53 @@
     }
 }
 
+struct DivPhiK {
+    const double *K, *Kb, *gx, *gy, *gz, *phi, *phib, *rho, *rho0, *K0, *dpdt, *Cx, *Cy, *Cz;
+    double *divK, *ddtK, *ndpdt;
+    double rdt, twoByk, lo, hi;
+    int scheme;
+};
+template <int W>
+__global__ __launch_bounds__(256) void k_div_phiK(MeshView q, DivPhiK a)
+{
+    CELL_SCHED(ci, q) {
+        const int c = (int)ci;
+        RowEnt<W> L, U; load_lower<W>(q.v, c, L); load_upper<W>(q.v, c, U);
+        const double cx = a.Cx[c], cy = a.Cy[c], cz = a.Cz[c];
+        const double P = a.K[c], gxc = a.gx[c], gyc = a.gy[c], gzc = a.gz[c];
+        double fl[W], fu[W], wl[W], wu[W], kl[W], ku[W], dlx[W], dly[W], dlz[W], dux[W], duy[W], duz[W], glx[W], gly[W], glz[W], gux[W], guy[W], guz[W];
+#pragma unroll
+        for (int s = 0; s < W; s++) {
+            const int el = L.f[s], eu = U.f[s], o = L.nb[s], n = U.nb[s];
+            fl[s] = a.phi[el]; fu[s] = a.phi[eu]; wl[s] = q.w[el]; wu[s] = q.w[eu];
+            kl[s] = a.K[o]; ku[s] = a.K[n];
+            dlx[s] = cx - a.Cx[o]; dly[s] = cy - a.Cy[o]; dlz[s] = cz - a.Cz[o];
+            dux[s] = a.Cx[n] - cx; duy[s] = a.Cy[n] - cy; duz[s] = a.Cz[n] - cz;
+            const bool upl = fl[s] > 0, upu = fu[s] > 0;
+            glx[s] = upl ? a.gx[o] : gxc; gly[s] = upl ? a.gy[o] : gyc; glz[s] = upl ? a.gz[o] : gzc;
+            gux[s] = upu ? gxc : a.gx[n]; guy[s] = upu ? gyc : a.gy[n]; guz[s] = upu ? gzc : a.gz[n];
+        }
+        double acc = 0.0;
+#pragma unroll
+        for (int s = 0; s < W; s++) if (L.on[s]) {
+            const double w = limited_weight(a.scheme, a.twoByk, a.lo, a.hi, fl[s], wl[s], kl[s], P, dlx[s], dly[s], dlz[s], glx[s], gly[s], glz[s]);
+            const double Kf = w * kl[s] + (1.0 - w) * P;
+            acc = acc - fl[s] * Kf;
+        }
+#pragma unroll
+        for (int s = 0; s < W; s++) if (U.on[s]) {
+            const double w = limited_weight(a.scheme, a.twoByk, a.lo, a.hi, fu[s], wu[s], P, ku[s], dux[s], duy[s], duz[s], gux[s], guy[s], guz[s]);
+            const double Kf = w * P + (1.0 - w) * ku[s];
+            acc += fu[s] * Kf;
+        }
+        const int j = q.cellB[c];
+        if (j >= 0) for (int t = q.bcStart[j]; t < q.bcStart[j + 1]; t++) { const int k = q.bcItem[t]; acc += a.phib[k] * a.Kb[k]; }
+        a.divK[c] = acc / q.V[c];
+        a.ddtK[c] = a.rdt * (a.rho[c] * P - a.rho0[c] * a.K0[c]);
+        a.ndpdt[c] = -a.dpdt[c];
+    }
+}
+
 
 extern "C" int ffm_fvc_grad_multi(ffm_mesh *m, int nf, const double *const *vf, const double *const *vb, double *const *gx,
                                   double *const *gy, double *const *gz)
@@ -458,7 +506,7 @@
                        (m->B && (!f[q] || !ref[q] || !refGrad[q])))) return FFM_ERR_ARG;
         a.vf[i] = vf[q]; a.gx[i] = gx[q]; a.gy[i] = gy[q]; a.gz[i] = gz[q]; a.vf0[i] = vf0[q];
         a.f[i] = f[q]; a.ref[i] = ref[q]; a.refGrad[i] = refGrad[q];
-        a.su[i] = su ? su[q] : nullptr;
+        a.su[i] = su ? su[q] : nullptr; a.suFactor[i] = 1.0;
         a.su2[i] = su2 ? su2[q] : nullptr; a.sp[i] = sp ? sp[q] : nullptr;
         for (int e = 0; e < 3; e++) a.expl[i][e] = expl3 ? expl3[3 * q + e] : nullptr;
         if (a.expl[i][0] && (!a.expl[i][1] || !a.expl[i][2])) return FFM_ERR_ARG;
@@ -492,14 +540,15 @@
     return FFM_OK;
 }
 
-extern "C" int ffm_fvm_scalar_transport_multi_w(ffm_mesh *m, int nf, const double *w_f, double rDeltaT, const double *rho, const double *rho0,
-                                                const double *phi_f, const double *phi_b, const double *gamma_f, const double *gamma_b,
-                                                const double *const *vf0, const double *const *f, const double *const *ref,
-                                                const double *const *refGrad, const double *const *su, const double *const *su2,
-                                                const double *const *sp, const double *const *expl3, double *const *diag,
-                                                double *const *upper, double *const *lower, double *const *source)
-{
-    CHECK_M(m);
+extern "C" int ffm_fvm_scalar_transport_multi_ws(ffm_mesh *m, int nf, const double *w_f, double rDeltaT, const double *rho, const double *rho0,
+                                                 const double *phi_f, const double *phi_b, const double *gamma_f, const double *gamma_b,
+                                                 const double *const *vf0, const double *const *f, const double *const *ref,
+                                                 const double *const *refGrad, const double *const *su, const double *suFactor,
+                                                 const double *const *su2, const double *const *sp, const double *const *expl3,
+                                                 double *const *diag, double *const *upper, double *const *lower, double *const *source)
+{
+    CHECK_M(m);
+    if (suFactor && !su) return FFM_ERR_ARG;
     if (nf < 1 || nf > FUSE_MAX || !w_f || !rho || !rho0 || !phi_f || !gamma_f || (m->B && (!phi_b || !gamma_b))) return FFM_ERR_ARG;
     if (!vf0 || !f || !ref || !refGrad || !diag || !upper || !lower || !source) return FFM_ERR_ARG;
     ScalarEqns a;
@@ -508,7 +557,7 @@
         if (i < nf && (!vf0[q] || !diag[q] || !source[q] || (m->B && (!f[q] || !ref[q] || !refGrad[q])))) return FFM_ERR_ARG;
         a.vf[i] = a.gx[i] = a.gy[i] = a.gz[i] = nullptr; a.vf0[i] = vf0[q];
         a.f[i] = f[q]; a.ref[i] = ref[q]; a.refGrad[i] = refGrad[q];
-        a.su[i] = su ? su[q] : nullptr;
+        a.su[i] = su ? su[q] : nullptr; a.suFactor[i] = suFactor ? suFactor[q] : 1.0;
         a.su2[i] = su2 ? su2[q] : nullptr; a.sp[i] = sp ? sp[q] : nullptr;
         for (int e = 0; e < 3; e++) a.expl[i][e] = expl3 ? expl3[3 * q + e] : nullptr;
         if (a.expl[i][0] && (!a.expl[i][1] || !a.expl[i][2])) return FFM_ERR_ARG;
@@ -519,11 +568,22 @@
     a.rdt = rDeltaT; a.twoByk = 2.0; a.lo = 0.0; a.hi = 1.0; a.scheme = 0; a.wGiven = w_f;
     a.nOffDiag = 0;
     for (int i = 0; i < nf; i++) { if (upper[i] && lower[i]) { if (a.nOffDiag != i) return FFM_ERR_ARG; a.nOffDiag = i + 1; } else if ((upper[i] == nullptr) != (lower[i] == nullptr)) return FFM_ERR_ARG; }
-#define SEW(NF) FFM_DISPATCH_W(m->A->maxW, LAUNCH_CELLS((k_scalar_eqns<W, NF, true>), mview(m), a))
+#define SEW(NF) do { if (suFactor) FFM_DISPATCH_W(m->A->maxW, LAUNCH_CELLS((k_scalar_eqns<W, NF, true, true>), mview(m), a)); \
+                     else FFM_DISPATCH_W(m->A->maxW, LAUNCH_CELLS((k_scalar_eqns<W, NF, true, false>), mview(m), a)); } while (0)
     switch (nf) { case 1: SEW(1); break; case 2: SEW(2); break; case 3: SEW(3); break; default: SEW(4); break; }
 #undef SEW
     FFM_HIP(hipGetLastError());
     return FFM_OK;
+}
+extern "C" int ffm_fvm_scalar_transport_multi_w(ffm_mesh *m, int nf, const double *w_f, double rDeltaT, const double *rho, const double *rho0,
+                                                const double *phi_f, const double *phi_b, const double *gamma_f, const double *gamma_b,
+                                                const double *const *vf0, const double *const *f, const double *const *ref,
+                                                const double *const *refGrad, const double *const *su, const double *const *su2,
+                                                const double *const *sp, const double *const *expl3, double *const *diag,
+                                                double *const *upper, double *const *lower, double *const *source)
+{
+    return ffm_fvm_scalar_transport_multi_ws(m, nf, w_f, rDeltaT, rho, rho0, phi_f, phi_b, gamma_f, gamma_b, vf0, f, ref, refGrad, su, nullptr, su2, sp,
+                                             expl3, diag, upper, lower, source);
 }
 
 extern "C" int ffm_fvm_lust_source3(ffm_mesh *m, double rDeltaT, const double *phi_f, const double *rho0, const double *const *U0,
@@ -540,6 +600,26 @@
     a.phi = phi_f; a.rho0 = rho0; a.Cx = m->C[0]; a.Cy = m->C[1]; a.Cz = m->C[2]; a.Cfx = m->Cf[0]; a.Cfy = m->Cf[1]; a.Cfz = m->Cf[2];
     a.rdt = rDeltaT;
     FFM_DISPATCH_W(m->A->maxW, LAUNCH_CELLS(k_lust_source<W>, mview(m), a));
+    FFM_HIP(hipGetLastError());
+    return FFM_OK;
+}
+
+extern "C" int ffm_fvc_div_phiK_terms(ffm_mesh *m, int scheme, double k, double lo, double hi, double rDeltaT, const double *phi_f,
+                                      const double *phi_b, const double *K, const double *K_b, const double *gx, const double *gy,
+                                      const double *gz, const double *rho, const double *rho0, const double *K0, const double *dpdt,
+                                      double *divK, double *ddtK, double *negDpdt)
+{
+    CHECK_M(m);
+    if ((scheme != 2 && scheme != 3) || !phi_f || !K || !gx || !gy || !gz || !rho || !rho0 || !K0 || !dpdt || !divK || !ddtK || !negDpdt) return FFM_ERR_ARG;
+    if (m->B && (!phi_b || !K_b)) return FFM_ERR_ARG;
+    DivPhiK a;
+    a.K = K; a.Kb = K_b; a.gx = gx; a.gy = gy; a.gz = gz; a.phi = phi_f; a.phib = phi_b; a.rho = rho; a.rho0 = rho0; a.K0 = K0; a.dpdt = dpdt;
+    a.Cx = m->C[0]; a.Cy = m->C[1]; a.Cz = m->C[2]; a.divK = divK; a.ddtK = ddtK; a.ndpdt = negDpdt;
+    a.rdt = rDeltaT; a.twoByk = 2.0 / std::max(k, 1e-15); a.lo = lo; a.hi = hi; a.scheme = scheme;
+    if (m->A->maxW > 8) return FFM_ERR_UNSUPPORTED;
+    if (m->A->maxW <= 3) LAUNCH_CELLS(k_div_phiK<3>, mview(m), a);
+    else if (m->A->maxW <= 4) LAUNCH_CELLS(k_div_phiK<4>, mview(m), a);
+    else LAUNCH_CELLS(k_div_phiK<8>, mview(m), a);
     FFM_HIP(hipGetLastError());
     return FFM_OK;
 }
@@ -608,6 +688,30 @@
             out[e] = (w * Px + (1.0 - w) * (rN * vx[nb])) * q.Sfx[e] + (w * Py + (1.0 - w) * (rN * vy[nb])) * q.Sfy[e] + (w * Pz + (1.0 - w) * (rN * vz[nb])) * q.Sfz[e];
         }
     }
+}
+__global__ __launch_bounds__(256) void k_ddt_corr(MeshView q, double rdt, const double *__restrict__ rho, const double *__restrict__ vx,
+                                                  const double *__restrict__ vy, const double *__restrict__ vz, const double *__restrict__ phi0,
+                                                  double *__restrict__ out)
+{
+    CELL_SCHED(ci, q) {
+        const int c = (int)ci; const double rP = rho[c]; const double Px = rP * vx[c], Py = rP * vy[c], Pz = rP * vz[c];
+        FOR_OWN_FACES(q, c, e, nb) {
+            const double w = q.w[e], rN = rho[nb];
+            const double fl0 = (w * Px + (1.0 - w) * (rN * vx[nb])) * q.Sfx[e] + (w * Py + (1.0 - w) * (rN * vy[nb])) * q.Sfy[e] + (w * Pz + (1.0 - w) * (rN * vz[nb])) * q.Sfz[e];
+            const double p0 = phi0[e], phiCorr = p0 - fl0;
+            const double coeff = 1.0 - fmin(fabs(phiCorr) / (fabs(p0) + 1e-15), 1.0);
+            out[e] = coeff * rdt * phiCorr;
+        }
+    }
+}
+extern "C" int ffm_fvc_ddt_corr(ffm_mesh *m, double rDeltaT, const double *rho0, const double *vx0, const double *vy0, const double *vz0,
+                                const double *phi0_f, double *out_f)
+{
+    CHECK_M(m);
+    if (!rho0 || !vx0 || !vy0 || !vz0 || !phi0_f || !out_f) return FFM_ERR_ARG;
+    LAUNCH_CELLS(k_ddt_corr, mview(m), rDeltaT, rho0, vx0, vy0, vz0, phi0_f, out_f);
+    FFM_HIP(hipGetLastError());
+    return FFM_OK;
 }
 extern "C" int ffm_fvc_flux_rho(ffm_mesh *m, const double *rho, const double *vx, const double *vy, const double *vz, double *out_f)
 {
diff --git a/firefoam-dev_amd/csrc/ffm_fv.hip b/firefoam-dev_amd/csrc/ffm_fv.hip
--- a/firefoam-dev_amd/csrc/ffm_fv.hip
+++ b/firefoam-dev_amd/csrc/ffm_fv.hip
@@ -333,6 +333,28 @@
 }
 
 template <int W>
+__global__ void k_rho_eqn(MeshView q, double rdt, const double *__restrict__ ssf, const double *__restrict__ ssb, const double *__restrict__ rho0,
+                          double *__restrict__ rho)
+{
+    CELL_SCHED(ci, q) {
+        const int c = (int)ci;
+        RowEnt<W> L, U; load_lower<W>(q.v, c, L); load_upper<W>(q.v, c, U);
+        double a[W], b[W];
+#pragma unroll
+        for (int s = 0; s < W; s++) { a[s] = ssf[L.f[s]]; b[s] = ssf[U.f[s]]; }
+        double acc = 0.0;
+#pragma unroll
+        for (int s = 0; s < W; s++) if (L.on[s]) acc = acc - a[s];
+#pragma unroll
+        for (int s = 0; s < W; s++) if (U.on[s]) acc += b[s];
+        const int j = q.cellB[c];
+        if (j >= 0 && ssb) for (int t = q.bcStart[j]; t < q.bcStart[j + 1]; t++) acc += ssb[q.bcItem[t]];
+        const double V = q.V[c], div = acc / V;
+        rho[c] = (rdt * rho0[c] * V - V * div) / (rdt * V);
+    }
+}
+
+template <int W>
 __global__ void k_grad(MeshView q, const double *__restrict__ vf, const double *__restrict__ vb, double *__restrict__ gx,
                        double *__restrict__ gy, double *__restrict__ gz)
 {
@@ -487,6 +509,24 @@
     }
 }
 
+__global__ void k_matrix_rAU(MeshView q, int nc, const double *__restrict__ diag, const double *__restrict__ ic0, const double *__restrict__ ic1,
+                             const double *__restrict__ ic2, const double *__restrict__ psi, const double *__restrict__ p,
+                             double *__restrict__ rho, double *__restrict__ rAU, double *__restrict__ rhorAU)
+{
+    CELL_SCHED(ci, q) {
+        const int c = (int)ci;
+        double d = diag[c];
+        const int j = q.cellB[c];
+        if (j >= 0) for (int t = q.bcStart[j]; t < q.bcStart[j + 1]; t++) {
+            const int k = q.bcItem[t];
+            d += (nc == 3) ? (ic0[k] + ic1[k] + ic2[k]) / 3.0 : ic0[k];
+        }
+        const double A = d / q.V[c];
+        const double r = psi[c] * p[c], ra = 1.0 / A;
+        rho[c] = r; rAU[c] = ra; rhorAU[c] = r * ra;
+    }
+}
+
 template <int W>
 __global__ void k_matrix_H(MeshView q, int nc, const double *__restrict__ upper, const double *__restrict__ lower,
                            const double *__restrict__ src, const double *__restrict__ icC, const double *__restrict__ ic0,
@@ -542,6 +582,17 @@
 { CHECK_M(m); LAUNCH_CELLS(k_flux, mview(m), vx, vy, vz, out_f); DONE(); }
 extern "C" int ffm_fvc_surface_integrate(ffm_mesh *m, const double *ssf, const double *ssb, double *out)
 { CHECK_M(m); FFM_DISPATCH_W(m->A->maxW, LAUNCH_CELLS((k_face_sum<0, W>), mview(m), ssf, ssb, out)); DONE(); }
+extern "C" int ffm_fvc_rho_eqn(ffm_mesh *m, double rDeltaT, const double *phi_f, const double *phi_b, const double *rho0, double *rho)
+{
+    CHECK_M(m);
+    if (!phi_f || !rho0 || !rho || rho == rho0) return FFM_ERR_ARG;
+    if (m->A->maxW > 16) return FFM_ERR_UNSUPPORTED;
+    if (m->A->maxW <= 3) LAUNCH_CELLS(k_rho_eqn<3>, mview(m), rDeltaT, phi_f, phi_b, rho0, rho);
+    else if (m->A->maxW <= 4) LAUNCH_CELLS(k_rho_eqn<4>, mview(m), rDeltaT, phi_f, phi_b, rho0, rho);
+    else if (m->A->maxW <= 8) LAUNCH_CELLS(k_rho_eqn<8>, mview(m), rDeltaT, phi_f, phi_b, rho0, rho);
+    else LAUNCH_CELLS(k_rho_eqn<16>, mview(m), rDeltaT, phi_f, phi_b, rho0, rho);
+    DONE();
+}
 extern "C" int ffm_fvc_surface_sum(ffm_mesh *m, const double *ssf, const double *ssb, double *out)
 { CHECK_M(m); FFM_DISPATCH_W(m->A->maxW, LAUNCH_CELLS((k_face_sum<1, W>), mview(m), ssf, ssb, out)); DONE(); }
 extern "C" int ffm_fvc_grad(ffm_mesh *m, const double *vf, const double *vb, double *gx, double *gy, double *gz)
@@ -673,6 +724,13 @@
 { CHECK_M(m); LAUNCH_CELLS(k_add_boundary, mview(m), ic, bc, diag, src, su, diagOut, srcOut); DONE(); }
 extern "C" int ffm_fvm_A(ffm_mesh *m, int nc, const double *diag, const double *ic0, const double *ic1, const double *ic2, double *out)
 { CHECK_M(m); if (nc != 1 && nc != 3) return FFM_ERR_ARG; LAUNCH_CELLS(k_matrix_A, mview(m), nc, diag, ic0, ic1, ic2, out); DONE(); }
+extern "C" int ffm_fvm_rAU(ffm_mesh *m, int nc, const double *diag, const double *ic0, const double *ic1, const double *ic2, const double *psi,
+                           const double *p, double *rho, double *rAU, double *rhorAU)
+{
+    CHECK_M(m);
+    if ((nc != 1 && nc != 3) || !diag || !psi || !p || !rho || !rAU || !rhorAU) return FFM_ERR_ARG;
+    LAUNCH_CELLS(k_matrix_rAU, mview(m), nc, diag, ic0, ic1, ic2, psi, p, rho, rAU, rhorAU); DONE();
+}
 extern "C" int ffm_fvm_H(ffm_mesh *m, int nc, int cmpt, const double *upper, const double *lower, const double *src,
                          const double *ic0, const double *ic1, const double *ic2, const double *bcC, const double *psi, double *out)
 {
diff --git a/firefoam-dev_amd/csrc/ffm_plume.hip b/firefoam-dev_amd/csrc/ffm_plume.hip
--- a/firefoam-dev_amd/csrc/ffm_plume.hip
+++ b/firefoam-dev_amd/csrc/ffm_plume.hip
@@ -87,7 +87,7 @@
     double hAmb = 0.0;
     std::vector<double *> pool;
     double *Y[NSP], *Y0[NSP], *T, *hs, *hs0, *U[3], *U0[3], *p, *p0, *p_rgh, *p_rgh0, *psi, *psi0, *rho, *rho0, *K, *K0, *dpdt;
-    double *phi, *phi0, *phib, *phib0, *gh, *ghf, *ph_rgh, *ph_rgh_b;
+    double *phi, *phib, *gh, *ghf, *ph_rgh, *ph_rgh_b;
     double *kind_d;
     double *fU[3], *refU[3], *fS, *refS, *fP, *refP, *gradP, *zeroB, *oneB;
     double *fStaticU[3], *fStaticS, *fStaticH, *fH, *refY[NSP], *refH;
@@ -223,6 +223,11 @@
 
 static int rho_eqn(ffm_plume *P)
 {
+    if (P->fused) {
+        const int rc = ffm_fvc_rho_eqn(P->mesh, P->rdt, P->phi, P->phib, P->rho0, P->rho);
+        if (rc == FFM_OK) return HX(P, P->rho);
+        if (rc != FFM_ERR_UNSUPPORTED) return rc;
+    }
     double *div = P->wN[0];
     FFM_TRY(ffm_fvc_surface_integrate(P->mesh, P->phi, P->phib, div));
     const double *V = ffm_mesh_geom(P->mesh, 0), *rho0 = P->rho0; double *rho = P->rho; const double rdt = P->rdt;
@@ -377,10 +382,10 @@
     const double *Sx = ffm_mesh_geom(m, 9), *Sy = ffm_mesh_geom(m, 10), *Sz = ffm_mesh_geom(m, 11), *wlin = ffm_mesh_geom(m, 3);
     double *rho = P->rho; const double *psi = P->psi; double *p = P->p;
     double *rAU = P->wN[0], *rhorAU = P->wN[1], *HbyA[3] = {P->wN[2], P->wN[3], P->wN[4]};
+    if (P->fused && P->N == P->nOwn) {
+        FFM_TRY(ffm_fvm_rAU(m, 3, P->Udiag, P->Uic[0], P->Uic[1], P->Uic[2], psi, p, rho, rAU, rhorAU));
+    } else {
     FFM_TRY(ffm_fvm_A(m, 3, P->Udiag, P->Uic[0], P->Uic[1], P->Uic[2], rAU));
-    if (P->fused && P->N == P->nOwn) {
-        forN(P, N, [=] __device__(long i) { const double r = psi[i] * p[i], a = 1.0 / rAU[i]; rho[i] = r; rAU[i] = a; rhorAU[i] = r * a; });
-    } else {
     mul(P, rho, psi, p, N);
     forN(P, P->nOwn, [=] __device__(long i) { rAU[i] = 1.0 / rAU[i]; });
     FFM_TRY(HX(P, rAU));
@@ -432,19 +437,19 @@
     {
         double *dc = P->ddtCorrF;
         if (!P->ddtCorrValid) {
-            double *fl0 = P->wF[4];
-            if (P->fused) FFM_TRY(ffm_fvc_flux_rho(m, P->rho0, P->U0[0], P->U0[1], P->U0[2], fl0));
+            const double *phi0 = P->phi;
+            if (P->fused) FFM_TRY(ffm_fvc_ddt_corr(m, rdt, P->rho0, P->U0[0], P->U0[1], P->U0[2], phi0, dc));
             else {
+                double *fl0 = P->wF[4];
                 double *rU0[3] = {P->wN[8], P->wN[9], P->wN[10]};
                 for (int c = 0; c < 3; c++) mul(P, rU0[c], P->rho0, P->U0[c], N);
                 FFM_TRY(ffm_fvc_flux(m, rU0[0], rU0[1], rU0[2], fl0));
+                forN(P, nNat, [=] __device__(long e) {
+                    const double phiCorr = phi0[e] - fl0[e];
+                    const double coeff = 1.0 - fmin(fabs(phiCorr) / (fabs(phi0[e]) + 1e-15), 1.0);
+                    dc[e] = coeff * rdt * phiCorr;
+                });
             }
-            const double *phi0 = P->phi0;
-            forN(P, nNat, [=] __device__(long e) {
-                const double phiCorr = phi0[e] - fl0[e];
-                const double coeff = 1.0 - fmin(fabs(phiCorr) / (fabs(phi0[e]) + 1e-15), 1.0);
-                dc[e] = coeff * rdt * phiCorr;
-            });
             P->ddtCorrValid = true;
         }
         if (P->fused) FFM_TRY(ffm_pc_phiHbyA(m, rho, HbyA[0], HbyA[1], HbyA[2], rhorAUf, dc, phig, phiHbyA));
@@ -526,10 +531,10 @@
     const double *V = ffm_mesh_geom(m, 0), *magSf = ffm_mesh_geom(m, 1);
     P->log.clear();
     P->ddtCorrValid = false;
-    dcopy(P, P->rho0, P->rho, N); dcopy(P, P->hs0, P->hs, N); dcopy(P, P->K0, P->K, N); dcopy(P, P->p0, P->p, N);
-    dcopy(P, P->psi0, P->psi, N); dcopy(P, P->p_rgh0, P->p_rgh, N); dcopy(P, P->phi0, P->phi, nNat); dcopy(P, P->phib0, P->phib, B);
+    std::swap(P->rho0, P->rho); std::swap(P->K0, P->K); std::swap(P->psi0, P->psi);
+    dcopy(P, P->hs0, P->hs, N); dcopy(P, P->p0, P->p, N); dcopy(P, P->p_rgh0, P->p_rgh, N);
     for (int c = 0; c < 3; c++) dcopy(P, P->U0[c], P->U[c], N);
-    for (int i = 0; i < NSP; i++) dcopy(P, P->Y0[i], P->Y[i], N);
+    for (int i = 0; i < NSP; i++) if (i != INERT) dcopy(P, P->Y0[i], P->Y[i], N);
     FFM_TRY(rho_eqn(P));
     FFM_TRY(update_bcs(P));
     double *Ub[3] = {P->wB[1], P->wB[2], P->wB[3]};
@@ -596,7 +601,8 @@
     double *wFuel = P->wN[8], *Qdot = P->wN[9], *Yt = P->wN[10], *su = P->wN[11];
     {
         const double *rho = P->rho, *fuel = P->Y[2], *o2 = P->Y[0];
-        forN(P, N, [=] __device__(long i) { const double w = rho[i] * fmin(fuel[i], o2[i] / S_O2) / TAU; wFuel[i] = w; Qdot[i] = w * HC; Yt[i] = 0.0; });
+        if (P->fused) forN(P, N, [=] __device__(long i) { const double w = rho[i] * fmin(fuel[i], o2[i] / S_O2) / TAU; wFuel[i] = w; Qdot[i] = w * HC; });
+        else forN(P, N, [=] __device__(long i) { const double w = rho[i] * fmin(fuel[i], o2[i] / S_O2) / TAU; wFuel[i] = w; Qdot[i] = w * HC; Yt[i] = 0.0; });
     }
     if (P->mvSelection && P->mvOverride) P->mvOverride = false;
     else if (P->mvSelection) {
@@ -648,18 +654,19 @@
         int sp[NSP - 1], ns = 0;
         for (int i = 0; i < NSP; i++) if (i != INERT) sp[ns++] = i;
         const double *vf[4], *vb[4], *vf0[4], *fq[4], *rq[4], *gq[4], *suq[4], *cgx[4], *cgy[4], *cgz[4];
-        double *ggx[4], *ggy[4], *ggz[4];
+        double *ggx[4], *ggy[4], *ggz[4], nuq[4];
         for (int j = 0; j < ns; j++) {
-            const int i = sp[j]; const double nu = NU[i]; double *sj = P->suM[j];
-            forN(P, N, [=] __device__(long c) { sj[c] = nu * wFuel[c]; });
+            const int i = sp[j]; const double nu = NU[i]; const double *sj = wFuel;
+            if (!P->mvSelection) { double *sm = P->suM[j]; forN(P, N, [=] __device__(long c) { sm[c] = nu * wFuel[c]; }); sj = sm; }
+            nuq[j] = nu;
             if (!P->mvSelection) FFM_TRY(ffm_bc_values(m, P->fS, P->refY[i], P->zeroB, P->Y[i], P->spB[j]));
             vf[j] = P->Y[i]; vb[j] = P->spB[j]; vf0[j] = P->Y0[i]; fq[j] = P->fS; rq[j] = P->refY[i]; gq[j] = P->zeroB; suq[j] = sj;
             ggx[j] = P->gM[j][0]; ggy[j] = P->gM[j][1]; ggz[j] = P->gM[j][2]; cgx[j] = ggx[j]; cgy[j] = ggy[j]; cgz[j] = ggz[j];
         }
         double *uShared[4] = {P->spU[0], nullptr, nullptr, nullptr}, *lShared[4] = {P->spL[0], nullptr, nullptr, nullptr};
         if (P->mvSelection)
-            FFM_TRY(ffm_fvm_scalar_transport_multi_w(m, ns, P->wMv, rdt, P->rho, P->rho0, P->phi, P->phib, af, afb, vf0, fq, rq, gq, suq, nullptr, nullptr,
-                                                     nullptr, P->spD, uShared, lShared, P->spS));
+            FFM_TRY(ffm_fvm_scalar_transport_multi_ws(m, ns, P->wMv, rdt, P->rho, P->rho0, P->phi, P->phib, af, afb, vf0, fq, rq, gq, suq, nuq, nullptr,
+                                                      nullptr, nullptr, P->spD, uShared, lShared, P->spS));
         else {
         FFM_TRY(ffm_fvc_grad_multi(m, ns, vf, vb, ggx, ggy, ggz));
         for (int j = 0; j < ns; j++) { FFM_TRY(HX(P, ggx[j])); FFM_TRY(HX(P, ggy[j])); FFM_TRY(HX(P, ggz[j])); }
@@ -675,8 +682,15 @@
             const int i = sp[j];
             if (!P->mvSelection) FFM_TRY(solve_named(P, SPN[i], FFM_PBICGSTAB, FFM_DILU, 1e-8, 0.0, P->spD[j], P->spU[j], P->spL[j], P->Y[i], P->spS[j]));
             FFM_TRY(HX(P, P->Y[i]));
-            double *Yi = P->Y[i];
-            forN(P, N, [=] __device__(long c) { const double v = fmax(Yi[c], 0.0); Yi[c] = v; Yt[c] += v; });
+        }
+        {
+            double *y0 = P->Y[sp[0]], *y1 = P->Y[sp[1]], *y2 = P->Y[sp[2]], *y3 = P->Y[sp[3]], *Yn = P->Y[INERT];
+            forN(P, N, [=] __device__(long c) {
+                const double a = fmax(y0[c], 0.0), b = fmax(y1[c], 0.0), d = fmax(y2[c], 0.0), e = fmax(y3[c], 0.0);
+                y0[c] = a; y1[c] = b; y2[c] = d; y3[c] = e;
+                const double t = (((0.0 + a) + b) + d) + e;
+                Yn[c] = fmax(1.0 - t, 0.0);
+            });
         }
     } else
     for (int i = 0; i < NSP; i++) {
@@ -687,7 +701,7 @@
         double *Yi = P->Y[i];
         forN(P, N, [=] __device__(long c) { const double v = fmax(Yi[c], 0.0); Yi[c] = v; Yt[c] += v; });
     }
-    {
+    if (!P->fused) {
         double *Yn = P->Y[INERT];
         forN(P, N, [=] __device__(long c) { Yn[c] = fmax(1.0 - Yt[c], 0.0); });
     }
@@ -700,15 +714,22 @@
         forN(P, B, [=] __device__(long k) { Kb[k] = 0.5 * ((b0[k] * b0[k] + b1[k] * b1[k]) + b2[k] * b2[k]); });
         FFM_TRY(ffm_fvc_grad(m, P->K, Kb, kgx, kgy, kgz));
         FFM_TRY(HX(P, kgx)); FFM_TRY(HX(P, kgy)); FFM_TRY(HX(P, kgz));
+        double *divK = P->wN[4], *ddtK = P->wN[0], *ndpdt = P->wN[5];
+        int rcK = FFM_ERR_UNSUPPORTED;
+        if (P->fused) {
+            rcK = ffm_fvc_div_phiK_terms(m, 2, 1.0, 0.0, 1.0, rdt, P->phi, P->phib, P->K, Kb, kgx, kgy, kgz, P->rho, P->rho0, P->K0, P->dpdt, divK, ddtK, ndpdt);
+            if (rcK != FFM_OK && rcK != FFM_ERR_UNSUPPORTED) return rcK;
+        }
+        if (rcK != FFM_OK) {
         FFM_TRY(ffm_fv_limited_weights(m, 2, 1.0, 0.0, 1.0, P->phi, P->K, kgx, kgy, kgz, wK));
         FFM_TRY(ffm_fvc_interpolate(m, wK, P->K, Kf));
         const double *phi = P->phi, *phib = P->phib;
         forN(P, nNat, [=] __device__(long e) { Kf[e] = phi[e] * Kf[e]; });
         forN(P, B, [=] __device__(long k) { KfB[k] = phib[k] * Kb[k]; });
-        double *divK = P->wN[4];
         FFM_TRY(ffm_fvc_surface_integrate(m, Kf, KfB, divK));
-        double *ddtK = P->wN[0], *ndpdt = P->wN[5]; const double *rho = P->rho, *rho0 = P->rho0, *K = P->K, *K0 = P->K0, *dpdt = P->dpdt;
+        const double *rho = P->rho, *rho0 = P->rho0, *K = P->K, *K0 = P->K0, *dpdt = P->dpdt;
         forN(P, N, [=] __device__(long c) { ddtK[c] = rdt * (rho[c] * K[c] - rho0[c] * K0[c]); ndpdt[c] = -dpdt[c]; });
+        }
         const double *expl[3] = {ddtK, divK, ndpdt};
         const double *shSu = nullptr, *shSp = nullptr;
         if (P->radCoupled && P->radHaveG) {
@@ -900,12 +921,12 @@
     const int ny_glob = gy;
     const int B = Btot; const long nNat = P->nNat;
     auto NN = [&]() { return dalloc(P, N); };
-    for (int i = 0; i < NSP; i++) { P->Y[i] = dfill(P, N, Y_AMB[i]); P->Y0[i] = NN(); }
+    for (int i = 0; i < NSP; i++) { P->Y[i] = dfill(P, N, Y_AMB[i]); P->Y0[i] = i == INERT ? nullptr : NN(); }
     P->T = dfill(P, N, TREF); P->hs = NN(); P->hs0 = NN();
     for (int c = 0; c < 3; c++) { P->U[c] = NN(); P->U0[c] = NN(); }
     P->p = dfill(P, N, PREF); P->p0 = NN(); P->p_rgh = NN(); P->p_rgh0 = NN(); P->psi = NN(); P->psi0 = NN();
     P->rho = NN(); P->rho0 = NN(); P->K = NN(); P->K0 = NN(); P->dpdt = NN(); P->ph_rgh = NN();
-    P->phi = dalloc(P, nNat); P->phi0 = dalloc(P, nNat); P->phib = dalloc(P, B); P->phib0 = dalloc(P, B); P->ph_rgh_b = dalloc(P, B);
+    P->phi = dalloc(P, nNat); P->phib = dalloc(P, B); P->ph_rgh_b = dalloc(P, B);
     {
         const double ghRef = -9.81 * (ny_glob * h);
         std::vector<double> gh(N), ghf(std::max<long>(nNat, 1), 0.0);
@@ -1047,9 +1068,16 @@
 extern "C" int ffm_plume_set_initial_state(ffm_plume *P, const double *const *Y, const double *h, const double *Yamb, const double *Yin, double hAmb)
 {
     if (!P || !Y || !h || !Yamb || !Yin) return FFM_ERR_ARG;
-    if (P->stepNo != 0 || P->N != P->nOwn) { ffm_set_error("plume: the start state can be set on a single block before the first step only"); return FFM_ERR_ARG; }
+    if (P->N != P->nOwn) { ffm_set_error("plume: the start state can be set on a single block only"); return FFM_ERR_ARG; }
     PL_HIP(hipSetDevice(P->ctx->device));
     const int N = P->N, B = P->B;
+    if (P->stepNo != 0) {
+        PL_HIP(hipStreamSynchronize(P->ctx->stream));
+        for (int c = 0; c < 3; c++) FFM_TRY(ffm_dzero(P->ctx, P->U[c], sizeof(double) * N));
+        FFM_TRY(ffm_dzero(P->ctx, P->K, sizeof(double) * N)); FFM_TRY(ffm_dzero(P->ctx, P->dpdt, sizeof(double) * N));
+        FFM_TRY(ffm_dzero(P->ctx, P->phi, sizeof(double) * std::max<long>(P->nNat, 1))); FFM_TRY(ffm_dzero(P->ctx, P->phib, sizeof(double) * std::max(B, 1)));
+        P->stepNo = 0; P->time = 0.0; P->radHaveG = false; P->mvOverride = false; P->ddtCorrValid = false;
+    }
     std::vector<double> v(N);
     auto up = [&](double *dst, const double *nat) -> int {
         for (int c = 0; c < N; c++) v[c] = nat[P->newToOld[c]];
@@ -1129,6 +1157,10 @@
     if (n == "K") return cellF(P->K); if (n == "dpdt") return cellF(P->dpdt); if (n == "gh") return cellF(P->gh); if (n == "T") return cellF(P->T);
     if (n == "Ux") return cellF(P->U[0]); if (n == "Uy") return cellF(P->U[1]); if (n == "Uz") return cellF(P->U[2]);
     for (int i = 0; i < NSP; i++) if (n == SPN[i]) return cellF(P->Y[i]);
+    if (n == "rho0") return cellF(P->rho0); if (n == "K0") return cellF(P->K0); if (n == "psi0") return cellF(P->psi0); if (n == "psi") return cellF(P->psi);
+    if (n == "h0") return cellF(P->hs0); if (n == "p0") return cellF(P->p0); if (n == "p_rgh0") return cellF(P->p_rgh0);
+    for (int c = 0; c < 3; c++) if (n == std::string("U0") + char('x' + c)) return cellF(P->U0[c]);
+    for (int i = 0; i < NSP; i++) if (i != INERT && n == std::string(SPN[i]) + "_0") return cellF(P->Y0[i]);
     if (n == "phi") return faceF(P->phi); if (n == "ghf") return faceF(P->ghf);
     if (n == "phib") return bndF(P->phib); if (n == "ph_rgh_b") return bndF(P->ph_rgh_b); if (n == "kind") return bndF(P->kind_d);
     if (n == "fStaticS") return bndF(P->fStaticS); if (n == "fStaticH") return bndF(P->fStaticH); if (n == "refH") return bndF(P->refH);
diff --git a/include/ffm.h b/include/ffm.h
--- a/include/ffm.h
+++ b/include/ffm.h
@@ -216,6 +216,15 @@
                 const double *rhorAUf, double *flux_f, double *phi_f, double *t_f);
 int ffm_ue_buoyancy_flux(ffm_mesh *m, const double *ghf, const double *rho, const double *p_rgh, double *t_f);
 int ffm_fvc_flux_rho(ffm_mesh *m, const double *rho, const double *vx, const double *vy, const double *vz, double *out_f);
+int ffm_fvc_ddt_corr(ffm_mesh *m, double rDeltaT, const double *rho0, const double *vx0, const double *vy0, const double *vz0,
+                     const double *phi0_f, double *out_f);
+int ffm_fvm_rAU(ffm_mesh *m, int nCmpt, const double *diag, const double *ic0, const double *ic1, const double *ic2,
+                const double *psi, const double *p, double *rho, double *rAU, double *rhorAU);
+int ffm_fvc_rho_eqn(ffm_mesh *m, double rDeltaT, const double *phi_f, const double *phi_b, const double *rho0, double *rho);
+int ffm_fvc_div_phiK_terms(ffm_mesh *m, int scheme, double k, double lo, double hi, double rDeltaT, const double *phi_f,
+                           const double *phi_b, const double *K, const double *K_b, const double *gx, const double *gy,
+                           const double *gz, const double *rho, const double *rho0, const double *K0, const double *dpdt,
+                           double *divK, double *ddtK, double *negDpdt);
 int ffm_fvm_flux(ffm_mesh *m, const double *upper, const double *lower, const double *internalCoeffs,
                  const double *boundaryCoeffs, const double *psi, double *out_f, double *out_b);
 
@@ -236,6 +245,12 @@
                                      const double *const *refGrad, const double *const *su, const double *const *su2,
                                      const double *const *sp, const double *const *expl3, double *const *diag,
                                      double *const *upper, double *const *lower, double *const *source);
+int ffm_fvm_scalar_transport_multi_ws(ffm_mesh *m, int nf, const double *w_f, double rDeltaT, const double *rho, const double *rho0,
+                                      const double *phi_f, const double *phi_b, const double *gamma_f, const double *gamma_b,
+                                      const double *const *vf0, const double *const *f, const double *const *ref,
+                                      const double *const *refGrad, const double *const *su, const double *suFactor,
+                                      const double *const *su2, const double *const *sp, const double *const *expl3,
+                                      double *const *diag, double *const *upper, double *const *lower, double *const *source);
 int ffm_fvm_lust_source3(ffm_mesh *m, double rDeltaT, const double *phi_f, const double *rho0, const double *const *U0,
                          const double *const *gx, const double *const *gy, const double *const *gz, double *const *source);
 
```

Measured after the change: 2.909 outer-iterations/s (median of 6 runs). 1.9% higher.
